# googlegenomics/spark-examples

Hardware: NVIDIA B200
Metric: genotype-cells/sec (N x V) into Gram (higher is better)
Workload: dtype int8

## Files before the change

### include/vpca.h

```cpp
#ifndef VPCA_H_
#define VPCA_H_

#include <stddef.h>
#include <stdint.h>

#ifdef __cplusplus
extern "C" {
#endif

#define VPCA_VERSION_MAJOR 0
#define VPCA_VERSION_MINOR 2

typedef enum vpca_status {
    VPCA_OK = 0,
    VPCA_ERR_BAD_ARG = -1,
    VPCA_ERR_INDEX_OUT_OF_RANGE = -2,
    VPCA_ERR_CUDA = -3,
    VPCA_ERR_NCCL = -4,
    VPCA_ERR_OVERFLOW = -5,
    VPCA_ERR_STATE = -6,
    VPCA_ERR_NOMEM = -7,
    VPCA_ERR_UNSUPPORTED = -8
} vpca_status;

typedef enum vpca_dtype {
    VPCA_DTYPE_I8 = 0,
    VPCA_DTYPE_BF16 = 1,
    VPCA_DTYPE_E2M1 = 2
} vpca_dtype;

typedef struct vpca_ctx vpca_ctx;

typedef struct vpca_config {
    uint32_t struct_size;
    int32_t n_samples;
    int32_t device;
    int32_t dtype;
    int32_t num_pc;
    int32_t max_multiplicity;
    int32_t partitions_in_flight;
    int32_t staging_lanes;
    int64_t chunk_variants;
    int64_t chunk_nnz;
    void* stream;
    void* d_gram;
    int32_t gram_band_row0;
    int32_t gram_band_rows;
} vpca_config;

int vpca_version(void);
int vpca_create(const vpca_config* cfg, vpca_ctx** out);
int vpca_destroy(vpca_ctx* ctx);
const char* vpca_last_error(const vpca_ctx* ctx);
int vpca_reset(vpca_ctx* ctx);
int vpca_synchronize(vpca_ctx* ctx);
int vpca_host_alloc(size_t bytes, void** out);
int vpca_host_free(void* p);

int vpca_encode_calls(vpca_ctx* ctx, const int64_t* offsets, const int32_t* sample_idx, int64_t nv, void* out,
                      int64_t ld);

int vpca_accumulate_calls(vpca_ctx* ctx, int64_t partition_id, const int64_t* offsets, const int32_t* sample_idx,
                          int64_t nv);
int vpca_accumulate_calls_u16(vpca_ctx* ctx, int64_t partition_id, const int64_t* offsets, const uint16_t* sample_idx,
                              int64_t nv);
int vpca_accumulate_bits(vpca_ctx* ctx, int64_t partition_id, const uint8_t* bits, int64_t nv, int64_t stride_bytes);
int vpca_accumulate_bed(vpca_ctx* ctx, int64_t partition_id, const uint8_t* rows, int64_t nv, int64_t stride_bytes,
                        int32_t counted_allele);
int vpca_commit(vpca_ctx* ctx, int64_t partition_id);
int vpca_abort(vpca_ctx* ctx, int64_t partition_id);

int vpca_accumulate_dense(vpca_ctx* ctx, const void* x, int64_t nv, int64_t ld, int on_device);

int vpca_accumulate_panels(vpca_ctx* ctx, const void* d_x, int64_t nv, int64_t panel_variants);

int vpca_gram_device_ptr(vpca_ctx* ctx, void** d_gram);
int vpca_gram_export_ipc(vpca_ctx* ctx, void* handle64);
int vpca_gram_set_peers(vpca_ctx* ctx, const void* handles, int32_t world, int32_t rank);
int vpca_gram_set_peers_local(vpca_ctx* const* ctxs, int32_t world);
int vpca_peer_barrier(vpca_ctx* ctx);
enum { VPCA_PEER_REPLICATE = 0, VPCA_PEER_OWNER_ROWS = 1 };
int vpca_gram_set_peer_mode(vpca_ctx* ctx, int32_t mode);
int vpca_gram_gather(vpca_ctx* ctx);
int vpca_owner_row_bands(int32_t n_samples, int32_t world, int32_t* row_end );
int vpca_get_gram_band(vpca_ctx* ctx, int32_t row0, int32_t rows, int32_t* out);

int vpca_finalize_gram(vpca_ctx* ctx);
int vpca_get_gram(vpca_ctx* ctx, int32_t* out);
int vpca_get_partial_gram(vpca_ctx* ctx, int32_t* out, int64_t* variants_in_gram );
int vpca_load_partial_gram(vpca_ctx* ctx, const int32_t* gram, int64_t variants_in_gram);
int64_t vpca_variant_count(vpca_ctx* ctx);
int vpca_set_gram(vpca_ctx* ctx, const int32_t* gram);

int vpca_compute_pca(vpca_ctx* ctx, int32_t k, double* vecs, double* evals, int32_t* non_zero_rows);
int vpca_get_centered(vpca_ctx* ctx, double* out);
int vpca_get_tridiagonal(vpca_ctx* ctx, double* diag, double* offdiag);

typedef struct vpca_projection {
    uint32_t struct_size;
    int32_t n_projected;
    const int32_t* sample_rows;
} vpca_projection;
int vpca_create_projecting(const vpca_config* cfg, const vpca_projection* proj, vpca_ctx** out);
int vpca_get_cross_gram(vpca_ctx* ctx, int32_t* out);
int vpca_project_pca(vpca_ctx* ctx, int32_t k, double* out);
int vpca_pca_loadings_calls(vpca_ctx* ctx, int32_t k, const int64_t* offsets, const int32_t* sample_idx, int64_t nv,
                            double* loadings, int32_t* carriers);
int vpca_pca_loadings_bed(vpca_ctx* ctx, int32_t k, const uint8_t* rows, int64_t nv, int64_t stride_bytes,
                          int32_t counted_allele, double* loadings, int32_t* carriers);
int vpca_pca_loadings_panels(vpca_ctx* ctx, int32_t k, const void* d_x, int64_t nv, int64_t panel_variants,
                             double* loadings, int32_t* carriers);
int vpca_pca_model_terms(vpca_ctx* ctx, int32_t k, double* eigenvalues, double* col_sums, double* rowsum_dots,
                         double* matrix_mean);

typedef struct vpca_model {
    uint32_t struct_size;
    int32_t n_fitted, k;
    int64_t n_variants;
    const double* loadings;
    const int32_t* carriers;
    const double* eigenvalues, *col_sums, *rowsum_dots;
    double matrix_mean;
} vpca_model;
int vpca_create_scoring(const vpca_config* cfg, const vpca_model* model, vpca_ctx** out);
int vpca_score_calls(vpca_ctx* ctx, int64_t partition_id, const int64_t* offsets, const int32_t* sample_idx, int64_t nv,
                     const int32_t* model_rows);
int vpca_score_bed(vpca_ctx* ctx, int64_t partition_id, const uint8_t* rows, int64_t nv, int64_t stride_bytes,
                   int32_t counted_allele, const int32_t* model_rows);
int vpca_score_panels(vpca_ctx* ctx, const void* d_x, int64_t nv, int64_t panel_variants, const int32_t* model_rows);
int vpca_score_project(vpca_ctx* ctx, int32_t k, double* out, int64_t* matched_variants );

int vpca_debug_projection_tiles(int32_t n_fit, int32_t n_total, int32_t cta_group, int32_t mxf4, int32_t* out,
                                int32_t max_tiles);

typedef struct vpca_pool vpca_pool;
int vpca_pool_create(const vpca_config* cfg, int32_t n_gpus, const int32_t* devices ,
                     vpca_pool** out);
int vpca_pool_destroy(vpca_pool* pool);
int32_t vpca_pool_size(const vpca_pool* pool);
vpca_ctx* vpca_pool_ctx(vpca_pool* pool, int64_t partition_id);
const char* vpca_pool_last_error(const vpca_pool* pool);
int vpca_pool_reset(vpca_pool* pool);
int vpca_pool_accumulate_calls(vpca_pool* pool, int64_t partition_id, const int64_t* offsets, const int32_t* sample_idx,
                               int64_t nv);
int vpca_pool_accumulate_calls_u16(vpca_pool* pool, int64_t partition_id, const int64_t* offsets,
                                   const uint16_t* sample_idx, int64_t nv);
int vpca_pool_accumulate_bits(vpca_pool* pool, int64_t partition_id, const uint8_t* bits, int64_t nv, int64_t stride_bytes);
int vpca_pool_accumulate_bed(vpca_pool* pool, int64_t partition_id, const uint8_t* rows, int64_t nv, int64_t stride_bytes,
                             int32_t counted_allele);
int vpca_pool_commit(vpca_pool* pool, int64_t partition_id);
int vpca_pool_abort(vpca_pool* pool, int64_t partition_id);
int vpca_pool_reduce_and_finalize(vpca_pool* pool);
int vpca_pool_get_gram(vpca_pool* pool, int32_t* out);
int vpca_pool_compute_pca(vpca_pool* pool, int32_t k, double* vecs, double* evals, int32_t* non_zero_rows);
struct vpca_stats;
int vpca_pool_get_stats(vpca_pool* pool, struct vpca_stats* out);

int vpca_synth_dense_device(vpca_ctx* ctx, uint64_t seed, int64_t v0, int64_t nv, int mode, void* d_x, int64_t ld);

int vpca_synth_panels_device(vpca_ctx* ctx, uint64_t seed, int64_t v0, int64_t nv, int mode, void* d_x,
                             int64_t panel_variants);

typedef struct vpca_stats {
    int64_t variants_accumulated;
    int64_t gram_launches;
    int64_t kernel_launches;
    int64_t h2d_bytes;
    int64_t d2h_bytes;
    float last_gram_ms;
    float last_eig_ms;
    int32_t gram_cta_group;
    int32_t gram_resident;
    int32_t eig_method;
    int32_t eig_iterations;
} vpca_stats;
int vpca_get_stats(vpca_ctx* ctx, vpca_stats* out);
int vpca_debug_gram_profile(vpca_ctx* ctx, int64_t* out, int32_t max_ctas);
int vpca_debug_lanczos_profile(vpca_ctx* ctx, int64_t* out, int32_t max_steps);

#define VPCA_JOIN 0
#define VPCA_MERGE 1
int vpca_hash_keys(vpca_ctx* ctx, const uint8_t* payload, const int64_t* key_offsets, int64_t nkeys, uint64_t* out);
int vpca_join_rows(vpca_ctx* ctx, int32_t mode, int32_t variant_set_count, int64_t n_left, const uint8_t* key_payload,
                   const int64_t* key_offsets, const int64_t* offsets, const int32_t* sample_idx, int64_t nrows,
                   int64_t* out_rows, int64_t* out_nnz);
int vpca_join_fetch(vpca_ctx* ctx, int64_t* out_offsets, int32_t* out_idx);
int vpca_join_size(vpca_ctx* ctx, int64_t* out_rows, int64_t* out_nnz);
int vpca_accumulate_joined(vpca_ctx* ctx, int64_t partition_id);

int vpca_debug_rebalance(const int32_t* tiles, int32_t num_tiles, int32_t workers, int32_t kb_window, int32_t col_limit,
                         double* cum, int32_t* out, int32_t max_pieces);
int vpca_debug_tiles(int32_t n_samples, int32_t cta_group, int32_t exact, int32_t* out, int32_t max_tiles);
int vpca_debug_band_tiles(int32_t n_samples, int32_t cta_group, int32_t row0, int32_t rows, int32_t* out, int32_t max_tiles);
int vpca_debug_max_clusters(int32_t device, int32_t cluster_size);
int vpca_debug_plan(const int32_t* tiles, int32_t num_tiles, int32_t workers, int32_t kb_window, int32_t* out, int32_t max_pieces);

#ifdef __cplusplus
}
#endif
#endif
```

### spark_examples_b200/csrc/gram_sm100.cu

```cuda
#include <cuda.h>
#include <cuda_runtime.h>

#include <cstring>

#include <algorithm>
#include <map>
#include <mutex>
#include <tuple>
#include <cstdio>
#include <cstdlib>
#include <string>
#include <vector>

#include "ptx_sm100.cuh"
#include "vpca_internal.h"

namespace vpca {

namespace {

constexpr int kThreads = 256;
constexpr int kKBytes = 128;
constexpr int kBoxRows = 128;
constexpr int kBoxBytes = kBoxRows * kKBytes;
constexpr int kUmmaN = 256;
constexpr int kUmmaNScaled = 240;
constexpr uint32_t kSfCol = 480;
constexpr uint32_t kTmemCols = 512;
constexpr long long kWatchdogCycles = 20000000000LL;

template <int CG, int KIND = 0>
struct Cfg {
    static constexpr int A_BYTES = kBoxBytes;
    static constexpr int B_BYTES = (kUmmaN / CG) * kKBytes;
    static constexpr int STAGE_BYTES = A_BYTES + B_BYTES;
    static constexpr int STAGES = CG == 1 ? 4 : 6;
    static constexpr int BAR_BYTES = 256;
    static constexpr int SMEM_BYTES = STAGES * STAGE_BYTES + BAR_BYTES + 1024;
};

constexpr int kMaxPeers = 16;

struct TileDesc {
    int rowA0, rowA1;
    int rowB;
    int n_eff;
    int wstart;
    int flags;
    int acc_cols;
    int pad1;
};
constexpr int kTileXpose = 1, kTileFiller = 2, kTileSelfB = 4;
constexpr int kMaxSegs = 4;

struct GramArgs {
    int32_t* S;
    int32_t* peer[kMaxPeers];
    int num_peers;
    int peer_mode;
    int own_end[kMaxPeers];
    const TileDesc* tiles;
    int* err;
    int n_cols;
    int num_tiles;
    int num_full;
    int total_weight;
    int kb_total;
    int kb_window;
    int num_workers;
    int resident;
    int elems_per_kb;
    int kb_per_panel;
    int sync_lead;
    int active_workers;
    int* win_done;
    long long* prof;
    const double* cum;
    int col_limit;
    int acc_stride;
    int row_limit;
    int red64;
    int tx_shift;
};

struct Seg {
    int tile, kb0, kb1, col, slot, first, flush, use, win, last_in_win;
    int rowA0, rowA1, rowB, n_eff, flags;
};

struct SegPlan {
    int n;
    int tile[kMaxSegs], lo[kMaxSegs], hi[kMaxSegs], col[kMaxSegs];
    int cols;
    int overflow;
};

__host__ __device__ inline void plan_segments(const TileDesc* tiles, int num_tiles, int first_tile, long long u_begin,
                                              long long u_end, int len, SegPlan& p) {
    p.n = 0;
    p.cols = 0;
    p.overflow = 0;
    const long long origin = (long long)tiles[first_tile].wstart * len;
    long long u = u_begin;
    int t = first_tile;
    while (u < u_end && t < num_tiles) {
        const int w = tiles[t].n_eff >> 4;
        const long long base = (long long)tiles[t].wstart * len - origin;
        const long long tend = base + (long long)w * len;
        if (tend <= u) {
            ++t;
            continue;
        }
        const long long e = u_end < tend ? u_end : tend;
        const int lo = (int)((u - base) / w);
        const int hi = e == tend ? len : (int)((e - base) / w);
        u = e;
        if (lo >= hi) continue;
        if (p.n == kMaxSegs) {
            p.overflow = 1;
            return;
        }
        p.tile[p.n] = t;
        p.lo[p.n] = lo;
        p.hi[p.n] = hi;
        p.col[p.n] = p.cols;
        p.cols += tiles[t].acc_cols;
        ++p.n;
    }
}

__host__ __device__ inline long long feasible_end(const TileDesc* tiles, int num_tiles, long long u_begin, long long u_end,
                                                  int len, int col_limit, int& hint) {
    int n = 0, cols = 0;
    long long u = u_begin;
    int t = hint;
    bool first = true;
    while (u < u_end && t < num_tiles) {
        const int w = tiles[t].n_eff >> 4;
        const long long base = (long long)tiles[t].wstart * len;
        const long long tend = base + (long long)w * len;
        if (tend <= u) {
            ++t;
            continue;
        }
        if (first) {
            hint = t;
            first = false;
        }
        const long long e = u_end < tend ? u_end : tend;
        const int lo = (int)((u - base) / w);
        const int hi = e == tend ? len : (int)((e - base) / w);
        if (lo < hi) {
            if (n == kMaxSegs || cols + tiles[t].acc_cols > col_limit) return u;
            ++n;
            cols += tiles[t].acc_cols;
        }
        u = e;
    }
    return u_end;
}

__host__ __device__ inline bool repair_split(const TileDesc* tiles, int num_tiles, int workers, long long uw, int len,
                                             int col_limit, double* cand) {
    long long ub = 0;
    int hint = 0;
    for (int i = 0; i < workers; ++i) {
        long long ue = (i + 1 == workers) ? uw : (long long)((double)uw * cand[i + 1]);
        if (ue < ub) ue = ub;
        const long long fe = feasible_end(tiles, num_tiles, ub, ue, len, col_limit, hint);
        if (fe < ue) {
            if (i + 1 == workers) return false;
            ue = fe;
        }
        if (i + 1 < workers) cand[i + 1] = ((double)ue + 0.5) / (double)uw;
        ub = ue;
    }
    return true;
}

struct Sched {
    SegPlan plan;
    long long u_begin, u_end, u;
    int kbw, nwin, kb_total, resident, win, seg_i, nflush, acc_stride;
    int worker, workers, num_tiles, wave, full_waves, tail_first;
    const TileDesc* tiles;

    __device__ void init(const GramArgs& a, int w) {
        kbw = a.kb_window;
        kb_total = a.kb_total;
        resident = a.resident;
        acc_stride = a.acc_stride;
        worker = w;
        workers = a.num_workers;
        num_tiles = a.num_tiles;
        tiles = a.tiles;
        nwin = (kb_total + kbw - 1) / kbw;
        win = 0;
        seg_i = 0;
        nflush = 0;
        wave = 0;
        if (resident) {
            const long long uw = (long long)a.total_weight * kbw;
            u_begin = (long long)((double)uw * a.cum[worker]);
            u_end = (worker + 1 == a.num_workers) ? uw : (long long)((double)uw * a.cum[worker + 1]);
            plan_segments(tiles, num_tiles, 0, u_begin, u_end, kbw, plan);
            if (plan.overflow || plan.cols > a.col_limit) {
                if (a.err != nullptr && threadIdx.x == 0) {
                    a.err[0] = 9;
                    a.err[1] = (int)blockIdx.x;
                    a.err[2] = plan.cols;
                    a.err[3] = plan.n;
                    __threadfence_system();
                }
                __trap();
            }
        } else {
            full_waves = a.num_full / workers;
            tail_first = full_waves * workers;
            const long long tail_units =
                tail_first < num_tiles ? (long long)(a.total_weight - tiles[tail_first].wstart) * kb_total : 0;
            u_begin = tail_units * worker / workers;
            u_end = tail_units * (worker + 1) / workers;
            plan.n = 0;
        }
        u = u_begin;
    }
    __device__ void fill(Seg& s, int t) const {
        const int4 lo = __ldg(reinterpret_cast<const int4*>(tiles + t));
        const int4 hi = __ldg(reinterpret_cast<const int4*>(tiles + t) + 1);
        s.tile = t;
        s.rowA0 = lo.x;
        s.rowA1 = lo.y;
        s.rowB = lo.z;
        s.n_eff = lo.w;
        s.flags = hi.y;
    }
    __device__ bool next(Seg& s) {
        if (!resident) {
            s.win = 0;
            s.last_in_win = 0;
            s.first = 1;
            s.flush = 1;
            s.slot = nflush & 1;
            s.col = s.slot * acc_stride;
            s.use = nflush >> 1;
            if (wave < full_waves) {
                fill(s, wave * workers + worker);
                s.kb0 = 0;
                s.kb1 = kb_total;
                ++wave;
                ++nflush;
                return true;
            }
            while (true) {
                if (seg_i < plan.n) {
                    fill(s, plan.tile[seg_i]);
                    s.kb0 = plan.lo[seg_i];
                    s.kb1 = plan.hi[seg_i];
                    ++seg_i;
                    ++nflush;
                    return true;
                }
                if (u >= u_end) return false;
                plan_segments(tiles, num_tiles, tail_first, u, u_end, kb_total, plan);
                seg_i = 0;
                if (plan.n == 0) return false;
                const int lt = plan.tile[plan.n - 1];
                const long long base = (long long)(tiles[lt].wstart - tiles[tail_first].wstart) * kb_total;
                const long long endu = base + (long long)plan.hi[plan.n - 1] * (tiles[lt].n_eff >> 4);
                u = plan.overflow ? endu : u_end;
            }
        }
        if (plan.n == 0) return false;
        if (seg_i == plan.n) {
            ++win;
            seg_i = 0;
        }
        if (win >= nwin) return false;
        const int i = seg_i++;
        fill(s, plan.tile[i]);
        const int base = win * kbw;
        const int cnt = min(kbw, kb_total - base);
        s.kb0 = base + min(plan.lo[i], cnt);
        s.kb1 = base + min(plan.hi[i], cnt);
        s.win = win;
        s.last_in_win = (seg_i == plan.n);
        s.col = plan.col[i];
        s.slot = i;
        s.first = (win == 0);
        s.flush = (win == nwin - 1);
        s.use = 0;
        return true;
    }
};

__device__ __forceinline__ void mbar_wait(uint32_t bar, uint32_t parity, int* err, int code) {
    if (ptx::mbar_try_wait(bar, parity)) return;
    const long long t0 = clock64();
    while (!ptx::mbar_try_wait(bar, parity)) {
        if (clock64() - t0 > kWatchdogCycles) {
            if (err != nullptr) {
                err[0] = code;
                err[1] = (int)blockIdx.x;
                err[2] = (int)bar;
                err[3] = (int)parity;
                __threadfence_system();
            }
            __trap();
        }
    }
}

__device__ __forceinline__ long long globaltimer_ns() {
    long long t;
    asm volatile("mov.u64 %0, %%globaltimer;" : "=l"(t));
    return t;
}

__device__ __forceinline__ void wait_window(const int* win_done, int w, int need) {
    const long long t0 = globaltimer_ns();
    while (true) {
        int v;
        asm volatile("ld.acquire.gpu.global.s32 %0, [%1];" : "=r"(v) : "l"(win_done + w) : "memory");
        if (v >= need) return;
        if (globaltimer_ns() - t0 > 200000) return;
        __nanosleep(256);
    }
}

__device__ __forceinline__ uint64_t make_smem_desc(uint32_t saddr) {
    return (uint64_t)((saddr & 0x3FFFFu) >> 4) | ((uint64_t)(1024 >> 4) << 32) | (1ull << 46) | (2ull << 61);
}

template <int CG, int KIND>
__device__ __forceinline__ uint32_t make_instr_desc(uint32_t N) {
    constexpr uint32_t M = 128 * CG;
    if constexpr (KIND == 3) {
        return (1u << 7) | (1u << 10) | ((N >> 3) << 17) | (1u << 23) | ((M >> 4) << 24);
    }
    constexpr uint32_t cfmt = (KIND == 0) ? 2u : 1u;
    constexpr uint32_t abfmt = (KIND == 2) ? 5u : 1u;
    return (cfmt << 4) | (abfmt << 7) | (abfmt << 10) | ((N >> 3) << 17) | ((M >> 4) << 24);
}

template <int CG, int KIND>
__global__ void __launch_bounds__(kThreads, 1) gram_kernel(const __grid_constant__ CUtensorMap tmap,
                                                           const __grid_constant__ CUtensorMap tmap_half, const GramArgs a) {
    using C = Cfg<CG, KIND>;
    extern __shared__ uint8_t smem_raw[];
    uint8_t* smem = reinterpret_cast<uint8_t*>((reinterpret_cast<uintptr_t>(smem_raw) + 1023) & ~uintptr_t(1023));
    const uint32_t smem_base = ptx::smem_u32(smem);
    const uint32_t bar_base = smem_base + C::STAGES * C::STAGE_BYTES;
    auto sA = [&](uint32_t st) { return smem_base + st * C::A_BYTES; };
    auto sB = [&](uint32_t st) { return smem_base + C::STAGES * C::A_BYTES + st * C::B_BYTES; };
    auto full_bar = [&](uint32_t i) { return bar_base + 8u * i; };
    auto empty_bar = [&](uint32_t i) { return bar_base + 8u * (C::STAGES + i); };
    auto tfull_bar = [&](uint32_t i) { return bar_base + 8u * (2 * C::STAGES + i); };
    auto tempty_bar = [&](uint32_t i) { return bar_base + 8u * (2 * C::STAGES + kMaxSegs + i); };
    volatile uint32_t* tmem_ptr_smem =
        reinterpret_cast<volatile uint32_t*>(smem + C::STAGES * C::STAGE_BYTES + 8 * (2 * C::STAGES + kMaxSegs + 2));

    const int warp = __shfl_sync(0xffffffffu, (int)(threadIdx.x >> 5), 0);
    const uint32_t lane = ptx::lane_id();
    const uint32_t cta_rank = (CG == 2) ? ptx::cluster_ctarank() : 0u;
    const bool leader = cta_rank == 0;
    const int worker = (CG == 2) ? (int)(blockIdx.x >> 1) : (int)blockIdx.x;
    const bool issuer = ptx::elect_one();

    if constexpr (CG == 2) ptx::cluster_sync();

    if (warp == 0 && issuer) {
        ptx::prefetch_tensormap(&tmap);
        ptx::prefetch_tensormap(&tmap_half);
    } else if (warp == 1 && issuer) {
        for (uint32_t i = 0; i < (uint32_t)C::STAGES; ++i) {
            ptx::mbar_init(full_bar(i), CG);
            ptx::mbar_init(empty_bar(i), 1);
        }
        for (uint32_t i = 0; i < (uint32_t)kMaxSegs; ++i) ptx::mbar_init(tfull_bar(i), 1);
        for (uint32_t i = 0; i < 2; ++i) ptx::mbar_init(tempty_bar(i), CG * 128);
        ptx::fence_mbar_init();
    } else if (warp == 2) {
        ptx::tmem_alloc<CG>(ptx::smem_u32(const_cast<uint32_t*>(tmem_ptr_smem)), kTmemCols);
        ptx::tmem_relinquish<CG>();
    }
    ptx::tc_fence_before();
    if constexpr (CG == 2) ptx::cluster_sync(); else __syncthreads();
    ptx::tc_fence_after();
    const uint32_t tmem_base = *tmem_ptr_smem;
    if constexpr (KIND == 3) {
        if (warp >= 4) {
            ptx::tmem_st_32x32b_x16_const(tmem_base + ((uint32_t)((warp & 3) * 32) << 16) + kSfCol, 0x7F7F7F7Fu);
            ptx::tmem_st_wait();
        }
        ptx::tc_fence_before();
        if constexpr (CG == 2) ptx::cluster_sync(); else __syncthreads();
        ptx::tc_fence_after();
    }
    if (a.prof != nullptr && threadIdx.x == 0) a.prof[(size_t)blockIdx.x * 4 + 0] = globaltimer_ns();

    if (warp == 0) {
        if (issuer) {
            Sched sc;
            sc.init(a, worker);
            Seg s;
            uint32_t it = 0;
            int synced_win = -1;
            while (sc.next(s)) {
                const int rowA = (CG == 2 && cta_rank != 0) ? s.rowA1 : s.rowA0;
                const int rowB = s.rowB + ((CG == 2) ? (int)cta_rank * (s.n_eff / 2) : 0);
                const bool half_box = (CG == 2) && (s.n_eff <= 128);
                const bool two_boxes = (CG == 1) && (s.n_eff > kBoxRows);
                const bool self_b = (CG == 2) && (s.flags & kTileSelfB) != 0;
                const uint32_t tx_cta =
                    (uint32_t)(C::A_BYTES + (self_b ? 0 : (half_box ? kBoxBytes / 2 : (two_boxes ? 2 * kBoxBytes : kBoxBytes))));
                if (a.sync_lead > 0 && leader && s.win != synced_win) {
                    synced_win = s.win;
                    if (s.win >= a.sync_lead) wait_window(a.win_done, s.win - a.sync_lead, a.active_workers);
                }
                for (int kb = s.kb0; kb < s.kb1; ++kb, ++it) {
                    const uint32_t st = it % C::STAGES, ph = (it / C::STAGES) & 1u;
                    mbar_wait(empty_bar(st), ph ^ 1u, a.err, 1);
                    const int pnl = kb / a.kb_per_panel;
                    const int kc = (kb - pnl * a.kb_per_panel) * a.elems_per_kb;
                    if constexpr (CG == 1) {
                        ptx::mbar_arrive_expect_tx(full_bar(st), tx_cta >> a.tx_shift);
                        ptx::tma_load_3d(sA(st), &tmap, full_bar(st), kc, rowA, pnl);
                        ptx::tma_load_3d(sB(st), &tmap, full_bar(st), kc, rowB, pnl);
                        if (two_boxes) ptx::tma_load_3d(sB(st) + kBoxBytes, &tmap, full_bar(st), kc, rowB + kBoxRows, pnl);
                    } else {
                        ptx::tma_load_3d_2sm(sA(st), &tmap, full_bar(st), kc, rowA, pnl);
                        if (!self_b) ptx::tma_load_3d_2sm(sB(st), half_box ? &tmap_half : &tmap, full_bar(st), kc, rowB, pnl);
                        if (leader) ptx::mbar_arrive_expect_tx(full_bar(st), (2u * tx_cta) >> a.tx_shift);
                        else ptx::mbar_arrive_cluster(full_bar(st), 0);
                    }
                }
                if (a.sync_lead > 0 && leader && s.last_in_win)
                    asm volatile("red.release.gpu.global.add.s32 [%0], 1;" ::"l"(a.win_done + s.win) : "memory");
            }
        }
    } else if (warp == 1 && leader) {
        Sched sc;
        sc.init(a, worker);
        Seg s;
        uint32_t it = 0;
        while (sc.next(s)) {
            if (s.first && !a.resident) {
                mbar_wait(tempty_bar((uint32_t)s.slot), (uint32_t)(s.use & 1) ^ 1u, a.err, 2);
                ptx::tc_fence_after();
            }
            const uint32_t d_tmem = tmem_base + (uint32_t)s.col;
            const uint32_t idesc = make_instr_desc<CG, KIND>((uint32_t)s.n_eff);
            for (int kb = s.kb0; kb < s.kb1; ++kb, ++it) {
                const uint32_t st = it % C::STAGES, ph = (it / C::STAGES) & 1u;
                mbar_wait(full_bar(st), ph, a.err, 3);
                ptx::tc_fence_after();
                if (issuer) {
                    const uint64_t adesc = make_smem_desc(sA(st));
                    const uint64_t bdesc = make_smem_desc((CG == 2 && (s.flags & kTileSelfB) != 0) ? sA(st) : sB(st));
                    uint32_t acc = (s.first && kb == s.kb0) ? 0u : 1u;
#pragma unroll
                    for (int k = 0; k < kKBytes / 32; ++k) {
                        if constexpr (KIND == 3)
                            ptx::umma_ss_mxf4<CG>(d_tmem, adesc + 2 * k, bdesc + 2 * k, idesc, acc, tmem_base + kSfCol,
                                                  tmem_base + kSfCol + 4);
                        else
                            ptx::umma_ss<CG, KIND>(d_tmem, adesc + 2 * k, bdesc + 2 * k, idesc, acc);
                        acc = 1u;
                    }
                    ptx::umma_commit<CG>(empty_bar(st));
                }
                __syncwarp();
            }
            if (s.flush) {
                if (issuer) ptx::umma_commit<CG>(tfull_bar((uint32_t)s.slot));
                __syncwarp();
            }
        }
        if (a.prof != nullptr && issuer) a.prof[(size_t)blockIdx.x * 4 + 2] = globaltimer_ns();
    } else if (warp >= 4) {
        const int q = warp & 3;
        Sched sc;
        sc.init(a, worker);
        Seg s;
        while (sc.next(s)) {
            if (!s.flush) continue;
            const uint32_t bar_i = (uint32_t)s.slot;
            mbar_wait(tfull_bar(bar_i), (uint32_t)(s.use & 1), a.err, 4);
            ptx::tc_fence_after();
            const bool filler = (CG == 2) && cta_rank != 0 && (s.flags & kTileFiller) != 0;
            const int colbase = ((CG == 2 && cta_rank != 0) ? s.rowA1 : s.rowA0) + q * 32;
            const int col = colbase + (int)lane;
            const uint32_t taddr = tmem_base + ((uint32_t)(q * 32) << 16) + (uint32_t)s.col;
            const int row_end = min(a.row_limit, s.rowB + s.n_eff);
            const int nchunks = filler ? 0 : (s.n_eff + 31) / 32;
#pragma unroll 1
            for (int c = 0; c < nchunks; ++c) {
                const int rbase = s.rowB + c * 32;
                if (rbase >= row_end) break;
                bool xpose = false;
                if (rbase + 31 < colbase) {
                    if ((s.flags & kTileXpose) == 0 || (rbase >> 7) >= (colbase >> 7)) continue;
                    xpose = true;
                }
                uint32_t r[32];
                ptx::tmem_ld_32x32b_x32(taddr + (uint32_t)(c * 32), r);
                ptx::tmem_ld_wait();
                int32_t* own_lo = nullptr;
                int32_t* own_hi = nullptr;
                int own_split = 0;
                if (a.num_peers != 0 && a.peer_mode == 1) {
                    const int probe = xpose ? col : rbase;
                    int o = 0;
                    while (o + 1 < a.num_peers && probe >= a.own_end[o]) ++o;
                    own_split = xpose ? 0x7fffffff : a.own_end[o];
                    own_lo = a.peer[o];
                    own_hi = a.peer[min(o + 1, a.num_peers - 1)];
                }
                if (!xpose && a.red64 != 0 && (a.n_cols & 1) == 0) {
#pragma unroll
                    for (int jj = 0; jj < 16; ++jj) {
                        const int row0 = rbase + 2 * jj, row1 = row0 + 1;
                        int v0, v1;
                        if constexpr (KIND == 0) { v0 = (int)r[2 * jj]; v1 = (int)r[2 * jj + 1]; }
                        else { v0 = __float2int_rn(__uint_as_float(r[2 * jj])); v1 = __float2int_rn(__uint_as_float(r[2 * jj + 1])); }
                        if (!(row0 < row_end && col < a.n_cols && row0 >= col)) v0 = 0;
                        if (!(row1 < row_end && col < a.n_cols && row1 >= col)) v1 = 0;
                        const int got = __shfl_xor_sync(0xffffffffu, (lane & 1) ? v0 : v1, 1);
                        const int srow = (lane & 1) ? row1 : row0;
                        const unsigned long long packed = (lane & 1)
                            ? ((unsigned long long)(unsigned)got | ((unsigned long long)(unsigned)v1 << 32))
                            : ((unsigned long long)(unsigned)v0 | ((unsigned long long)(unsigned)got << 32));
                        if (packed != 0ull) {
                            const size_t o = (size_t)srow * (size_t)a.n_cols + (size_t)(col & ~1);
                            if (a.num_peers == 0) {
                                asm volatile("red.global.add.u64 [%0], %1;" ::"l"(a.S + o), "l"(packed) : "memory");
                            } else if (a.peer_mode == 1) {
                                int32_t* dst = (srow >= own_split ? own_hi : own_lo) + o;
                                asm volatile("red.relaxed.sys.global.add.u64 [%0], %1;" ::"l"(dst), "l"(packed) : "memory");
                            } else {
                                for (int d = 0; d < a.num_peers; ++d)
                                    asm volatile("red.relaxed.sys.global.add.u64 [%0], %1;" ::"l"(a.peer[d] + o), "l"(packed)
                                                 : "memory");
                            }
                        }
                    }
                    continue;
                }
#pragma unroll
                for (int j = 0; j < 32; ++j) {
                    const int row = rbase + j;
                    if (row < row_end && col < a.n_cols && (xpose || row >= col)) {
                        int v;
                        if constexpr (KIND == 0) v = (int)r[j];
                        else v = __float2int_rn(__uint_as_float(r[j]));
                        if (v != 0) {
                            const int srow = xpose ? col : row, scol = xpose ? row : col;
                            const size_t o = (size_t)srow * (size_t)a.n_cols + (size_t)scol;
                            if (a.num_peers == 0) {
                                asm volatile("red.global.add.s32 [%0], %1;" ::"l"(a.S + o), "r"(v) : "memory");
                            } else if (a.peer_mode == 1) {
                                int32_t* dst = (srow >= own_split ? own_hi : own_lo) + o;
                                asm volatile("red.relaxed.sys.global.add.s32 [%0], %1;" ::"l"(dst), "r"(v) : "memory");
                            } else {
                                for (int d = 0; d < a.num_peers; ++d)
                                    asm volatile("red.relaxed.sys.global.add.s32 [%0], %1;" ::"l"(a.peer[d] + o), "r"(v)
                                                 : "memory");
                            }
                        }
                    }
                }
            }
            ptx::tc_fence_before();
            if (!a.resident) {
                if constexpr (CG == 1) ptx::mbar_arrive(tempty_bar(bar_i));
                else ptx::mbar_arrive_cluster(tempty_bar(bar_i), 0);
            }
        }
    }

    ptx::tc_fence_before();
    if constexpr (CG == 2) ptx::cluster_sync(); else __syncthreads();
    if (warp == 2) ptx::tmem_dealloc<CG>(tmem_base, kTmemCols);
    if (a.prof != nullptr && threadIdx.x == 0) a.prof[(size_t)blockIdx.x * 4 + 3] = globaltimer_ns();
}

__global__ void rebalance_kernel(const long long* __restrict__ prof, double* __restrict__ cum, int workers, int cta_group,
                                 double gain, double max_share, long long min_ns, int* __restrict__ gen, const TileDesc* __restrict__ tiles,
                                 int num_tiles, int total_weight, int kbw, int col_limit) {
    __shared__ double sh[1024];
    __shared__ double cand[1025];
    __shared__ double red_sum, red_min;
    __shared__ int reject, need_repair;
    const int w = threadIdx.x;
    const bool active = w < workers;
    double t = 0.0, share_old = 0.0;
    if (active) {
        const long long t0 = prof[(size_t)w * cta_group * 4 + 0], t1 = prof[(size_t)w * cta_group * 4 + 2];
        t = (double)(t1 - t0);
        share_old = cum[w + 1] - cum[w];
    }
    sh[w] = active ? t : 1e30;
    if (w == 0) {
        reject = 0;
        need_repair = 0;
    }
    __syncthreads();
    if (w == 0) {
        double mn = 1e30, mx = 0.0;
        for (int i = 0; i < workers; ++i) {
            mn = fmin(mn, sh[i]);
            mx = fmax(mx, sh[i]);
        }
        red_min = (mn < (double)min_ns || (mx - mn) < 0.03 * mx) ? -1.0 : mn;
    }
    __syncthreads();
    if (red_min < 0.0) return;
    const double speed = active ? share_old / t : 0.0;
    sh[w] = speed;
    __syncthreads();
    if (w == 0) {
        double sum = 0.0;
        for (int i = 0; i < workers; ++i) sum += sh[i];
        red_sum = sum;
    }
    __syncthreads();
    double share = 0.0;
    if (active) {
        const double est = speed / red_sum;
        share = (1.0 - gain) * share_old + gain * est;
        const double avg = 1.0 / workers;
        share = fmin(fmax(share, 0.5 * avg), max_share * avg);
    }
    __syncthreads();
    sh[w] = share;
    __syncthreads();
    if (w == 0) {
        double sum = 0.0;
        for (int i = 0; i < workers; ++i) sum += sh[i];
        double acc = 0.0;
        cand[0] = 0.0;
        for (int i = 0; i < workers; ++i) {
            acc += sh[i] / sum;
            cand[i + 1] = (i + 1 == workers) ? 1.0 : acc;
        }
    }
    __syncthreads();
    if (active) {
// ... 2 lines not shown
        const long long ue = (w + 1 == workers) ? uw : (long long)((double)uw * cand[w + 1]);
        int hint = 0;
        if (feasible_end(tiles, num_tiles, ub, ue, kbw, col_limit, hint) < ue) atomicExch(&need_repair, 1);
    }
    __syncthreads();
    if (need_repair && w == 0 && !repair_split(tiles, num_tiles, workers, (long long)total_weight * kbw, kbw, col_limit, cand)) reject = 1;
    __syncthreads();
    if (reject) return;
    if (w <= workers) cum[w] = cand[w];
    if (w == 0) *gen += 1;
}

__global__ void symmetrize_kernel(int32_t* __restrict__ S, int n) {
    __shared__ int32_t tile[32][33];
    const int bx = blockIdx.x, by = blockIdx.y;
    if (bx < by) return;
    const int tx = threadIdx.x, ty = threadIdx.y;
    for (int r = ty; r < 32; r += 8) {
        const int row = bx * 32 + r, col = by * 32 + tx;
        tile[r][tx] = (row < n && col < n) ? S[(size_t)row * n + col] : 0;
    }
    __syncthreads();
    for (int r = ty; r < 32; r += 8) {
        const int row = by * 32 + r, col = bx * 32 + tx;
        if (row < n && col < n && row < col) S[(size_t)row * n + col] = tile[tx][r];
    }
}

__global__ void add_i32_kernel(int32_t* __restrict__ dst, const int32_t* __restrict__ src, int64_t count) {
    int64_t i = (int64_t)blockIdx.x * blockDim.x + threadIdx.x;
    const int64_t stride = (int64_t)gridDim.x * blockDim.x;
    for (; i < count; i += stride) dst[i] += src[i];
}

struct PeerPtrs {
    int32_t* p[kMaxPeers];
};

__global__ void add_i32_peers_kernel(PeerPtrs dst, int npeers, const int32_t* __restrict__ src, int64_t count) {
    int64_t i = (int64_t)blockIdx.x * blockDim.x + threadIdx.x;
    const int64_t stride = (int64_t)gridDim.x * blockDim.x;
    for (; i < count; i += stride) {
        const int v = src[i];
        if (v != 0)
            for (int d = 0; d < npeers; ++d)
                asm volatile("red.relaxed.sys.global.add.s32 [%0], %1;" ::"l"(dst.p[d] + i), "r"(v) : "memory");
    }
}

struct OwnEnds {
    int e[kMaxPeers];
};

__device__ __forceinline__ int owner_of_row(const OwnEnds& own, int npeers, int row) {
    int q = 0;
    while (q + 1 < npeers && row >= own.e[q]) ++q;
    return q;
}

__global__ void add_i32_owner_kernel(PeerPtrs dst, OwnEnds own, int npeers, const int32_t* __restrict__ src, int n) {
    for (int row = blockIdx.x; row < n; row += gridDim.x) {
        int32_t* d = dst.p[owner_of_row(own, npeers, row)] + (size_t)row * n;
        const int32_t* s = src + (size_t)row * n;
        for (int c = threadIdx.x; c <= row; c += blockDim.x) {
            const int v = s[c];
            if (v != 0) asm volatile("red.relaxed.sys.global.add.s32 [%0], %1;" ::"l"(d + c), "r"(v) : "memory");
        }
    }
}

__global__ void __launch_bounds__(256) gather_rows_kernel(PeerPtrs src, int32_t* __restrict__ dst, OwnEnds own, int npeers,
                                                          int rank, int n) {
    const bool vec = (n & 3) == 0;
    for (int row = blockIdx.x; row < n; row += gridDim.x) {
        const int q = owner_of_row(own, npeers, row);
        if (q == rank) continue;
        const int32_t* s = src.p[q] + (size_t)row * n;
        int32_t* d = dst + (size_t)row * n;
        if (vec) {
            const int4* s4 = reinterpret_cast<const int4*>(s);
            int4* d4 = reinterpret_cast<int4*>(d);
            for (int c = threadIdx.x; c < (row + 4) / 4; c += blockDim.x) d4[c] = s4[c];
        } else {
            for (int c = threadIdx.x; c <= row; c += blockDim.x) d[c] = s[c];
        }
    }
}

__global__ void __launch_bounds__(256) push_rows_kernel(PeerPtrs dst, const int32_t* __restrict__ src, OwnEnds own,
                                                        int npeers, int rank, int n) {
    const bool vec = (n & 3) == 0;
    const int row_lo = rank == 0 ? 0 : own.e[rank - 1], row_hi = own.e[rank];
    for (int row = row_lo + blockIdx.x; row < row_hi; row += gridDim.x) {
        const int32_t* s = src + (size_t)row * n;
        if (vec) {
            const int4* s4 = reinterpret_cast<const int4*>(s);
            for (int c = threadIdx.x; c < (row + 4) / 4; c += blockDim.x) {
                const int4 v = s4[c];
                for (int d = 0; d < npeers; ++d)
                    if (d != rank) reinterpret_cast<int4*>(dst.p[d] + (size_t)row * n)[c] = v;
            }
        } else {
            for (int c = threadIdx.x; c <= row; c += blockDim.x) {
                const int v = s[c];
                for (int d = 0; d < npeers; ++d)
                    if (d != rank) dst.p[d][(size_t)row * n + c] = v;
            }
        }
    }
}

__global__ void peer_barrier_kernel(PeerPtrs flags, int npeers, int rank, int epoch) {
    const int d = threadIdx.x;
    if (d < npeers) {
        __threadfence_system();
        asm volatile("st.release.sys.global.s32 [%0], %1;" ::"l"(flags.p[d] + rank), "r"(epoch) : "memory");
        int v;
        const long long t0 = globaltimer_ns();
        do {
            asm volatile("ld.acquire.sys.global.s32 %0, [%1];" : "=r"(v) : "l"(flags.p[rank] + d) : "memory");
            if (v < epoch && globaltimer_ns() - t0 > 30000000000LL) __trap();
        } while (v < epoch);
    }
    __syncthreads();
    __threadfence_system();
}

typedef CUresult (*EncodeTiledFn)(CUtensorMap*, CUtensorMapDataType, cuuint32_t, void*, const cuuint64_t*,
                                  const cuuint64_t*, const cuuint32_t*, const cuuint32_t*, CUtensorMapInterleave,
                                  CUtensorMapSwizzle, CUtensorMapL2promotion, CUtensorMapFloatOOBfill);

EncodeTiledFn get_encode_fn() {
    static EncodeTiledFn fn = nullptr;
    if (fn == nullptr) {
        void* p = nullptr;
        cudaDriverEntryPointQueryResult qres;
        if (cudaGetDriverEntryPoint("cuTensorMapEncodeTiled", &p, cudaEnableDefault, &qres) == cudaSuccess &&
            qres == cudaDriverEntryPointSuccess)
            fn = reinterpret_cast<EncodeTiledFn>(p);
    }
    return fn;
}

template <int CG, int KIND>
cudaError_t launch(const CUtensorMap& tmap, const CUtensorMap& tmap_half, const GramArgs& args, int grid, cudaStream_t stream) {
    using C = Cfg<CG, KIND>;
    cudaError_t ea = cudaFuncSetAttribute(gram_kernel<CG, KIND>, cudaFuncAttributeMaxDynamicSharedMemorySize, C::SMEM_BYTES);
    if (ea != cudaSuccess) return ea;
    cudaLaunchConfig_t cfg{};
    cfg.gridDim = dim3((unsigned)grid);
    cfg.blockDim = dim3(kThreads);
    cfg.dynamicSmemBytes = C::SMEM_BYTES;
    cfg.stream = stream;
    cudaLaunchAttribute attr[1];
    attr[0].id = cudaLaunchAttributeClusterDimension;
    attr[0].val.clusterDim.x = CG;
    attr[0].val.clusterDim.y = 1;
    attr[0].val.clusterDim.z = 1;
    cfg.attrs = attr;
    cfg.numAttrs = 1;
    return cudaLaunchKernelEx(&cfg, gram_kernel<CG, KIND>, tmap, tmap_half, args);
}

}

namespace {
struct SplitKey {
    int dev, n, rows, tiles, kbw, workers, elem;
    bool operator<(const SplitKey& o) const {
        return std::tie(dev, n, rows, tiles, kbw, workers, elem) <
               std::tie(o.dev, o.n, o.rows, o.tiles, o.kbw, o.workers, o.elem);
    }
};
std::mutex g_split_mu;
std::map<SplitKey, std::vector<double>> g_splits;
}

static void remember_split(GramPlan& plan) {
    if (plan.d_cum == nullptr || plan.cum_workers <= 0 || !plan.adaptive) return;
    if (plan.own_hi > plan.own_lo && plan.num_peers <= 1) return;
    std::vector<double> cum((size_t)plan.cum_workers + 1);
    if (cudaMemcpy(cum.data(), plan.d_cum, cum.size() * sizeof(double), cudaMemcpyDeviceToHost) != cudaSuccess) {
        cudaGetLastError();
        return;
    }
    std::lock_guard<std::mutex> lk(g_split_mu);
    g_splits[SplitKey{plan.cum_dev, plan.cum_for_n, plan.cum_for_rows, plan.cum_tiles, plan.cum_kbw, plan.cum_workers, plan.cum_elem}] = std::move(cum);
}

void gram_plan_free(GramPlan& plan) {
    remember_split(plan);
    if (plan.d_tiles) cudaFree(plan.d_tiles);
    plan.h_tiles.clear();
    if (plan.d_err) cudaFreeHost(plan.d_err);
    if (plan.d_win_done) cudaFree(plan.d_win_done);
    if (plan.d_prof) cudaFree(plan.d_prof);
    if (plan.d_cum) cudaFree(plan.d_cum);
    plan.d_cum = nullptr;
    plan.d_win_done = nullptr;
    plan.d_prof = nullptr;
    plan.d_tiles = nullptr;
    plan.d_err = nullptr;
    plan.tiles_for_n = -1;
}

int gram_read_profile(GramPlan& plan, long long* out, int max_ctas) {
    if (plan.d_prof == nullptr) return 0;
    const int ctas = std::min(max_ctas, std::min(1024, plan.num_sms));
    if (cudaMemcpy(out, plan.d_prof, (size_t)ctas * 4 * sizeof(long long), cudaMemcpyDeviceToHost) != cudaSuccess) return 0;
    return ctas;
}

static void make_tiles(int n, int cg, bool exact, int bn, int row_lo, int row_hi, bool self_b, std::vector<TileDesc>& out,
                       int* num_full) {
    out.clear();
    auto n_eff = [&](int row0, int want) { return std::min(want, ((n - row0) + 15) & ~15); };
    if (!exact) {
        const int BM = 128 * cg;
        const int span = row_hi - row_lo;
        const int nbn = (span + bn - 1) / bn, nbm = (n + BM - 1) / BM;
        const int units = (span + 15) / 16;
        std::vector<int> row0(nbn + 1, row_lo);
        for (int b = 0; b < nbn; ++b) row0[b + 1] = row0[b] + 16 * (units / nbn + (b < units % nbn ? 1 : 0));
        constexpr int kStrip = 8;
        for (int bb = 0; bb < nbn; bb += kStrip)
            for (int am = 0; am < nbm; ++am)
                for (int b = bb; b < std::min(nbn, bb + kStrip); ++b) {
                    const int max_row = std::min(row_hi, row0[b + 1]) - 1;
                    if (am * BM > max_row) continue;
                    TileDesc t{};
                    t.rowA0 = am * BM;
                    t.rowA1 = am * BM + 128;
                    t.rowB = row0[b];
                    t.n_eff = std::min(row0[b + 1], ((row_hi + 15) & ~15)) - row0[b];
                    t.acc_cols = bn;
                    if (self_b && cg == 2 && t.rowB == t.rowA0 && t.n_eff == 2 * 128) t.flags |= kTileSelfB;
                    out.push_back(t);
                }
    } else {
        const int nb = (n + 127) / 128;
        std::vector<TileDesc> two, one;
        auto emit = [&](std::vector<TileDesc>& dst, int c0, int c1, int r0, int rows, bool filler) {
            TileDesc t{};
            t.rowA0 = c0 * 128;
            t.rowA1 = c1 * 128;
            t.rowB = r0 * 128;
            t.n_eff = n_eff(r0 * 128, rows * 128);
            t.acc_cols = (t.n_eff + 31) & ~31;
            t.flags = kTileXpose | (filler ? kTileFiller : 0);
            dst.push_back(t);
        };
        std::vector<std::vector<int>> need(nb);
        for (int r = 0; r < nb; ++r)
            for (int c = 0; c <= r; ++c) need[r].push_back(c);
        if (cg == 2)
            for (int r = 0; r + 2 < nb; r += 4) {
                need[r].push_back(r + 2);
                need[r + 2].erase(std::find(need[r + 2].begin(), need[r + 2].end(), r));
            }
        for (int r0 = 0; r0 < nb; r0 += 2) {
            const bool pair = r0 + 1 < nb;
            std::vector<int> common, left0, left1;
            if (pair) {
                for (int c : need[r0])
                    if (std::find(need[r0 + 1].begin(), need[r0 + 1].end(), c) != need[r0 + 1].end()) common.push_back(c);
                if (cg == 2 && (common.size() & 1)) common.pop_back();
            }
            for (int c : need[r0])
                if (std::find(common.begin(), common.end(), c) == common.end()) left0.push_back(c);
            if (pair)
                for (int c : need[r0 + 1])
                    if (std::find(common.begin(), common.end(), c) == common.end()) left1.push_back(c);
            for (size_t i = 0; i < common.size(); i += cg) emit(two, common[i], common[cg == 2 ? i + 1 : i], r0, 2, false);
            for (int side = 0; side < (pair ? 2 : 1); ++side) {
                const std::vector<int>& left = side == 0 ? left0 : left1;
                for (size_t i = 0; i < left.size(); i += cg) {
                    const bool filler = cg == 2 && i + 1 >= left.size();
                    emit(one, left[i], filler ? left[i] : left[cg == 2 ? i + 1 : i], r0 + side, 1, filler);
                }
            }
        }
        auto mid = std::stable_partition(two.begin(), two.end(), [&](const TileDesc& t) { return t.n_eff == 256; });
        std::stable_sort(two.begin(), mid, [](const TileDesc& x, const TileDesc& y) {
            const int sx = x.rowB / 1024, sy = y.rowB / 1024;
            if (sx != sy) return sx < sy;
            const int cx = std::min(x.rowA0, x.rowA1) / 256, cy = std::min(y.rowA0, y.rowA1) / 256;
            if (cx != cy) return cx < cy;
            return x.rowB < y.rowB;
        });
        *num_full = (int)(mid - two.begin());
        out = two;
        out.insert(out.end(), one.begin(), one.end());
    }
    if (!exact) *num_full = (int)out.size();
    int w = 0;
    for (auto& t : out) {
        t.wstart = w;
        w += t.n_eff >> 4;
    }
}

static cudaError_t build_tiles(GramPlan& plan, int n, bool exact, int BN, int row_lo, int row_hi, cudaStream_t stream) {
    std::vector<TileDesc> tiles;
    int num_full = 0;
    make_tiles(n, plan.cta_group, exact, BN, row_lo, row_hi, plan.self_b, tiles, &num_full);
    if (plan.d_tiles) cudaFree(plan.d_tiles);
    plan.d_tiles = nullptr;
    cudaError_t e = cudaMalloc(&plan.d_tiles, tiles.size() * sizeof(TileDesc));
    if (e != cudaSuccess) return e;
    e = cudaMemcpyAsync(plan.d_tiles, tiles.data(), tiles.size() * sizeof(TileDesc), cudaMemcpyHostToDevice, stream);
    if (e != cudaSuccess) return e;
    e = cudaStreamSynchronize(stream);
    plan.h_tiles.assign(reinterpret_cast<const int32_t*>(tiles.data()),
                        reinterpret_cast<const int32_t*>(tiles.data() + tiles.size()));
    plan.num_tiles = (int)tiles.size();
    plan.num_full = num_full;
    plan.total_weight = tiles.empty() ? 0 : tiles.back().wstart + (tiles.back().n_eff >> 4);
    plan.tiles_for_n = n;
    plan.tiles_for_cg = plan.cta_group;
    plan.tiles_for_bn = exact ? -1 : BN;
    plan.tiles_row_lo = row_lo;
    plan.tiles_row_hi = row_hi;
    plan.tiles_col_limit = (!exact && BN == kUmmaNScaled) ? (int)kSfCol : (int)kTmemCols;
    return e;
}

static bool initial_split(const GramPlan& plan, int workers, int kbw, std::vector<double>& cum) {
    if (plan.total_weight <= 0) return false;
    const TileDesc* tiles = reinterpret_cast<const TileDesc*>(plan.h_tiles.data());
    const long long uw = (long long)plan.total_weight * kbw;
    cum.resize((size_t)workers + 1);
    for (int w = 0; w <= workers; ++w) cum[w] = (double)w / (double)workers;
    if (!repair_split(tiles, plan.num_tiles, workers, uw, kbw, plan.tiles_col_limit, cum.data())) return false;
    for (int w = 0; w < workers; ++w) {
        const long long ub = (long long)((double)uw * cum[w]);
        const long long ue = (w + 1 == workers) ? uw : (long long)((double)uw * cum[w + 1]);
        SegPlan p;
        plan_segments(tiles, plan.num_tiles, 0, ub, ue, kbw, p);
        if (p.overflow || p.cols > plan.tiles_col_limit) return false;
    }
    return true;
}

int gram_debug_tiles(int n, int cta_group, int exact, int32_t* out, int max_tiles) {
    std::vector<TileDesc> tiles;
    int num_full = 0;
    make_tiles(n, cta_group == 1 ? 1 : 2, exact != 0, exact ? kUmmaN : kUmmaNScaled, 0, n, true, tiles, &num_full);
    const int cnt = std::min<int>((int)tiles.size(), max_tiles);
    if (out != nullptr && cnt > 0) memcpy(out, tiles.data(), (size_t)cnt * sizeof(TileDesc));
    return (int)tiles.size();
}

int gram_debug_projection_tiles(int n_fit, int n_total, int cta_group, bool mxf4, int32_t* out, int max_tiles) {
    std::vector<TileDesc> tiles;
    int num_full = 0;
    make_tiles(n_fit, cta_group == 1 ? 1 : 2, false, mxf4 ? kUmmaNScaled : kUmmaN, 0, n_total, true, tiles, &num_full);
    const int cnt = std::min<int>((int)tiles.size(), max_tiles);
    if (out != nullptr && cnt > 0) memcpy(out, tiles.data(), (size_t)cnt * sizeof(TileDesc));
    return (int)tiles.size();
}

int gram_debug_band_tiles(int n, int cta_group, int row_lo, int row_hi, int32_t* out, int max_tiles) {
    std::vector<TileDesc> tiles;
    int num_full = 0;
    make_tiles(n, cta_group == 1 ? 1 : 2, false, kUmmaN, row_lo, row_hi, true, tiles, &num_full);
    const int cnt = std::min<int>((int)tiles.size(), max_tiles);
    if (out != nullptr && cnt > 0) memcpy(out, tiles.data(), (size_t)cnt * sizeof(TileDesc));
    return (int)tiles.size();
}

int gram_debug_plan(const int32_t* tiles8, int num_tiles, int workers, int kbw, int32_t* out, int max_pieces) {
    const TileDesc* tiles = reinterpret_cast<const TileDesc*>(tiles8);
    if (num_tiles <= 0) return 0;
    const int col_limit = tiles[0].acc_cols == kUmmaNScaled ? (int)kSfCol : (int)kTmemCols;
    std::vector<double> cum((size_t)workers + 1);
    for (int w = 0; w <= workers; ++w) cum[w] = (double)w / (double)workers;
    return gram_debug_repair(tiles8, num_tiles, workers, kbw, col_limit, cum.data(), out, max_pieces);
}

int gram_debug_repair(const int32_t* tiles8, int num_tiles, int workers, int kbw, int col_limit, double* cum, int32_t* out,
                      int max_pieces) {
    const TileDesc* tiles = reinterpret_cast<const TileDesc*>(tiles8);
    if (num_tiles <= 0) return 0;
    const long long total = tiles[num_tiles - 1].wstart + (tiles[num_tiles - 1].n_eff >> 4);
    const long long uw = total * kbw;
    if (!repair_split(tiles, num_tiles, workers, uw, kbw, col_limit, cum)) return -1000;
    int cnt = 0;
    for (int w = 0; w < workers; ++w) {
        const long long ub = (long long)((double)uw * cum[w]);
        const long long ue = (w + 1 == workers) ? uw : (long long)((double)uw * cum[w + 1]);
        SegPlan p;
        plan_segments(tiles, num_tiles, 0, ub, ue, kbw, p);
        if (p.overflow || p.cols > col_limit) return -1 - w;
        for (int i = 0; i < p.n; ++i, ++cnt)
            if (cnt < max_pieces) {
                int32_t* o = out + (size_t)cnt * 6;
                o[0] = w; o[1] = p.tile[i]; o[2] = p.lo[i]; o[3] = p.hi[i]; o[4] = p.col[i]; o[5] = p.cols;
            }
    }
    return cnt;
}

cudaError_t gram_accumulate(GramPlan& plan, const void* d_x, int elem_bits, int n, int n_rows, int64_t nv, int64_t ld,
                            int64_t panel, int32_t* d_S, cudaStream_t stream, std::string* err) {
    if (nv <= 0) return cudaSuccess;
    EncodeTiledFn encode = get_encode_fn();
    if (encode == nullptr) {
        if (err) *err = "cuTensorMapEncodeTiled entry point not available";
        return cudaErrorNotSupported;
    }
    if (plan.num_sms == 0) {
        int dev = 0;
        cudaGetDevice(&dev);
        cudaDeviceGetAttribute(&plan.num_sms, cudaDevAttrMultiProcessorCount, dev);
        const char* cg = getenv("VPCA_CTA_GROUP");
        if (cg != nullptr) plan.cta_group = (atoi(cg) == 1) ? 1 : 2;
        const char* kw = getenv("VPCA_KB_WINDOW");
        if (kw != nullptr) plan.kb_window = atoi(kw);
        const char* sl = getenv("VPCA_SYNC_LEAD");
        if (sl != nullptr) plan.sync_lead = atoi(sl);
        const char* pf = getenv("VPCA_GRAM_PROF");
        plan.profile = (pf != nullptr && atoi(pf) != 0);
        const char* ad = getenv("VPCA_ADAPTIVE");
        if (ad != nullptr) plan.adaptive = atoi(ad) != 0;
        const char* mx = getenv("VPCA_E2M1_MXF4");
        if (mx != nullptr) plan.e2m1_mxf4 = atoi(mx) != 0;
        const char* sb = getenv("VPCA_SELF_B");
        if (sb != nullptr) plan.self_b = atoi(sb) != 0;
        const char* r64 = getenv("VPCA_RED64");
        if (r64 != nullptr) plan.red64 = atoi(r64) != 0;
        const char* gain = getenv("VPCA_REBALANCE_GAIN");
        if (gain != nullptr) plan.gain = std::min(1.0, std::max(0.1, atof(gain)));
        const char* ex = getenv("VPCA_EXACT_COVER");
        if (ex != nullptr) plan.exact_cover = atoi(ex) != 0;
    }
    if (plan.d_win_done == nullptr) {
        cudaError_t e = cudaMalloc(&plan.d_win_done, GramPlan::kMaxWindows * sizeof(int));
        if (e != cudaSuccess) return e;
    }
    if ((plan.profile || plan.adaptive) && plan.d_prof == nullptr) {
        cudaError_t e = cudaMalloc(&plan.d_prof, 1024 * 4 * sizeof(long long));
        if (e != cudaSuccess) return e;
        e = cudaMemsetAsync(plan.d_prof, 0, 1024 * 4 * sizeof(long long), stream);
        if (e != cudaSuccess) return e;
    }
    if (plan.d_err == nullptr) {
        cudaError_t e = cudaHostAlloc(&plan.d_err, 4 * sizeof(int), cudaHostAllocMapped);
        if (e != cudaSuccess) return e;
        for (int i = 0; i < 4; ++i) plan.d_err[i] = 0;
    }
    const bool mxf4 = (elem_bits == 4 && plan.e2m1_mxf4);
    const int tile_bn = mxf4 ? kUmmaNScaled : kUmmaN;
    const bool banded = plan.own_hi > plan.own_lo && plan.num_peers <= 1;
    const int row_lo = banded ? plan.own_lo : 0, row_hi = banded ? plan.own_hi : n_rows;
    const bool exact = !mxf4 && plan.exact_cover && !banded;
    if ((banded || exact || plan.num_peers > 1) && n_rows != n) {
        if (err) *err = "projected rows need the rectangle tiling without peers or bands";
        return cudaErrorNotSupported;
    }
    if (plan.tiles_for_n != n || plan.tiles_for_cg != plan.cta_group || plan.tiles_for_bn != (exact ? -1 : tile_bn) ||
        plan.tiles_row_lo != row_lo || plan.tiles_row_hi != row_hi) {
        cudaError_t e = build_tiles(plan, n, exact, tile_bn, row_lo, row_hi, stream);
        if (e != cudaSuccess) return e;
    }
    if (panel > 0) {
        if ((panel % 128) != 0) {
            if (err) *err = "panel_variants must be a multiple of 128";
            return cudaErrorInvalidValue;
        }
        ld = panel;
    }
    const uintptr_t align = (elem_bits == 4) ? 31 : 15;
    if ((reinterpret_cast<uintptr_t>(d_x) & align) != 0 || (((ld * elem_bits) / 8) & align) != 0 ||
        (elem_bits == 4 && (ld % 128) != 0)) {
        if (err) *err = "dense tile must be 16-byte aligned with a 16-byte multiple row pitch (32 / ld % 128 == 0 for e2m1)";
        return cudaErrorInvalidValue;
    }

    const int cgp = plan.cta_group;
    const int workers = (cgp == 2) ? plan.num_sms / 2 : plan.num_sms;
    const int elems_per_kb = (elem_bits == 16) ? 64 : (mxf4 ? 256 : 128);
    const int kind = (elem_bits == 8) ? 0 : (elem_bits == 16 ? 1 : (mxf4 ? 3 : 2));
    if (mxf4 && panel > 0 && (panel % 256) != 0) {
        if (err) *err = "kind::mxf4 needs panel_variants % 256 == 0";
        return cudaErrorInvalidValue;
    }

    CUtensorMap tmap;
    const int64_t npanels = panel > 0 ? (nv + panel - 1) / panel : 1;
    const int64_t dim0 = panel > 0 ? panel : (elem_bits == 4 ? (mxf4 ? ((nv + 1) / 2) * 2 : ((nv + 127) / 128) * 128) : nv);
    const cuuint64_t gdim[3] = {(cuuint64_t)dim0, (cuuint64_t)n_rows, (cuuint64_t)npanels};
    const cuuint64_t gstride[2] = {(cuuint64_t)ld * (cuuint64_t)elem_bits / 8,
                                   (cuuint64_t)n_rows * (cuuint64_t)ld * (cuuint64_t)elem_bits / 8};
    const cuuint32_t box[3] = {(cuuint32_t)elems_per_kb, (cuuint32_t)kBoxRows, 1};
    const cuuint32_t estr[3] = {1, 1, 1};
    const CUtensorMapDataType tmtype = elem_bits == 8 ? CU_TENSOR_MAP_DATA_TYPE_UINT8
                                       : (elem_bits == 16 ? CU_TENSOR_MAP_DATA_TYPE_BFLOAT16
                                                          : (mxf4 ? CU_TENSOR_MAP_DATA_TYPE_16U4_ALIGN8B
                                                                  : CU_TENSOR_MAP_DATA_TYPE_16U4_ALIGN16B));
    CUresult r = encode(&tmap, tmtype, 3,
                        const_cast<void*>(d_x), gdim, gstride, box, estr, CU_TENSOR_MAP_INTERLEAVE_NONE,
                        CU_TENSOR_MAP_SWIZZLE_128B, CU_TENSOR_MAP_L2_PROMOTION_L2_256B,
                        CU_TENSOR_MAP_FLOAT_OOB_FILL_NONE);
    if (r != CUDA_SUCCESS) {
        if (err) *err = "cuTensorMapEncodeTiled failed with CUresult " + std::to_string((int)r);
        return cudaErrorInvalidValue;
    }
    CUtensorMap tmap_half;
    const cuuint32_t box_half[3] = {(cuuint32_t)elems_per_kb, (cuuint32_t)(kBoxRows / 2), 1};
    r = encode(&tmap_half, tmtype, 3, const_cast<void*>(d_x), gdim, gstride, box_half, estr, CU_TENSOR_MAP_INTERLEAVE_NONE,
               CU_TENSOR_MAP_SWIZZLE_128B, CU_TENSOR_MAP_L2_PROMOTION_L2_256B, CU_TENSOR_MAP_FLOAT_OOB_FILL_NONE);
    if (r != CUDA_SUCCESS) {
        if (err) *err = "cuTensorMapEncodeTiled (64-row box) failed with CUresult " + std::to_string((int)r);
        return cudaErrorInvalidValue;
    }

    GramArgs args{};
    args.S = banded ? d_S - (ptrdiff_t)plan.own_lo * n : d_S;
    args.num_peers = (plan.num_peers > 1 && d_S == plan.peer_base[plan.peer_rank]) ? plan.num_peers : 0;
    for (int d = 0; d < kMaxPeers; ++d) args.peer[d] = d < plan.num_peers ? plan.peer_S[d] : nullptr;
    args.peer_mode = plan.peer_mode;
    for (int d = 0; d < kMaxPeers; ++d) args.own_end[d] = plan.own_end[d];
    args.tiles = static_cast<const TileDesc*>(plan.d_tiles);
    cudaHostGetDevicePointer(reinterpret_cast<void**>(&args.err), plan.d_err, 0);
    args.n_cols = n;
    args.num_tiles = plan.num_tiles;
    args.num_full = plan.num_full;
    args.total_weight = plan.total_weight;
    args.kb_total = (int)((nv + elems_per_kb - 1) / elems_per_kb);
    args.kb_per_panel = panel > 0 ? (int)(panel / elems_per_kb) : args.kb_total;
    args.num_workers = workers;
    args.elems_per_kb = elems_per_kb;
    args.acc_stride = mxf4 ? kUmmaNScaled : kUmmaN;
    args.col_limit = plan.tiles_col_limit;
    args.row_limit = row_hi;
    args.red64 = plan.red64 ? 1 : 0;
    {
        int kbw = plan.kb_window;
        if (kbw <= 0 && panel > 0) kbw = args.kb_per_panel;
        if (kbw <= 0) {
            const long long target = 32ll << 20;
            kbw = (int)std::max<long long>(8, std::min<long long>(4096, target / ((long long)n_rows * kKBytes)));
        }
        kbw = std::min(kbw, args.kb_total);
        std::vector<double> cum0;
        args.resident = (plan.num_tiles <= 4 * workers && initial_split(plan, workers, kbw, cum0)) ? 1 : 0;
        int dev = 0;
        cudaGetDevice(&dev);
        args.kb_window = args.resident ? kbw : args.kb_total;
        if (args.resident && (plan.d_cum == nullptr || plan.cum_workers != workers || plan.cum_tiles != plan.num_tiles ||
                              plan.cum_kbw != kbw || plan.cum_for_n != n || plan.cum_for_rows != n_rows ||
                              plan.cum_elem != elem_bits)) {
            remember_split(plan);
            if (plan.adaptive && !banded) {
                std::lock_guard<std::mutex> lk(g_split_mu);
                auto it = g_splits.find(SplitKey{dev, n, n_rows, plan.num_tiles, kbw, workers, elem_bits});
                if (it != g_splits.end()) {
                    std::vector<double> learned = it->second;
                    const TileDesc* tiles = reinterpret_cast<const TileDesc*>(plan.h_tiles.data());
                    if (repair_split(tiles, plan.num_tiles, workers, (long long)plan.total_weight * kbw, kbw, plan.tiles_col_limit,
                                     learned.data()))
                        cum0 = learned;
                }
            }
            if (plan.d_cum) cudaFree(plan.d_cum);
            plan.d_cum = nullptr;
            cudaError_t e = cudaMalloc(&plan.d_cum, (size_t)(workers + 2) * sizeof(double) + sizeof(int));
            if (e != cudaSuccess) return e;
            cum0.push_back(0.0);
            cum0.push_back(0.0);
            e = cudaMemcpyAsync(plan.d_cum, cum0.data(), (size_t)(workers + 2) * sizeof(double) + sizeof(int),
                                cudaMemcpyHostToDevice, stream);
            if (e != cudaSuccess) return e;
            plan.cum_workers = workers;
            plan.cum_tiles = plan.num_tiles;
            plan.cum_kbw = kbw;
            plan.cum_for_n = n;
            plan.cum_for_rows = n_rows;
            plan.cum_dev = dev;
            plan.cum_elem = elem_bits;
        }
    }
    plan.last_resident = args.resident;
    const int nwin = (args.kb_total + args.kb_window - 1) / args.kb_window;
    const long long uw = (long long)args.total_weight * args.kb_window;
    args.active_workers = (int)std::min<long long>(workers, uw);
    args.sync_lead = (args.resident && nwin <= GramPlan::kMaxWindows) ? plan.sync_lead : 0;
    args.win_done = plan.d_win_done;
    const bool adapt = plan.adaptive && args.resident && workers <= 1024 && args.active_workers == workers;
    args.prof = (plan.profile || adapt) ? plan.d_prof : nullptr;
    args.cum = plan.d_cum;
    args.tx_shift = (elem_bits == 4 && !mxf4 && getenv("VPCA_E2M1_TX_FULL") == nullptr) ? 1 : 0;
    if (args.sync_lead > 0) {
        cudaError_t e = cudaMemsetAsync(plan.d_win_done, 0, (size_t)nwin * sizeof(int), stream);
        if (e != cudaSuccess) return e;
    }

    const int grid = workers * cgp;
    cudaError_t le;
    if (cgp == 2)
        le = kind == 0 ? launch<2, 0>(tmap, tmap_half, args, grid, stream)
                       : (kind == 1 ? launch<2, 1>(tmap, tmap_half, args, grid, stream)
                                    : (kind == 2 ? launch<2, 2>(tmap, tmap_half, args, grid, stream) : launch<2, 3>(tmap, tmap_half, args, grid, stream)));
    else
        le = kind == 0 ? launch<1, 0>(tmap, tmap_half, args, grid, stream)
                       : (kind == 1 ? launch<1, 1>(tmap, tmap_half, args, grid, stream)
                                    : (kind == 2 ? launch<1, 2>(tmap, tmap_half, args, grid, stream) : launch<1, 3>(tmap, tmap_half, args, grid, stream)));
    if (le != cudaSuccess) return le;
    if (adapt) {
        rebalance_kernel<<<1, 1024, 0, stream>>>(plan.d_prof, plan.d_cum, workers, cgp, plan.gain, 1.35, 300000,
                                                 reinterpret_cast<int*>(plan.d_cum + workers + 2), static_cast<const TileDesc*>(plan.d_tiles), plan.num_tiles,
                                                 plan.total_weight, args.kb_window, plan.tiles_col_limit);
        le = cudaGetLastError();
    }
    return le;
}

cudaError_t gram_preload_kernels(cudaStream_t stream) {
    cudaFuncAttributes fa;
    cudaError_t e = cudaSuccess;
#define VPCA_LOAD(k) if (e == cudaSuccess) e = cudaFuncGetAttributes(&fa, k)
    VPCA_LOAD((gram_kernel<1, 0>)); VPCA_LOAD((gram_kernel<1, 1>)); VPCA_LOAD((gram_kernel<1, 2>)); VPCA_LOAD((gram_kernel<1, 3>));
    VPCA_LOAD((gram_kernel<2, 0>)); VPCA_LOAD((gram_kernel<2, 1>)); VPCA_LOAD((gram_kernel<2, 2>)); VPCA_LOAD((gram_kernel<2, 3>));
    VPCA_LOAD(rebalance_kernel); VPCA_LOAD(symmetrize_kernel); VPCA_LOAD(add_i32_kernel); VPCA_LOAD(add_i32_peers_kernel);
    VPCA_LOAD(add_i32_owner_kernel); VPCA_LOAD(gather_rows_kernel); VPCA_LOAD(push_rows_kernel); VPCA_LOAD(peer_barrier_kernel);
#undef VPCA_LOAD
    if (e != cudaSuccess) return e;
    PeerPtrs pp{};
    OwnEnds own{};
    peer_barrier_kernel<<<1, 32, 0, stream>>>(pp, 0, 0, 0);
    push_rows_kernel<<<1, 32, 0, stream>>>(pp, nullptr, own, 0, 0, 0);
    gather_rows_kernel<<<1, 32, 0, stream>>>(pp, nullptr, own, 0, 0, 0);
    add_i32_owner_kernel<<<1, 32, 0, stream>>>(pp, own, 0, nullptr, 0);
    add_i32_peers_kernel<<<1, 32, 0, stream>>>(pp, 0, nullptr, 0);
    add_i32_kernel<<<1, 32, 0, stream>>>(nullptr, nullptr, 0);
    symmetrize_kernel<<<dim3(1, 1), dim3(32, 8), 0, stream>>>(nullptr, 0);
    return cudaGetLastError();
}

int gram_debug_max_clusters(int cluster_size) {
    using C = Cfg<2, 0>;
    if (cudaFuncSetAttribute(gram_kernel<2, 0>, cudaFuncAttributeMaxDynamicSharedMemorySize, C::SMEM_BYTES) != cudaSuccess) return -1;
    if (cluster_size > 8 &&
        cudaFuncSetAttribute(gram_kernel<2, 0>, cudaFuncAttributeNonPortableClusterSizeAllowed, 1) != cudaSuccess) return -1;
    int sms = 0, dev = 0;
    cudaGetDevice(&dev);
    cudaDeviceGetAttribute(&sms, cudaDevAttrMultiProcessorCount, dev);
    cudaLaunchConfig_t cfg{};
    cfg.gridDim = dim3((unsigned)(sms / cluster_size * cluster_size));
    cfg.blockDim = dim3(kThreads);
    cfg.dynamicSmemBytes = C::SMEM_BYTES;
    cudaLaunchAttribute attr[1];
    attr[0].id = cudaLaunchAttributeClusterDimension;
    attr[0].val.clusterDim.x = (unsigned)cluster_size;
    attr[0].val.clusterDim.y = 1;
    attr[0].val.clusterDim.z = 1;
    cfg.attrs = attr;
    cfg.numAttrs = 1;
    int clusters = 0;
    if (cudaOccupancyMaxActiveClusters(&clusters, gram_kernel<2, 0>, &cfg) != cudaSuccess) {
        cudaGetLastError();
        return -1;
    }
    return clusters;
}

cudaError_t gram_symmetrize(int32_t* d_S, int n, cudaStream_t stream) {
    const int nb = (n + 31) / 32;
    symmetrize_kernel<<<dim3(nb, nb), dim3(32, 8), 0, stream>>>(d_S, n);
    return cudaGetLastError();
}

cudaError_t gram_add(int32_t* d_dst, const int32_t* d_src, int64_t count, cudaStream_t stream) {
    add_i32_kernel<<<592, 256, 0, stream>>>(d_dst, d_src, count);
    return cudaGetLastError();
}

cudaError_t gram_add_peers(GramPlan& plan, const int32_t* d_src, int64_t count, cudaStream_t stream) {
    PeerPtrs pp{};
    for (int d = 0; d < plan.num_peers; ++d) pp.p[d] = plan.peer_S[d];
    add_i32_peers_kernel<<<592, 256, 0, stream>>>(pp, plan.num_peers, d_src, count);
    return cudaGetLastError();
}

cudaError_t gram_add_owners(GramPlan& plan, const int32_t* d_src, int n, cudaStream_t stream) {
    PeerPtrs pp{};
    OwnEnds own{};
    for (int d = 0; d < plan.num_peers; ++d) pp.p[d] = plan.peer_S[d];
    for (int d = 0; d < kMaxPeers; ++d) own.e[d] = plan.own_end[d];
    add_i32_owner_kernel<<<592, 256, 0, stream>>>(pp, own, plan.num_peers, d_src, n);
    return cudaGetLastError();
}

cudaError_t gram_gather_rows(GramPlan& plan, int32_t* d_S, int n, cudaStream_t stream) {
    PeerPtrs pp{};
    OwnEnds own{};
    for (int d = 0; d < plan.num_peers; ++d) pp.p[d] = plan.peer_S[d];
    for (int d = 0; d < kMaxPeers; ++d) own.e[d] = plan.own_end[d];
    const char* how = getenv("VPCA_GATHER");
    if (how != nullptr && strcmp(how, "pull") == 0) {
        gather_rows_kernel<<<1184, 256, 0, stream>>>(pp, d_S, own, plan.num_peers, plan.peer_rank, n);
    } else if (how != nullptr && strcmp(how, "copy") == 0) {
        for (int q = 0; q < plan.num_peers; ++q) {
            if (q == plan.peer_rank) continue;
            const int r0 = q == 0 ? 0 : plan.own_end[q - 1], r1 = plan.own_end[q];
            cudaError_t e = cudaMemcpy2DAsync(d_S + (size_t)r0 * n, (size_t)n * 4, plan.peer_S[q] + (size_t)r0 * n,
                                              (size_t)n * 4, (size_t)std::min(n, r1) * 4, (size_t)(r1 - r0),
                                              cudaMemcpyDeviceToDevice, stream);
            if (e != cudaSuccess) return e;
        }
    } else {
        push_rows_kernel<<<1184, 256, 0, stream>>>(pp, d_S, own, plan.num_peers, plan.peer_rank, n);
    }
    return cudaGetLastError();
}

cudaError_t gram_peer_barrier(GramPlan& plan, cudaStream_t stream) {
    PeerPtrs pp{};
    for (int d = 0; d < plan.num_peers; ++d) pp.p[d] = plan.peer_flags[d];
    plan.peer_epoch += 1;
    peer_barrier_kernel<<<1, 32, 0, stream>>>(pp, plan.num_peers, plan.peer_rank, plan.peer_epoch);
    return cudaGetLastError();
}

}
```

### spark_examples_b200/csrc/vpca.cu

```cuda
#include <cuda_runtime.h>

#include <algorithm>
#include <atomic>
#include <cmath>
#include <condition_variable>
#include <cstdarg>
#include <cstdio>
#include <cstring>
#include <map>
#include <mutex>
#include <string>
#include <vector>

#include "vpca_internal.h"

using namespace vpca;

namespace {
thread_local std::string tls_error;
thread_local const vpca_ctx* tls_error_ctx = nullptr;
thread_local std::string tls_error_copy;
}

struct vpca_ctx {
// ... 137 lines not shown
    return VPCA_OK;
}

void free_lane(vpca_ctx::Lane& L) {
    if (L.stream) cudaStreamSynchronize(L.stream);
    if (L.copy_stream) cudaStreamSynchronize(L.copy_stream);
    for (int b = 0; b < 2; ++b) {
        cudaFree(L.d_off[b]);
        cudaFree(L.d_idx[b]);
        cudaFree(L.d_x[b]);
        if (L.ev_copy[b]) cudaEventDestroy(L.ev_copy[b]);
        if (L.ev_done[b]) cudaEventDestroy(L.ev_done[b]);
        L.d_off[b] = nullptr;
        L.d_idx[b] = nullptr;
        L.d_x[b] = nullptr;
        L.ev_copy[b] = L.ev_done[b] = nullptr;
    }
    for (cudaEvent_t* ev : {&L.ev_order, &L.ev_t0, &L.ev_t1})
        if (*ev) {
            cudaEventDestroy(*ev);
            *ev = nullptr;
        }
    cudaFree(L.d_flags);
    L.d_flags = nullptr;
    cudaFree(L.d_scratch);
    L.d_scratch = nullptr;
    L.cap_scratch = 0;
    if (L.h_flags) cudaFreeHost(L.h_flags);
    L.h_flags = nullptr;
    gram_plan_free(L.plan);
    if (L.copy_stream) cudaStreamDestroy(L.copy_stream);
    if (L.stream) cudaStreamDestroy(L.stream);
    L.copy_stream = L.stream = nullptr;
    L.ready = false;
}

void copy_peers(const GramPlan& from, GramPlan& to) {
    to.own_lo = from.own_lo;
    to.own_hi = from.own_hi;
    to.num_peers = from.num_peers;
    to.peer_rank = from.peer_rank;
    to.peer_mode = from.peer_mode;
    for (int d = 0; d < 16; ++d) {
        to.peer_S[d] = from.peer_S[d];
        to.peer_flags[d] = from.peer_flags[d];
        to.own_end[d] = from.own_end[d];
    }
}

void sync_peers_to_lanes(vpca_ctx* ctx) {
    for (auto& L : ctx->lanes) copy_peers(ctx->plan, L.plan);
}

void staging_geometry(vpca_ctx* ctx) {
    if (ctx->chunk_variants != 0) return;
    const int n = ctx->rows(), bits = ctx->elem_bits;
    int64_t cv = ctx->cfg.chunk_variants;
    if (cv <= 0) {
        cv = (256ll << 20) * 8 / ((int64_t)n * bits);
        cv = std::max<int64_t>(1024, std::min<int64_t>(cv, 1 << 20));
    }
    if (const char* pe = getenv("VPCA_PANEL")) {
        const int64_t pv = atoll(pe);
        if (pv >= 128 && pv % 128 == 0) ctx->panel = pv;
    }
    cv = std::max<int64_t>(ctx->panel, (cv / ctx->panel) * ctx->panel);
    int64_t cz = ctx->cfg.chunk_nnz;
    if (cz <= 0) cz = 64ll << 20;
    cz = std::max<int64_t>(cz, 1024);
    ctx->chunk_variants = cv;
    ctx->chunk_nnz = cz;
}

int ensure_lane(vpca_ctx* ctx, vpca_ctx::Lane& L) {
    if (L.ready) return VPCA_OK;
    const int n = ctx->rows(), bits = ctx->elem_bits;
    const int64_t cv = ctx->chunk_variants, cz = ctx->chunk_nnz;
    cudaError_t e = cudaStreamCreateWithFlags(&L.stream, cudaStreamNonBlocking);
    if (e == cudaSuccess) e = cudaStreamCreateWithFlags(&L.copy_stream, cudaStreamNonBlocking);
    for (int b = 0; b < 2 && e == cudaSuccess; ++b) {
        e = cudaMalloc(&L.d_off[b], (size_t)(cv + 1) * sizeof(int64_t));
        if (e == cudaSuccess) e = cudaMalloc(&L.d_idx[b], (size_t)cz * sizeof(int32_t));
        if (e == cudaSuccess) e = cudaMalloc(&L.d_x[b], (size_t)n * (size_t)cv * bits / 8);
        if (e == cudaSuccess) e = cudaEventCreateWithFlags(&L.ev_copy[b], cudaEventDisableTiming);
        if (e == cudaSuccess) e = cudaEventCreateWithFlags(&L.ev_done[b], cudaEventDisableTiming);
    }
    if (e == cudaSuccess) e = cudaEventCreateWithFlags(&L.ev_order, cudaEventDisableTiming);
    if (e == cudaSuccess) e = cudaEventCreate(&L.ev_t0);
    if (e == cudaSuccess) e = cudaEventCreate(&L.ev_t1);
    if (e == cudaSuccess) e = cudaMalloc(&L.d_flags, sizeof(int));
    if (e == cudaSuccess) e = cudaHostAlloc(&L.h_flags, sizeof(int), cudaHostAllocPortable);
    if (e != cudaSuccess) {
        free_lane(L);
        return fail(ctx, e == cudaErrorMemoryAllocation ? VPCA_ERR_NOMEM : VPCA_ERR_CUDA, "staging lane: %s",
                    cudaGetErrorString(e));
    }
    copy_peers(ctx->plan, L.plan);
    L.ready = true;
    return VPCA_OK;
}

struct LaneGuard {
    vpca_ctx* ctx;
    vpca_ctx::Lane* lane = nullptr;
    int rc = VPCA_OK;
    explicit LaneGuard(vpca_ctx* c) : ctx(c) {
        std::unique_lock<std::mutex> lk(ctx->mu);
        staging_geometry(ctx);
        ctx->cv.wait(lk, [&] {
            for (auto& L : ctx->lanes)
                if (!L.busy) return true;
            return false;
        });
        for (auto& L : ctx->lanes)
            if (!L.busy) {
                lane = &L;
                break;
            }
        lane->busy = true;
        rc = ensure_lane(ctx, *lane);
        if (rc == VPCA_OK) {
            cudaError_t e = cudaEventRecord(lane->ev_order, ctx->stream);
            if (e == cudaSuccess) e = cudaStreamWaitEvent(lane->stream, lane->ev_order, 0);
            if (e != cudaSuccess) rc = fail(ctx, VPCA_ERR_CUDA, "lane ordering: %s", cudaGetErrorString(e));
        }
    }
    ~LaneGuard() {
        {
            std::lock_guard<std::mutex> lk(ctx->mu);
            lane->busy = false;
        }
        ctx->cv.notify_one();
    }
};

int launch_gram(vpca_ctx* ctx, GramPlan& plan, cudaStream_t stream, cudaEvent_t t0, cudaEvent_t t1, const void* d_x,
                int64_t nv, int64_t ld, int64_t panel, int32_t* d_target) {
    int64_t limit = nv;
    if (ctx->elem_bits != 8) {
        limit = (int64_t)(16777216ll / ((int64_t)ctx->max_mult * ctx->max_mult));
        const int64_t q = panel > 0 ? panel : 128;
        limit = (limit / q) * q;
        if (limit <= 0)
            return fail(ctx, VPCA_ERR_UNSUPPORTED, "max_multiplicity %d leaves no exact fp32 accumulation window for panels of "
                        "%lld variants", ctx->max_mult, (long long)q);
    }
    for (int64_t v0 = 0; v0 < nv; v0 += limit) {
        const int64_t cnt = std::min<int64_t>(limit, nv - v0);
        std::string msg;
        cudaEventRecord(t0, stream);
        const size_t byte_off = panel > 0 ? (size_t)(v0 / panel) * (size_t)ctx->rows() * (size_t)panel * ctx->elem_bits / 8
                                          : (size_t)v0 * ctx->elem_bits / 8;
        cudaError_t e = gram_accumulate(plan, static_cast<const char*>(d_x) + byte_off, ctx->elem_bits, ctx->n, ctx->rows(),
                                        cnt, ld, panel, d_target, stream, &msg);
        cudaEventRecord(t1, stream);
        if (e != cudaSuccess)
            return fail(ctx, VPCA_ERR_CUDA, "Gram launch failed: %s %s", cudaGetErrorString(e), msg.c_str());
        ctx->c_gram += 1;
        ctx->c_launches += 1;
    }
    return VPCA_OK;
}

vpca_ctx::Slot* find_slot(vpca_ctx* ctx, int64_t pid, bool create, int* rc) {
    *rc = VPCA_OK;
    for (auto& s : ctx->slots)
        if (s.used && s.pid == pid) return &s;
    if (!create) return nullptr;
    for (auto& s : ctx->slots)
        if (!s.used) {
            if (s.d_S == nullptr) {
                cudaError_t e = cudaMalloc(&s.d_S, ctx->slot_bytes());
                if (e == cudaSuccess) e = cudaEventCreateWithFlags(&s.ev_free, cudaEventDisableTiming);
                if (e != cudaSuccess) {
                    cudaFree(s.d_S);
                    s.d_S = nullptr;
                    *rc = fail(ctx, VPCA_ERR_NOMEM, "cudaMalloc of a partition Gram failed: %s", cudaGetErrorString(e));
                    return nullptr;
                }
            }
            s.used = true;
            s.fresh = true;
            s.busy = false;
            s.pid = pid;
            s.nv = 0;
            s.matched = 0;
            return &s;
        }
    *rc = fail(ctx, VPCA_ERR_STATE, "more than %d partitions in flight; commit or abort one first",
               (int)ctx->slots.size());
    return nullptr;
}

struct CallScope {
    vpca_ctx* ctx;
    int64_t pid, nv;
    int64_t matched = 0;
    vpca_ctx::Slot* slot = nullptr;
    int32_t* target = nullptr;
    bool fresh = false;
    int begin() {
        std::lock_guard<std::mutex> lk(ctx->mu);
        if (ctx->finalized) return fail(ctx, VPCA_ERR_STATE, "Gram already finalized; call vpca_reset first");
        int rc = ctx->scoring ? VPCA_OK : check_overflow(ctx, nv);
        if (rc != VPCA_OK) return rc;
        target = ctx->scoring ? reinterpret_cast<int32_t*>(ctx->d_direct) : ctx->d_S;
        if (pid >= 0) {
            slot = find_slot(ctx, pid, true, &rc);
            if (slot == nullptr) return rc;
            if (slot->busy) {
                slot = nullptr;
                return fail(ctx, VPCA_ERR_STATE, "partition %lld is being written by another thread (spark.speculation "
                            "must stay off)", (long long)pid);
            }
            slot->busy = true;
            fresh = slot->fresh;
            slot->fresh = false;
            target = slot->d_S;
            ctx->inflight_variants += nv;
        } else if (ctx->band_rows != ctx->n) {
            return fail(ctx, VPCA_ERR_STATE, "a band-only Gram takes device-resident input (vpca_accumulate_panels / "
                        "vpca_accumulate_dense with on_device = 1)");
        }
        return VPCA_OK;
    }
    int end(int rc) {
        std::lock_guard<std::mutex> lk(ctx->mu);
        if (slot != nullptr) {
            slot->busy = false;
            if (rc == VPCA_OK) {
                slot->nv += nv;
                slot->matched += matched;
            } else {
                ctx->inflight_variants -= nv + slot->nv;
                ctx->st.variants_accumulated -= slot->nv;
                slot->used = false;
            }
        } else if (rc == VPCA_OK) {
            ctx->total_variants += nv;
            ctx->direct_matched += matched;
        } else if (rc == VPCA_ERR_INDEX_OUT_OF_RANGE || rc == VPCA_ERR_OVERFLOW) {
            std::lock_guard<std::mutex> lk2(ctx->err_mu);
            ctx->err += " [direct accumulation: the Gram may hold a partial batch, call vpca_reset]";
            tls_error = ctx->err;
        }
        if (rc == VPCA_OK) ctx->st.variants_accumulated += nv;
        return rc;
    }
};

int prepare_slot(vpca_ctx* ctx, vpca_ctx::Lane& L, CallScope& sc) {
    if (sc.slot == nullptr || !sc.fresh) return VPCA_OK;
    CUDA_OK(ctx, cudaStreamWaitEvent(L.stream, sc.slot->ev_free, 0));
    CUDA_OK(ctx, cudaMemsetAsync(sc.slot->d_S, 0, ctx->slot_bytes(), L.stream));
    return VPCA_OK;
}

void lane_gram_time(vpca_ctx* ctx, vpca_ctx::Lane& L) {
    float ms = 0.f;
    if (cudaEventElapsedTime(&ms, L.ev_t0, L.ev_t1) == cudaSuccess) {
        ctx->lane_gram_ms.store(ms);
        std::lock_guard<std::mutex> lk(ctx->mu);
        ctx->gram_timed = false;
        ctx->st.gram_cta_group = L.plan.cta_group;
        ctx->st.gram_resident = L.plan.last_resident;
    }
}

struct ChunkSink {
    enum Kind { GRAM, LOADINGS, SCORE } kind = GRAM;
    int32_t* gram = nullptr;
    int k = 0;
    double* d_L = nullptr;
    int32_t* d_cnt = nullptr;
    double* h_L = nullptr;
    int32_t* h_cnt = nullptr;
    const int32_t* d_mrows = nullptr;
    double* d_part = nullptr;
    double* d_acc = nullptr;
    bool launched = false;
};

int consume_chunk(vpca_ctx* ctx, GramPlan& plan, cudaStream_t stream, cudaEvent_t t0, cudaEvent_t t1, ChunkSink& sink,
                  const void* d_x, int64_t v, int64_t nvc, int64_t panel) {
    switch (sink.kind) {
    case ChunkSink::GRAM: {
        const int rc = launch_gram(ctx, plan, stream, t0, t1, d_x, nvc, panel, panel, sink.gram);
        if (rc == VPCA_OK) sink.launched = true;
        return rc;
    }
    case ChunkSink::LOADINGS:
        CUDA_OK(ctx, model_loadings(d_x, ctx->elem_bits, nvc, panel, ctx->rows(), ctx->n, ctx->eig.d_evecs, sink.k, sink.d_L,
                                    sink.d_cnt, stream));
        CUDA_OK(ctx, cudaMemcpyAsync(sink.h_L + (size_t)v * sink.k, sink.d_L, (size_t)nvc * sink.k * sizeof(double),
                                     cudaMemcpyDeviceToHost, stream));
        CUDA_OK(ctx, cudaMemcpyAsync(sink.h_cnt + v, sink.d_cnt, (size_t)nvc * sizeof(int32_t), cudaMemcpyDeviceToHost, stream));
        ctx->c_launches += (sink.k + 7) / 8;
        ctx->c_d2h += nvc * (sink.k * 8 + 4);
        return VPCA_OK;
    case ChunkSink::SCORE:
        CUDA_OK(ctx, model_score(d_x, ctx->elem_bits, nvc, panel, ctx->rows(), sink.d_mrows + v, ctx->d_model_L, ctx->d_model_n,
                                 sink.k, sink.d_part, sink.d_acc, stream));
        ctx->c_launches += (sink.k + 7) / 8 + 1;
        return VPCA_OK;
    }
    return fail(ctx, VPCA_ERR_BAD_ARG, "internal: unknown chunk consumer");
}
// ... 1146 lines not shown
    int rc = score_args(ctx, nv, model_rows, &matched);
    if (rc != VPCA_OK) return rc;
    if (offsets == nullptr || (nv > 0 && sample_idx == nullptr && offsets[nv] > offsets[0]))
        return fail(ctx, VPCA_ERR_BAD_ARG, "vpca_score_calls: bad argument");
    CUDA_OK(ctx, cudaSetDevice(ctx->cfg.device));
    if (nv == 0) return VPCA_OK;
    return score_on_lane(ctx, partition_id, nv, matched, model_rows, [&](vpca_ctx::Lane& L, ChunkSink& sink) {
        return process_calls(ctx, L, offsets, sample_idx, 4, nv, &sink, nullptr, 0);
    });
}

int vpca_score_bed(vpca_ctx* ctx, int64_t partition_id, const uint8_t* rows, int64_t nv, int64_t stride_bytes,
                   int32_t counted_allele, const int32_t* model_rows) {
    int64_t matched = 0;
    int rc = score_args(ctx, nv, model_rows, &matched);
    if (rc != VPCA_OK) return rc;
    if (counted_allele != 1 && counted_allele != 2)
        return fail(ctx, VPCA_ERR_BAD_ARG, "vpca_score_bed: counted_allele must be 1 (A1) or 2 (A2)");
    rc = packed_args(ctx, rows, nv, stride_bytes, counted_allele);
    if (rc != VPCA_OK) return rc;
    CUDA_OK(ctx, cudaSetDevice(ctx->cfg.device));
    if (nv == 0) return VPCA_OK;
    return score_on_lane(ctx, partition_id, nv, matched, model_rows, [&](vpca_ctx::Lane& L, ChunkSink& sink) {
        return packed_chunks(ctx, L, rows, nv, stride_bytes, counted_allele, sink);
    });
}

int vpca_score_panels(vpca_ctx* ctx, const void* d_x, int64_t nv, int64_t panel_variants, const int32_t* model_rows) {
    int64_t matched = 0;
    int rc = score_args(ctx, nv, model_rows, &matched);
    if (rc != VPCA_OK) return rc;
    std::lock_guard<std::mutex> dl(ctx->direct_mu);
    std::lock_guard<std::mutex> lk(ctx->mu);
    rc = panels_args(ctx, d_x, nv, panel_variants);
    if (rc != VPCA_OK) return rc;
    CUDA_OK(ctx, cudaSetDevice(ctx->cfg.device));
    if (nv == 0) return VPCA_OK;
    ChunkSink sink;
    rc = score_sink(ctx, &ctx->d_scratch, &ctx->cap_scratch, ctx->stream, model_rows, nv, ctx->d_direct, sink);
    if (rc == VPCA_OK) rc = consume_chunk(ctx, ctx->plan, ctx->stream, ctx->ev_t0, ctx->ev_t1, sink, d_x, 0, nv, panel_variants);
    if (rc != VPCA_OK) return rc;
    ctx->total_variants += nv;
    ctx->st.variants_accumulated += nv;
    ctx->direct_matched += matched;
    return VPCA_OK;
}

int vpca_score_project(vpca_ctx* ctx, int32_t k, double* out, int64_t* matched_variants) {
    if (ctx == nullptr) return fail(nullptr, VPCA_ERR_BAD_ARG, "ctx is NULL");
    if (!ctx->scoring) return fail(ctx, VPCA_ERR_UNSUPPORTED, "vpca_score_project needs a context made by vpca_create_scoring");
    std::lock_guard<std::mutex> dl(ctx->direct_mu);
    std::lock_guard<std::mutex> lk(ctx->mu);
    if (k < 1 || k > ctx->model_k) return fail(ctx, VPCA_ERR_BAD_ARG, "vpca_score_project: k=%d outside [1, %d]", k, ctx->model_k);
    if (out == nullptr) return fail(ctx, VPCA_ERR_BAD_ARG, "out is NULL");
    for (auto& s : ctx->slots)
        if (s.used) return fail(ctx, VPCA_ERR_STATE, "partition %lld is neither committed nor aborted", (long long)s.pid);
    for (auto& L : ctx->lanes)
        if (L.busy) return fail(ctx, VPCA_ERR_STATE, "vpca_score_project while a scoring call is in flight");
    CUDA_OK(ctx, cudaSetDevice(ctx->cfg.device));
    const int m = ctx->n, K = ctx->model_k;
    const size_t ab = align256(ctx->slot_bytes());
    CUDA_OK(ctx, grow_buffer(&ctx->d_scratch, &ctx->cap_scratch, (int64_t)(ab + (size_t)m * k * sizeof(double))));
    double* d_sum = reinterpret_cast<double*>(ctx->d_scratch);
    double* d_y = reinterpret_cast<double*>(ctx->d_scratch + ab);
    CUDA_OK(ctx, cudaMemcpyAsync(d_sum, ctx->d_direct, ctx->slot_bytes(), cudaMemcpyDeviceToDevice, ctx->stream));
    int64_t cnt = ctx->direct_matched;
    for (auto& kv : ctx->scored) {
        CUDA_OK(ctx, model_add(d_sum, kv.second.d_acc, m, K, ctx->stream));
        cnt += kv.second.matched;
    }
    CUDA_OK(ctx, model_finish(d_sum, m, K, k, ctx->model_nfit, ctx->d_model_terms, d_y, ctx->stream));
    ctx->c_launches += (int64_t)ctx->scored.size() + 1;
    CUDA_OK(ctx, cudaMemcpyAsync(out, d_y, (size_t)m * k * sizeof(double), cudaMemcpyDeviceToHost, ctx->stream));
    CUDA_OK(ctx, cudaStreamSynchronize(ctx->stream));
    ctx->c_d2h += (int64_t)m * k * 8;
    if (matched_variants != nullptr) *matched_variants = cnt;
    return VPCA_OK;
}

int vpca_debug_projection_tiles(int32_t n_fit, int32_t n_total, int32_t cta_group, int32_t mxf4, int32_t* out,
                                int32_t max_tiles) {
    if (n_fit < 1 || n_total < n_fit || max_tiles < 0 || (out == nullptr && max_tiles > 0))
        return fail(nullptr, VPCA_ERR_BAD_ARG, "vpca_debug_projection_tiles: bad argument");
    return gram_debug_projection_tiles(n_fit, n_total, cta_group, mxf4 != 0, out, max_tiles);
}

int vpca_get_centered(vpca_ctx* ctx, double* out) {
    if (ctx == nullptr || out == nullptr) return fail(ctx, VPCA_ERR_BAD_ARG, "NULL argument");
    REFUSE_ON_SCORING(ctx);
    std::lock_guard<std::mutex> lk(ctx->mu);
    if (!ctx->finalized) return fail(ctx, VPCA_ERR_STATE, "call vpca_finalize_gram first");
    if (ctx->band_rows != ctx->n) return fail(ctx, VPCA_ERR_STATE, "this context stores a row band of the Gram");
    CUDA_OK(ctx, cudaSetDevice(ctx->cfg.device));
    int rc = run_center(ctx, true);
    if (rc != VPCA_OK) return rc;
    const size_t bytes = (size_t)ctx->n * ctx->n * sizeof(double);
    CUDA_OK(ctx, cudaMemcpyAsync(out, ctx->eig.d_C, bytes, cudaMemcpyDeviceToHost, ctx->stream));
    CUDA_OK(ctx, cudaStreamSynchronize(ctx->stream));
    ctx->c_d2h += (int64_t)bytes;
    ctx->pca_done = false;
    return VPCA_OK;
}

int vpca_get_tridiagonal(vpca_ctx* ctx, double* diag, double* offdiag) {
    if (ctx == nullptr || diag == nullptr || offdiag == nullptr) return fail(ctx, VPCA_ERR_BAD_ARG, "NULL argument");
    REFUSE_ON_SCORING(ctx);
    std::lock_guard<std::mutex> lk(ctx->mu);
    if (!ctx->pca_done) return fail(ctx, VPCA_ERR_STATE, "call vpca_compute_pca first");
    if (ctx->eig.last_method == 2)
        return fail(ctx, VPCA_ERR_STATE, "the last solve used Lanczos and did not tridiagonalise C (set VPCA_EIG=direct)");
    CUDA_OK(ctx, cudaSetDevice(ctx->cfg.device));
    CUDA_OK(ctx, cudaMemcpyAsync(diag, ctx->eig.d_diag, (size_t)ctx->n * 8, cudaMemcpyDeviceToHost, ctx->stream));
    CUDA_OK(ctx, cudaMemcpyAsync(offdiag, ctx->eig.d_off, (size_t)(ctx->n - 1) * 8, cudaMemcpyDeviceToHost, ctx->stream));
    CUDA_OK(ctx, cudaStreamSynchronize(ctx->stream));
    return VPCA_OK;
}

int vpca_synth_dense_device(vpca_ctx* ctx, uint64_t seed, int64_t v0, int64_t nv, int mode, void* d_x, int64_t ld) {
    if (ctx == nullptr) return fail(nullptr, VPCA_ERR_BAD_ARG, "ctx is NULL");
    std::lock_guard<std::mutex> lk(ctx->mu);
    if (d_x == nullptr || nv < 0 || ld < nv || v0 < 0 || (mode != 0 && mode != 1))
        return fail(ctx, VPCA_ERR_BAD_ARG, "vpca_synth_dense_device: bad argument");
    if (mode == 1 && ctx->max_mult < 2)
        return fail(ctx, VPCA_ERR_BAD_ARG, "dosage mode needs max_multiplicity >= 2");
    CUDA_OK(ctx, cudaSetDevice(ctx->cfg.device));
    cudaError_t e = synth_dense(seed, ctx->rows(), v0, nv, mode, ctx->elem_bits, d_x, ld, 0, ctx->stream);
    if (e != cudaSuccess) return fail(ctx, VPCA_ERR_CUDA, "synthetic generator: %s", cudaGetErrorString(e));
    ctx->c_launches += 2 * ((nv + (1 << 22) - 1) >> 22);
    return VPCA_OK;
}

int vpca_get_stats(vpca_ctx* ctx, vpca_stats* out) {
    if (ctx == nullptr || out == nullptr) return fail(ctx, VPCA_ERR_BAD_ARG, "NULL argument");
    std::lock_guard<std::mutex> lk(ctx->mu);
    CUDA_OK(ctx, cudaSetDevice(ctx->cfg.device));
    if (ctx->gram_timed && cudaEventSynchronize(ctx->ev_t1) == cudaSuccess) {
        float ms = 0.f;
        if (cudaEventElapsedTime(&ms, ctx->ev_t0, ctx->ev_t1) == cudaSuccess) ctx->st.last_gram_ms = ms;
    } else if (!ctx->gram_timed) {
        ctx->st.last_gram_ms = ctx->lane_gram_ms.load();
    }
    if (ctx->eig_timed && cudaEventSynchronize(ctx->ev_e1) == cudaSuccess) {
        float ms = 0.f;
        if (cudaEventElapsedTime(&ms, ctx->ev_e0, ctx->ev_e1) == cudaSuccess) ctx->st.last_eig_ms = ms;
    }
    ctx->st.gram_launches = ctx->c_gram.load();
    ctx->st.kernel_launches = ctx->c_launches.load();
    ctx->st.h2d_bytes = ctx->c_h2d.load();
    ctx->st.d2h_bytes = ctx->c_d2h.load();
    *out = ctx->st;
    return VPCA_OK;
}

int vpca_gram_export_ipc(vpca_ctx* ctx, void* handle64) {
    if (ctx == nullptr || handle64 == nullptr) return fail(ctx, VPCA_ERR_BAD_ARG, "NULL argument");
    REFUSE_ON_SCORING(ctx);
    std::lock_guard<std::mutex> lk(ctx->mu);
    if (ctx->n_proj > 0) return fail(ctx, VPCA_ERR_UNSUPPORTED, "projecting contexts reduce through vpca_gram_device_ptr");
    if (!ctx->own_S) return fail(ctx, VPCA_ERR_STATE, "the peer-reduce mode needs a library-owned Gram (vpca_config.d_gram == NULL)");
    if (ctx->band_rows != ctx->n) return fail(ctx, VPCA_ERR_STATE, "band-only Grams are shared with vpca_gram_set_peers_local");
    static_assert(sizeof(cudaIpcMemHandle_t) == 64, "cudaIpcMemHandle_t is 64 bytes");
    CUDA_OK(ctx, cudaSetDevice(ctx->cfg.device));
    cudaIpcMemHandle_t h;
    CUDA_OK(ctx, cudaIpcGetMemHandle(&h, ctx->d_S));
    memcpy(handle64, &h, sizeof(h));
    return VPCA_OK;
}

int vpca_gram_set_peers(vpca_ctx* ctx, const void* handles, int32_t world, int32_t rank) {
    if (ctx == nullptr || handles == nullptr || world < 1 || world > 16 || rank < 0 || rank >= world)
        return fail(ctx, VPCA_ERR_BAD_ARG, "vpca_gram_set_peers: bad argument (world <= 16)");
    REFUSE_ON_SCORING(ctx);
    std::lock_guard<std::mutex> lk(ctx->mu);
    if (ctx->n_proj > 0) return fail(ctx, VPCA_ERR_UNSUPPORTED, "projecting contexts reduce through vpca_gram_device_ptr");
    if (!ctx->own_S) return fail(ctx, VPCA_ERR_STATE, "the peer-reduce mode needs a library-owned Gram");
    if (ctx->plan.num_peers != 0) return fail(ctx, VPCA_ERR_STATE, "peers already set");
    CUDA_OK(ctx, cudaSetDevice(ctx->cfg.device));
    const size_t nn = (size_t)ctx->n * ctx->n;
    for (int d = 0; d < world; ++d) {
        int32_t* base = ctx->d_S;
        if (d != rank) {
            cudaIpcMemHandle_t h;
            memcpy(&h, static_cast<const char*>(handles) + (size_t)d * sizeof(h), sizeof(h));
            void* ptr = nullptr;
            cudaError_t e = cudaIpcOpenMemHandle(&ptr, h, cudaIpcMemLazyEnablePeerAccess);
            if (e != cudaSuccess) {
                for (int q = 0; q < d; ++q)
                    if (q != rank) cudaIpcCloseMemHandle(ctx->plan.peer_base[q]);
                return fail(ctx, VPCA_ERR_NCCL, "cudaIpcOpenMemHandle(rank %d) failed: %s", d, cudaGetErrorString(e));
            }
            base = static_cast<int32_t*>(ptr);
        }
        ctx->plan.peer_base[d] = base;
        ctx->plan.peer_S[d] = base;
        ctx->plan.peer_flags[d] = base + nn;
    }
    CUDA_OK(ctx, gram_preload_kernels(ctx->stream));
    CUDA_OK(ctx, encode_preload_kernels());
    CUDA_OK(ctx, cudaStreamSynchronize(ctx->stream));
    ctx->plan.peers_ipc = true;
    ctx->plan.peer_rank = rank;
    ctx->plan.num_peers = world;
    sync_peers_to_lanes(ctx);
    return VPCA_OK;
}

int vpca_gram_set_peers_local(vpca_ctx* const* ctxs, int32_t world) {
    if (ctxs == nullptr || world < 1 || world > 16) return fail(nullptr, VPCA_ERR_BAD_ARG, "vpca_gram_set_peers_local: world must be in [1, 16]");
    for (int r = 0; r < world; ++r) {
        if (ctxs[r] == nullptr) return fail(nullptr, VPCA_ERR_BAD_ARG, "ctxs[%d] is NULL", r);
        REFUSE_ON_SCORING(ctxs[r]);
        if (ctxs[r]->n_proj > 0)
            return fail(ctxs[r], VPCA_ERR_UNSUPPORTED, "projecting contexts reduce through vpca_gram_device_ptr");
        if (!ctxs[r]->own_S) return fail(ctxs[r], VPCA_ERR_STATE, "the peer-reduce mode needs a library-owned Gram");
        if (ctxs[r]->n != ctxs[0]->n) return fail(ctxs[r], VPCA_ERR_BAD_ARG, "all contexts must have the same n_samples");
        if (ctxs[r]->plan.num_peers != 0) return fail(ctxs[r], VPCA_ERR_STATE, "peers already set");
        for (int q = 0; q < r; ++q)
            if (ctxs[q] == ctxs[r]) return fail(ctxs[r], VPCA_ERR_BAD_ARG, "ctxs[%d] and ctxs[%d] are the same context", q, r);
    }
    for (int r = 0; r < world; ++r) {
        vpca_ctx* c = ctxs[r];
        CUDA_OK(c, cudaSetDevice(c->cfg.device));
        for (int d = 0; d < world; ++d) {
            const int od = ctxs[d]->cfg.device;
            if (od == c->cfg.device) continue;
            int can = 0;
            CUDA_OK(c, cudaDeviceCanAccessPeer(&can, c->cfg.device, od));
            if (!can) return fail(c, VPCA_ERR_NCCL, "device %d cannot access device %d (no NVLink / PCIe peer path)", c->cfg.device, od);
            cudaError_t e = cudaDeviceEnablePeerAccess(od, 0);
            if (e == cudaErrorPeerAccessAlreadyEnabled) {
                cudaGetLastError();
            } else if (e != cudaSuccess) {
                return fail(c, VPCA_ERR_NCCL, "cudaDeviceEnablePeerAccess(%d -> %d): %s", c->cfg.device, od, cudaGetErrorString(e));
            }
        }
    }
    for (int r = 0; r < world; ++r) {
        vpca_ctx* c = ctxs[r];
        CUDA_OK(c, cudaSetDevice(c->cfg.device));
        CUDA_OK(c, gram_preload_kernels(c->stream));
        CUDA_OK(c, encode_preload_kernels());
        CUDA_OK(c, cudaStreamSynchronize(c->stream));
    }
    for (int r = 0; r < world; ++r) {
        vpca_ctx* c = ctxs[r];
        std::lock_guard<std::mutex> lk(c->mu);
        for (int d = 0; d < world; ++d) {
            vpca_ctx* o = ctxs[d];
            c->plan.peer_base[d] = o->d_S;
            c->plan.peer_S[d] = o->d_S - (ptrdiff_t)o->band_row0 * o->n;
            c->plan.peer_flags[d] = o->d_S + (size_t)o->band_rows * o->n;
            c->plan.band_row0[d] = o->band_row0;
            c->plan.band_rows[d] = o->band_rows;
        }
        c->plan.peers_ipc = false;
        c->plan.peer_rank = r;
        c->plan.num_peers = world;
        sync_peers_to_lanes(c);
    }
    return VPCA_OK;
}

int vpca_gram_set_peer_mode(vpca_ctx* ctx, int32_t mode) {
    if (ctx == nullptr) return fail(nullptr, VPCA_ERR_BAD_ARG, "ctx is NULL");
    REFUSE_ON_SCORING(ctx);
    std::lock_guard<std::mutex> lk(ctx->mu);
    if (mode != VPCA_PEER_REPLICATE && mode != VPCA_PEER_OWNER_ROWS)
        return fail(ctx, VPCA_ERR_BAD_ARG, "vpca_gram_set_peer_mode: unknown mode %d", mode);
    if (ctx->plan.num_peers < 1) return fail(ctx, VPCA_ERR_STATE, "call vpca_gram_set_peers first");
    const int world = ctx->plan.num_peers, n = ctx->n;
    if (mode == VPCA_PEER_OWNER_ROWS) {
        if (n < 64 * world)
            return fail(ctx, VPCA_ERR_UNSUPPORTED, "owner-rows mode needs n_samples >= 64 x world (%d < %d)", n, 64 * world);
        int ends[16];
        vpca_owner_row_bands(n, world, ends);
        for (int q = 0; q < 16; ++q) ctx->plan.own_end[q] = q < world ? ends[q] : n;
        for (int q = 0; q < world; ++q) {
            const int lo = q == 0 ? 0 : ends[q - 1];
            if (ctx->plan.band_rows[q] != 0 && ctx->plan.band_rows[q] != n &&
                (ctx->plan.band_row0[q] != lo || ctx->plan.band_rows[q] != ends[q] - lo))
                return fail(ctx, VPCA_ERR_BAD_ARG, "rank %d stores rows [%d, %d) but owns [%d, %d) (see vpca_owner_row_bands)", q,
                            ctx->plan.band_row0[q], ctx->plan.band_row0[q] + ctx->plan.band_rows[q], lo, ends[q]);
        }
    } else if (ctx->band_rows != n) {
        return fail(ctx, VPCA_ERR_BAD_ARG, "a band-only Gram supports VPCA_PEER_OWNER_ROWS only");
    }
    ctx->plan.peer_mode = mode;
    sync_peers_to_lanes(ctx);
    return VPCA_OK;
}

int vpca_owner_row_bands(int32_t n_samples, int32_t world, int32_t* row_end) {
    if (row_end == nullptr || world < 1 || world > 16 || n_samples < 64 * world)
        return fail(nullptr, VPCA_ERR_BAD_ARG, "vpca_owner_row_bands: need 1 <= world <= 16 and n_samples >= 64 x world");
    const int n = n_samples;
    int prev = 0;
    for (int q = 0; q < world; ++q) {
        int end = (q + 1 == world) ? n : (int)(std::sqrt((double)(q + 1) / world) * n / 32.0 + 0.5) * 32;
        end = std::max(end, prev + 32);
        if (q + 1 < world) end = std::min(end, n - 32 * (world - 1 - q));
        row_end[q] = end;
        prev = end;
    }
    return VPCA_OK;
}

// ... 103 lines not shown
```

### spark_examples_b200/csrc/vpca_internal.h

```cpp
#pragma once
#include <cstdint>
#include <cuda_runtime.h>
#include <string>
#include <vector>

#include "../../include/vpca.h"

namespace vpca {

struct GramPlan {
    int cta_group = 2;
    int kb_window = 0;
    int num_sms = 0;
    void* d_tiles = nullptr;
    std::vector<int32_t> h_tiles;
    int num_tiles = 0;
    int num_full = 0;
    int total_weight = 0;
    int tiles_col_limit = 512;
    bool exact_cover = false;
    int tiles_for_n = -1;
    int tiles_for_cg = 0;
    int tiles_for_bn = 0;
    int tiles_row_lo = 0, tiles_row_hi = 0;
    int own_lo = 0, own_hi = 0;
    bool e2m1_mxf4 = true;
    int last_resident = 0;
    int* d_err = nullptr;
    static constexpr int kMaxWindows = 1 << 16;
    int sync_lead = 0;
    int* d_win_done = nullptr;
    bool self_b = true;
    bool red64 = true;
    double gain = 0.5;
    bool adaptive = true;
    double* d_cum = nullptr;
    int cum_workers = 0, cum_tiles = 0, cum_kbw = 0, cum_for_n = 0, cum_for_rows = 0, cum_dev = 0, cum_elem = 0;
    int num_peers = 0, peer_rank = 0, peer_epoch = 0;
    int32_t* peer_S[16] = {};
    int32_t* peer_base[16] = {};
    int32_t* peer_flags[16] = {};
    int band_row0[16] = {}, band_rows[16] = {};
    bool peers_ipc = false;
    int peer_mode = 0;
    int own_end[16] = {};
    bool profile = false;
    long long* d_prof = nullptr;
};
int gram_read_profile(GramPlan& plan, long long* out, int max_ctas);

cudaError_t gram_accumulate(GramPlan& plan, const void* d_x, int elem_bits, int n, int n_rows, int64_t nv, int64_t ld,
                            int64_t panel, int32_t* d_S, cudaStream_t stream, std::string* err);
cudaError_t gram_symmetrize(int32_t* d_S, int n, cudaStream_t stream);
cudaError_t gram_add(int32_t* d_dst, const int32_t* d_src, int64_t count, cudaStream_t stream);
cudaError_t gram_add_peers(GramPlan& plan, const int32_t* d_src, int64_t count, cudaStream_t stream);
cudaError_t gram_add_owners(GramPlan& plan, const int32_t* d_src, int n, cudaStream_t stream);
cudaError_t gram_gather_rows(GramPlan& plan, int32_t* d_S, int n, cudaStream_t stream);
cudaError_t gram_peer_barrier(GramPlan& plan, cudaStream_t stream);
cudaError_t gram_preload_kernels(cudaStream_t stream);
cudaError_t encode_preload_kernels();
void gram_plan_free(GramPlan& plan);
int gram_debug_max_clusters(int cluster_size);
int gram_debug_band_tiles(int n, int cta_group, int row_lo, int row_hi, int32_t* out, int max_tiles);
int gram_debug_projection_tiles(int n_fit, int n_total, int cta_group, bool mxf4, int32_t* out, int max_tiles);
int gram_debug_tiles(int n, int cta_group, int exact, int32_t* out, int max_tiles);
int gram_debug_plan(const int32_t* tiles8, int num_tiles, int workers, int kbw, int32_t* out, int max_pieces);
int gram_debug_repair(const int32_t* tiles8, int num_tiles, int workers, int kbw, int col_limit, double* cum, int32_t* out,
                      int max_pieces);

cudaError_t encode_calls(const int64_t* d_off, int64_t base, const void* d_idx, int idx_bytes, int64_t nv, int n,
                         int elem_bits, int max_mult, void* d_x, int64_t ld, int64_t panel, const int32_t* d_rows,
                         int* d_flags, cudaStream_t stream);

cudaError_t encode_bits(const uint8_t* d_bits, int64_t stride, int64_t nv, int n, int elem_bits, void* d_x, int64_t ld,
                        int64_t panel, int code, const int32_t* d_rows, cudaStream_t stream);

struct JoinWork {
    uint64_t* d_hash = nullptr;
    int32_t* d_table = nullptr;
    uint64_t table_slots = 0;
    int64_t* d_rows = nullptr;
    int64_t* d_len = nullptr;
    int64_t* d_row_base = nullptr;
    int64_t* d_nnz_base = nullptr;
    int32_t* d_leader = nullptr;
    int64_t* d_prefix = nullptr;
    int64_t* d_block = nullptr;
    int64_t* d_totals = nullptr;
    int64_t* h_totals = nullptr;
    int64_t cap_rows = 0;
    int64_t* d_out_off = nullptr;
    int32_t* d_out_idx = nullptr;
    int64_t cap_out_rows = 0, cap_out_nnz = 0;
    int64_t out_rows = -1, out_nnz = 0;
    uint8_t* d_payload = nullptr;
    int64_t* d_key_off = nullptr;
    int64_t* d_off = nullptr;
    int32_t* d_idx = nullptr;
    int64_t cap_payload = 0, cap_in_rows = 0, cap_in_nnz = 0;
};
cudaError_t hash_keys(const uint8_t* d_payload, const int64_t* d_off, int64_t nkeys, uint64_t* d_hash, cudaStream_t stream);
cudaError_t join_rows(JoinWork& w, int mode, int variant_set_count, int64_t n_left, const uint8_t* d_payload,
                      const int64_t* d_key_off, const int64_t* d_off, const int32_t* d_idx, int64_t nrows, cudaStream_t stream,
                      int64_t* out_rows, int64_t* out_nnz, int64_t* launches);
void join_free(JoinWork& w);

struct EigWork {
    int n = 0;
    double* d_C = nullptr;
    double* d_rowsum = nullptr;
    double* d_v = nullptr;
    double* d_w = nullptr;
    double* d_p = nullptr;
    double* d_diag = nullptr;
    double* d_off = nullptr;
    double* d_tau = nullptr;
    double* d_scal = nullptr;
    double* d_mm = nullptr;
    double* d_evals = nullptr;
    double* d_evecs = nullptr;
    double* d_lu = nullptr;
    int* d_nz = nullptr;
    int* d_step = nullptr;
    cudaGraphExec_t graph_exec = nullptr;
    int graph_n = 0;
    bool graph_fused = false;
    int kmax = 0;
    double* d_V = nullptr;
    double* d_lzw = nullptr;
    double* d_lzs = nullptr;
    int* d_lzst = nullptr;
    unsigned* d_lzbar = nullptr;
    double* d_lzG = nullptr;
    long long* d_lzprof = nullptr;
    bool c_valid = false;
    int lz_blocks = 0;
    const int32_t* d_S = nullptr;
    cudaGraphExec_t lz_graph = nullptr;
    int last_method = 0;
    int last_iters = 0;
    int mode = 0;
};
cudaError_t eig_alloc(EigWork& w, int n, int kmax);
void eig_free(EigWork& w);
cudaError_t center_gram(EigWork& w, const int32_t* d_S, cudaStream_t stream, bool materialise);
cudaError_t center_matrix(EigWork& w, cudaStream_t stream);
cudaError_t eig_topk(EigWork& w, int k, cudaStream_t stream, int64_t* launches);
int proj_chunks(int n);
cudaError_t eig_project(const EigWork& w, const int32_t* d_X, int m, int k, double* d_rowmean, double* d_part, double* d_y,
                        cudaStream_t stream);

cudaError_t model_loadings(const void* d_x, int elem_bits, int64_t nv, int64_t panel, int rows, int n_fit, const double* d_u,
                           int k, double* d_L, int32_t* d_carriers, cudaStream_t stream);
size_t model_score_scratch(int m, int k);
cudaError_t model_score(const void* d_x, int elem_bits, int64_t nv, int64_t panel, int m, const int32_t* d_mrows,
                        const double* d_L, const int32_t* d_n, int k, double* d_scratch, double* d_acc, cudaStream_t stream);
cudaError_t model_terms(const double* d_u, const double* d_rowsum, int n, int k, double* d_a, double* d_b, cudaStream_t stream);
cudaError_t model_add(double* d_dst, const double* d_src, int m, int k, cudaStream_t stream);
cudaError_t model_finish(const double* d_acc, int m, int k, int kout, int n_fit, const double* d_terms, double* d_y,
                         cudaStream_t stream);

cudaError_t synth_dense(uint64_t seed, int n, int64_t v0, int64_t nv, int mode, int elem_bits, void* d_x,
                        int64_t ld, int64_t panel, cudaStream_t stream);

}
```

### spark_examples_b200/native.py

```python
from __future__ import annotations

import ctypes
import os
from pathlib import Path
from typing import Optional, Tuple

import numpy as np

VPCA_OK = 0
VPCA_ERR_BAD_ARG = -1
VPCA_ERR_INDEX_OUT_OF_RANGE = -2
VPCA_ERR_CUDA = -3
VPCA_ERR_NCCL = -4
VPCA_ERR_OVERFLOW = -5
VPCA_ERR_STATE = -6
VPCA_ERR_NOMEM = -7
VPCA_ERR_UNSUPPORTED = -8
JOIN, MERGE = 0, 1

DTYPE_I8 = 0
DTYPE_BF16 = 1
DTYPE_E2M1 = 2

_STATUS_NAMES = {
    -1: "BAD_ARG", -2: "INDEX_OUT_OF_RANGE", -3: "CUDA", -4: "NCCL", -5: "OVERFLOW", -6: "STATE",
    -7: "NOMEM", -8: "UNSUPPORTED",
}

EXPORTED_SYMBOLS = (
    "vpca_version", "vpca_create", "vpca_destroy", "vpca_last_error", "vpca_reset", "vpca_encode_calls",
    "vpca_accumulate_calls", "vpca_commit", "vpca_abort", "vpca_accumulate_dense", "vpca_gram_device_ptr",
    "vpca_finalize_gram", "vpca_get_gram", "vpca_set_gram", "vpca_compute_pca", "vpca_get_centered",
    "vpca_get_tridiagonal", "vpca_synth_dense_device", "vpca_get_stats", "vpca_debug_gram_profile",
    "vpca_gram_export_ipc", "vpca_gram_set_peers", "vpca_peer_barrier", "vpca_accumulate_panels",
    "vpca_synth_panels_device", "vpca_accumulate_calls_u16", "vpca_get_partial_gram", "vpca_load_partial_gram",
    "vpca_accumulate_bits", "vpca_gram_set_peer_mode", "vpca_gram_gather", "vpca_accumulate_bed",
    "vpca_synchronize", "vpca_host_alloc", "vpca_host_free", "vpca_gram_set_peers_local", "vpca_owner_row_bands",
    "vpca_get_gram_band", "vpca_variant_count", "vpca_debug_rebalance",
    "vpca_debug_lanczos_profile", "vpca_debug_max_clusters", "vpca_debug_band_tiles", "vpca_hash_keys", "vpca_join_rows", "vpca_join_fetch", "vpca_join_size", "vpca_accumulate_joined",
    "vpca_pool_create", "vpca_pool_destroy", "vpca_pool_size", "vpca_pool_ctx", "vpca_pool_last_error", "vpca_pool_reset",
    "vpca_pool_accumulate_calls", "vpca_pool_accumulate_calls_u16", "vpca_pool_accumulate_bits", "vpca_pool_accumulate_bed",
    "vpca_pool_commit", "vpca_pool_abort", "vpca_pool_reduce_and_finalize", "vpca_pool_get_gram", "vpca_pool_compute_pca",
    "vpca_pool_get_stats", "vpca_debug_tiles", "vpca_debug_plan",
    "vpca_create_projecting", "vpca_get_cross_gram", "vpca_project_pca", "vpca_debug_projection_tiles",
    "vpca_pca_loadings_calls", "vpca_pca_loadings_bed", "vpca_pca_loadings_panels", "vpca_pca_model_terms",
    "vpca_create_scoring", "vpca_score_calls", "vpca_score_bed", "vpca_score_panels", "vpca_score_project",
)


class VpcaError(RuntimeError):

    def __init__(self, code: int, message: str):
        super().__init__(f"vpca {_STATUS_NAMES.get(code, code)}: {message}")
        self.code = code


class IndexOutOfRange(VpcaError, IndexError):
    """Sample index outside [0, N): the reference throws at VariantsPca.scala:59 / :188."""


class VpcaConfig(ctypes.Structure):
    _fields_ = [
        ("struct_size", ctypes.c_uint32),
        ("n_samples", ctypes.c_int32),
        ("device", ctypes.c_int32),
        ("dtype", ctypes.c_int32),
        ("num_pc", ctypes.c_int32),
        ("max_multiplicity", ctypes.c_int32),
        ("partitions_in_flight", ctypes.c_int32),
        ("staging_lanes", ctypes.c_int32),
        ("chunk_variants", ctypes.c_int64),
        ("chunk_nnz", ctypes.c_int64),
        ("stream", ctypes.c_void_p),
        ("d_gram", ctypes.c_void_p),
        ("gram_band_row0", ctypes.c_int32),
        ("gram_band_rows", ctypes.c_int32),
    ]


class VpcaProjection(ctypes.Structure):
    _fields_ = [
        ("struct_size", ctypes.c_uint32),
        ("n_projected", ctypes.c_int32),
        ("sample_rows", ctypes.POINTER(ctypes.c_int32)),
    ]


class VpcaModel(ctypes.Structure):
    _fields_ = [
        ("struct_size", ctypes.c_uint32),
        ("n_fitted", ctypes.c_int32),
        ("k", ctypes.c_int32),
        ("n_variants", ctypes.c_int64),
        ("loadings", ctypes.c_void_p),
        ("carriers", ctypes.c_void_p),
        ("eigenvalues", ctypes.c_void_p),
        ("col_sums", ctypes.c_void_p),
        ("rowsum_dots", ctypes.c_void_p),
        ("matrix_mean", ctypes.c_double),
    ]


class VpcaStats(ctypes.Structure):
    _fields_ = [
        ("variants_accumulated", ctypes.c_int64),
        ("gram_launches", ctypes.c_int64),
        ("kernel_launches", ctypes.c_int64),
        ("h2d_bytes", ctypes.c_int64),
        ("d2h_bytes", ctypes.c_int64),
        ("last_gram_ms", ctypes.c_float),
        ("last_eig_ms", ctypes.c_float),
        ("gram_cta_group", ctypes.c_int32),
        ("gram_resident", ctypes.c_int32),
        ("eig_method", ctypes.c_int32),
        ("eig_iterations", ctypes.c_int32),
    ]


_PKG = Path(__file__).resolve().parent
LIB_PATH = _PKG / "libvpca.so"
_lib: Optional[ctypes.CDLL] = None


def library_path() -> Path:
    return Path(os.environ.get("VPCA_LIBRARY", str(LIB_PATH)))


def load_library() -> ctypes.CDLL:
    global _lib
    if _lib is not None:
        return _lib
    path = library_path()
    if not path.exists():
        raise VpcaError(VPCA_ERR_CUDA, f"{path} not found: build it with `python -c 'import __graft_entry__ as g; "
                        "g.build()'` (there is no CPU fallback)")
    L = ctypes.CDLL(str(path))
    vp, i64, i32 = ctypes.c_void_p, ctypes.c_int64, ctypes.c_int32
    L.vpca_version.restype = ctypes.c_int
    L.vpca_version.argtypes = []
    L.vpca_create.restype = ctypes.c_int
    L.vpca_create.argtypes = [ctypes.POINTER(VpcaConfig), ctypes.POINTER(vp)]
    L.vpca_destroy.restype = ctypes.c_int
    L.vpca_destroy.argtypes = [vp]
    L.vpca_last_error.restype = ctypes.c_char_p
    L.vpca_last_error.argtypes = [vp]
    L.vpca_reset.restype = ctypes.c_int
    L.vpca_reset.argtypes = [vp]
    L.vpca_encode_calls.restype = ctypes.c_int
    L.vpca_encode_calls.argtypes = [vp, vp, vp, i64, vp, i64]
    L.vpca_accumulate_calls.restype = ctypes.c_int
    L.vpca_accumulate_calls.argtypes = [vp, i64, vp, vp, i64]
    L.vpca_accumulate_calls_u16.restype = ctypes.c_int
    L.vpca_accumulate_calls_u16.argtypes = [vp, i64, vp, vp, i64]
    L.vpca_hash_keys.restype = ctypes.c_int
    L.vpca_hash_keys.argtypes = [vp, vp, vp, i64, vp]
    L.vpca_join_rows.restype = ctypes.c_int
    L.vpca_join_rows.argtypes = [vp, i32, i32, i64, vp, vp, vp, vp, i64, ctypes.POINTER(i64), ctypes.POINTER(i64)]
    L.vpca_join_size.restype = ctypes.c_int
    L.vpca_join_size.argtypes = [vp, ctypes.POINTER(i64), ctypes.POINTER(i64)]
    L.vpca_join_fetch.restype = ctypes.c_int
    L.vpca_join_fetch.argtypes = [vp, vp, vp]
    L.vpca_accumulate_joined.restype = ctypes.c_int
    L.vpca_accumulate_joined.argtypes = [vp, i64]
    L.vpca_accumulate_bits.restype = ctypes.c_int
    L.vpca_accumulate_bits.argtypes = [vp, i64, vp, i64, i64]
    L.vpca_accumulate_bed.restype = ctypes.c_int
    L.vpca_accumulate_bed.argtypes = [vp, i64, vp, i64, i64, ctypes.c_int32]
    L.vpca_commit.restype = ctypes.c_int
    L.vpca_commit.argtypes = [vp, i64]
    L.vpca_abort.restype = ctypes.c_int
    L.vpca_abort.argtypes = [vp, i64]
    L.vpca_accumulate_dense.restype = ctypes.c_int
    L.vpca_accumulate_dense.argtypes = [vp, vp, i64, i64, ctypes.c_int]
    L.vpca_gram_device_ptr.restype = ctypes.c_int
    L.vpca_gram_device_ptr.argtypes = [vp, ctypes.POINTER(vp)]
    L.vpca_finalize_gram.restype = ctypes.c_int
    L.vpca_finalize_gram.argtypes = [vp]
    L.vpca_get_gram.restype = ctypes.c_int
    L.vpca_get_gram.argtypes = [vp, vp]
    L.vpca_get_partial_gram.restype = ctypes.c_int
    L.vpca_get_partial_gram.argtypes = [vp, vp, ctypes.POINTER(i64)]
    L.vpca_load_partial_gram.restype = ctypes.c_int
    L.vpca_load_partial_gram.argtypes = [vp, vp, i64]
    L.vpca_variant_count.restype = i64
    L.vpca_variant_count.argtypes = [vp]
    L.vpca_synchronize.restype = ctypes.c_int
    L.vpca_synchronize.argtypes = [vp]
    L.vpca_host_alloc.restype = ctypes.c_int
    L.vpca_host_alloc.argtypes = [ctypes.c_size_t, ctypes.POINTER(vp)]
    L.vpca_host_free.restype = ctypes.c_int
    L.vpca_host_free.argtypes = [vp]
    L.vpca_gram_set_peers_local.restype = ctypes.c_int
    L.vpca_gram_set_peers_local.argtypes = [ctypes.POINTER(vp), i32]
    L.vpca_owner_row_bands.restype = ctypes.c_int
    L.vpca_owner_row_bands.argtypes = [i32, i32, ctypes.POINTER(i32)]
    L.vpca_get_gram_band.restype = ctypes.c_int
    L.vpca_get_gram_band.argtypes = [vp, i32, i32, vp]
    L.vpca_pool_create.restype = ctypes.c_int
    L.vpca_pool_create.argtypes = [ctypes.POINTER(VpcaConfig), i32, ctypes.POINTER(i32), ctypes.POINTER(vp)]
    L.vpca_pool_destroy.restype = ctypes.c_int
    L.vpca_pool_destroy.argtypes = [vp]
    L.vpca_pool_size.restype = i32
    L.vpca_pool_size.argtypes = [vp]
    L.vpca_pool_ctx.restype = vp
    L.vpca_pool_ctx.argtypes = [vp, i64]
    L.vpca_pool_last_error.restype = ctypes.c_char_p
    L.vpca_pool_last_error.argtypes = [vp]
    L.vpca_pool_reset.restype = ctypes.c_int
    L.vpca_pool_reset.argtypes = [vp]
    L.vpca_pool_accumulate_calls.restype = ctypes.c_int
    L.vpca_pool_accumulate_calls.argtypes = [vp, i64, vp, vp, i64]
    L.vpca_pool_accumulate_calls_u16.restype = ctypes.c_int
    L.vpca_pool_accumulate_calls_u16.argtypes = [vp, i64, vp, vp, i64]
    L.vpca_pool_accumulate_bits.restype = ctypes.c_int
    L.vpca_pool_accumulate_bits.argtypes = [vp, i64, vp, i64, i64]
    L.vpca_pool_accumulate_bed.restype = ctypes.c_int
    L.vpca_pool_accumulate_bed.argtypes = [vp, i64, vp, i64, i64, i32]
    L.vpca_pool_commit.restype = ctypes.c_int
    L.vpca_pool_commit.argtypes = [vp, i64]
    L.vpca_pool_abort.restype = ctypes.c_int
    L.vpca_pool_abort.argtypes = [vp, i64]
    L.vpca_pool_reduce_and_finalize.restype = ctypes.c_int
    L.vpca_pool_reduce_and_finalize.argtypes = [vp]
    L.vpca_pool_get_gram.restype = ctypes.c_int
    L.vpca_pool_get_gram.argtypes = [vp, vp]
    L.vpca_pool_compute_pca.restype = ctypes.c_int
    L.vpca_pool_compute_pca.argtypes = [vp, i32, vp, vp, ctypes.POINTER(i32)]
    L.vpca_pool_get_stats.restype = ctypes.c_int
    L.vpca_pool_get_stats.argtypes = [vp, ctypes.POINTER(VpcaStats)]
    L.vpca_debug_tiles.restype = ctypes.c_int
    L.vpca_debug_tiles.argtypes = [i32, i32, i32, vp, i32]
    L.vpca_debug_plan.restype = ctypes.c_int
    L.vpca_debug_plan.argtypes = [vp, i32, i32, i32, vp, i32]
    L.vpca_debug_lanczos_profile.restype = ctypes.c_int
    L.vpca_debug_lanczos_profile.argtypes = [vp, vp, i32]
    L.vpca_debug_rebalance.restype = ctypes.c_int
    L.vpca_debug_rebalance.argtypes = [vp, i32, i32, i32, i32, vp, vp, i32]
    L.vpca_set_gram.restype = ctypes.c_int
    L.vpca_set_gram.argtypes = [vp, vp]
    L.vpca_compute_pca.restype = ctypes.c_int
    L.vpca_compute_pca.argtypes = [vp, i32, vp, vp, ctypes.POINTER(i32)]
    L.vpca_get_centered.restype = ctypes.c_int
    L.vpca_get_centered.argtypes = [vp, vp]
    L.vpca_get_tridiagonal.restype = ctypes.c_int
    L.vpca_get_tridiagonal.argtypes = [vp, vp, vp]
    L.vpca_synth_dense_device.restype = ctypes.c_int
    L.vpca_synth_dense_device.argtypes = [vp, ctypes.c_uint64, i64, i64, ctypes.c_int, vp, i64]
    L.vpca_get_stats.restype = ctypes.c_int
    L.vpca_get_stats.argtypes = [vp, ctypes.POINTER(VpcaStats)]
    L.vpca_accumulate_panels.restype = ctypes.c_int
    L.vpca_accumulate_panels.argtypes = [vp, vp, i64, i64]
    L.vpca_synth_panels_device.restype = ctypes.c_int
    L.vpca_synth_panels_device.argtypes = [vp, ctypes.c_uint64, i64, i64, ctypes.c_int, vp, i64]
    L.vpca_gram_export_ipc.restype = ctypes.c_int
    L.vpca_gram_export_ipc.argtypes = [vp, vp]
    L.vpca_gram_set_peers.restype = ctypes.c_int
    L.vpca_gram_set_peers.argtypes = [vp, vp, i32, i32]
    L.vpca_peer_barrier.restype = ctypes.c_int
    L.vpca_peer_barrier.argtypes = [vp]
    L.vpca_gram_set_peer_mode.restype = ctypes.c_int
    L.vpca_gram_set_peer_mode.argtypes = [vp, ctypes.c_int32]
    L.vpca_gram_gather.restype = ctypes.c_int
    L.vpca_gram_gather.argtypes = [vp]
    L.vpca_debug_gram_profile.restype = ctypes.c_int
    L.vpca_debug_gram_profile.argtypes = [vp, vp, i32]
    L.vpca_create_projecting.restype = ctypes.c_int
    L.vpca_create_projecting.argtypes = [ctypes.POINTER(VpcaConfig), ctypes.POINTER(VpcaProjection), ctypes.POINTER(vp)]
    L.vpca_get_cross_gram.restype = ctypes.c_int
    L.vpca_get_cross_gram.argtypes = [vp, vp]
    L.vpca_project_pca.restype = ctypes.c_int
    L.vpca_project_pca.argtypes = [vp, i32, vp]
    L.vpca_debug_projection_tiles.restype = ctypes.c_int
    L.vpca_debug_projection_tiles.argtypes = [i32, i32, i32, i32, vp, i32]
    L.vpca_pca_loadings_calls.restype = ctypes.c_int
    L.vpca_pca_loadings_calls.argtypes = [vp, i32, vp, vp, i64, vp, vp]
    L.vpca_pca_loadings_bed.restype = ctypes.c_int
    L.vpca_pca_loadings_bed.argtypes = [vp, i32, vp, i64, i64, i32, vp, vp]
    L.vpca_pca_loadings_panels.restype = ctypes.c_int
    L.vpca_pca_loadings_panels.argtypes = [vp, i32, vp, i64, i64, vp, vp]
    L.vpca_pca_model_terms.restype = ctypes.c_int
    L.vpca_pca_model_terms.argtypes = [vp, i32, vp, vp, vp, vp]
    L.vpca_create_scoring.restype = ctypes.c_int
    L.vpca_create_scoring.argtypes = [ctypes.POINTER(VpcaConfig), ctypes.POINTER(VpcaModel), ctypes.POINTER(vp)]
    L.vpca_score_calls.restype = ctypes.c_int
    L.vpca_score_calls.argtypes = [vp, i64, vp, vp, i64, vp]
    L.vpca_score_bed.restype = ctypes.c_int
    L.vpca_score_bed.argtypes = [vp, i64, vp, i64, i64, i32, vp]
    L.vpca_score_panels.restype = ctypes.c_int
    L.vpca_score_panels.argtypes = [vp, vp, i64, i64, vp]
    L.vpca_score_project.restype = ctypes.c_int
    L.vpca_score_project.argtypes = [vp, i32, vp, ctypes.POINTER(i64)]
    _lib = L
    return L


def _host_ptr(a: np.ndarray) -> int:
    return a.ctypes.data


class NativePca:

    def __init__(self, n_samples: int, device: int = 0, dtype: int = DTYPE_I8, num_pc: int = 2,
                 max_multiplicity: int = 2, partitions_in_flight: int = 4, chunk_variants: int = 0,
                 chunk_nnz: int = 0, stream: int = 0, d_gram: int = 0, staging_lanes: int = 0,
                 gram_band: Optional[Tuple[int, int]] = None, n_projected: int = 0, sample_rows=None, model=None):
        self._lib = load_library()
        self.n = int(n_samples)
        self.n_projected = int(n_projected)
        self.rows = self.n + self.n_projected
        self.dtype = int(dtype)
        self.elem_bits = {DTYPE_I8: 8, DTYPE_BF16: 16, DTYPE_E2M1: 4}[self.dtype]
        self.elem_bytes = self.elem_bits / 8
        self.max_multiplicity = int(max_multiplicity) if max_multiplicity > 0 else 2
        row0, rows = gram_band if gram_band is not None else (0, 0)
        cfg = VpcaConfig(ctypes.sizeof(VpcaConfig), n_samples, device, dtype, num_pc, max_multiplicity,
                         partitions_in_flight, staging_lanes, chunk_variants, chunk_nnz, stream or None, d_gram or None,
                         row0, rows)
        handle = ctypes.c_void_p()
        self.model_k = 0
        if model is not None:
            L = np.ascontiguousarray(model.loadings, dtype=np.float64)
            n_var, k = L.shape
            cnt = np.ascontiguousarray(model.carriers, dtype=np.int32)
            terms = [np.ascontiguousarray(getattr(model, f), dtype=np.float64)
                     for f in ("eigenvalues", "col_sums", "rowsum_dots")]
            if cnt.shape != (n_var,) or any(t.shape != (k,) for t in terms):
                raise VpcaError(VPCA_ERR_BAD_ARG, "model: carriers must have V entries and the terms k")
            vm = VpcaModel(ctypes.sizeof(VpcaModel), int(model.n_fitted), k, n_var, _host_ptr(L) if n_var else None,
                           _host_ptr(cnt) if n_var else None, *[_host_ptr(t) for t in terms], float(model.matrix_mean))
            rc = self._lib.vpca_create_scoring(ctypes.byref(cfg), ctypes.byref(vm), ctypes.byref(handle))
            self.model_k = k
        elif self.n_projected > 0 or sample_rows is not None:
            rows_map = None
            if sample_rows is not None:
                rows_map = np.ascontiguousarray(sample_rows, dtype=np.int32)
                if rows_map.shape != (self.rows,):
                    raise VpcaError(VPCA_ERR_BAD_ARG, f"sample_rows must have n_samples + n_projected = {self.rows} entries")
            proj = VpcaProjection(ctypes.sizeof(VpcaProjection), self.n_projected,
                                  rows_map.ctypes.data_as(ctypes.POINTER(ctypes.c_int32)) if rows_map is not None else None)
            rc = self._lib.vpca_create_projecting(ctypes.byref(cfg), ctypes.byref(proj), ctypes.byref(handle))
        else:
            rc = self._lib.vpca_create(ctypes.byref(cfg), ctypes.byref(handle))
        self._h = handle if rc == VPCA_OK else None
        if rc != VPCA_OK:
            self._raise(rc, None)

    def _raise(self, rc: int, handle):
        msg = self._lib.vpca_last_error(handle).decode("utf-8", "replace")
        if rc == VPCA_ERR_INDEX_OUT_OF_RANGE:
            raise IndexOutOfRange(rc, msg)
        raise VpcaError(rc, msg)

    def _check(self, rc: int):
        if rc != VPCA_OK:
            self._raise(rc, self._h)

    def close(self):
        if getattr(self, "_h", None) is not None:
            self._lib.vpca_destroy(self._h)
            self._h = None

    def __del__(self):
        try:
            self.close()
        except Exception:
            pass

    def __enter__(self):
        return self

    def __exit__(self, *exc):
        self.close()

    def reset(self):
        self._check(self._lib.vpca_reset(self._h))

    @staticmethod
    def _csr(offsets, sample_idx) -> Tuple[np.ndarray, np.ndarray]:
        off = np.ascontiguousarray(offsets, dtype=np.int64)
        idx = np.ascontiguousarray(sample_idx, dtype=np.int32)
        if off.ndim != 1 or len(off) < 1:
            raise VpcaError(VPCA_ERR_BAD_ARG, "offsets must be a 1-D array with nv+1 entries")
        return off, idx

    def encodeCalls(self, offsets, sample_idx) -> np.ndarray:
        off, idx = self._csr(offsets, sample_idx)
        nv = len(off) - 1
        if self.elem_bits == 4:
            ld = max(128, ((nv + 127) // 128) * 128)
            out = np.zeros((self.rows, ld // 2), dtype=np.uint8)
            self._check(self._lib.vpca_encode_calls(self._h, _host_ptr(off), _host_ptr(idx) if len(idx) else None, nv,
                                                    _host_ptr(out), ld))
            return out
        out = np.zeros((self.rows, max(nv, 1)), dtype=np.int8 if self.elem_bits == 8 else np.uint16)
        self._check(self._lib.vpca_encode_calls(self._h, _host_ptr(off), _host_ptr(idx) if len(idx) else None, nv,
                                                _host_ptr(out), out.shape[1]))
        return out[:, :nv]

    def accumulateCalls(self, partition_id: int, offsets, sample_idx):
        off, idx = self._csr(offsets, sample_idx)
        self._check(self._lib.vpca_accumulate_calls(self._h, int(partition_id), _host_ptr(off),
                                                    _host_ptr(idx) if len(idx) else None, len(off) - 1))
# ... 123 lines not shown
        self._check(self._lib.vpca_gram_set_peers(self._h, blob, len(handles), int(rank)))
        self._check(self._lib.vpca_gram_set_peer_mode(self._h, {"replicate": 0, "owner_rows": 1}[mode]))

    def gatherGram(self):
        self._check(self._lib.vpca_gram_gather(self._h))

    def peerBarrier(self):
        self._check(self._lib.vpca_peer_barrier(self._h))

    def finalizeGram(self):
        self._check(self._lib.vpca_finalize_gram(self._h))

    def getGram(self) -> np.ndarray:
        out = np.empty((self.n, self.n), dtype=np.int32)
        self._check(self._lib.vpca_get_gram(self._h, _host_ptr(out)))
        return out

    def partialGram(self, with_count: bool = False):
        out = np.empty((self.rows, self.n), dtype=np.int32)
        nv = ctypes.c_int64(0)
        self._check(self._lib.vpca_get_partial_gram(self._h, _host_ptr(out), ctypes.byref(nv)))
        return (out, int(nv.value)) if with_count else out

    def loadPartialGram(self, gram: np.ndarray, variants_in_gram: int):
        g = np.ascontiguousarray(gram, dtype=np.int32)
        if g.shape != (self.rows, self.n):
            raise VpcaError(VPCA_ERR_BAD_ARG, "gram must be (n + n_projected, n)")
        self._check(self._lib.vpca_load_partial_gram(self._h, _host_ptr(g), int(variants_in_gram)))

    def variantCount(self) -> int:
        v = int(self._lib.vpca_variant_count(self._h))
        if v < 0:
            self._raise(v, self._h)
        return v

    def synchronize(self):
        self._check(self._lib.vpca_synchronize(self._h))

    def gramBand(self, row0: int, rows: int) -> np.ndarray:
        out = np.empty((rows, self.n), dtype=np.int32)
        self._check(self._lib.vpca_get_gram_band(self._h, int(row0), int(rows), _host_ptr(out)))
        return out

    def setGram(self, gram: np.ndarray):
        g = np.ascontiguousarray(gram, dtype=np.int32)
        if g.shape != (self.n, self.n):
            raise VpcaError(VPCA_ERR_BAD_ARG, "gram must be (n, n)")
        self._check(self._lib.vpca_set_gram(self._h, _host_ptr(g)))

    def computePca(self, k: int = 2):
        flat = np.empty(self.n * k, dtype=np.float64)
        evals = np.empty(k, dtype=np.float64)
        nz = ctypes.c_int32(0)
        self._check(self._lib.vpca_compute_pca(self._h, int(k), _host_ptr(flat), _host_ptr(evals), ctypes.byref(nz)))
        return flat.reshape(k, self.n).T.copy(), evals, int(nz.value)

    def crossGram(self) -> np.ndarray:
        out = np.empty((self.n_projected, self.n), dtype=np.int32)
        self._check(self._lib.vpca_get_cross_gram(self._h, _host_ptr(out)))
        return out

    def projectPca(self, k: int = 2) -> np.ndarray:
        flat = np.empty(max(self.n_projected * k, 1), dtype=np.float64)
        self._check(self._lib.vpca_project_pca(self._h, int(k), _host_ptr(flat)))
        return flat[:self.n_projected * k].reshape(k, self.n_projected).T.copy()

    def pcaLoadingsCalls(self, k: int, offsets, sample_idx):
        off, idx = self._csr(offsets, sample_idx)
        nv = len(off) - 1
        L, cnt = np.empty((nv, k), np.float64), np.empty(nv, np.int32)
        self._check(self._lib.vpca_pca_loadings_calls(self._h, int(k), _host_ptr(off), _host_ptr(idx) if len(idx) else None,
                                                      nv, _host_ptr(L), _host_ptr(cnt)))
        return L, cnt

    def pcaLoadingsBed(self, k: int, rows: np.ndarray, counted_allele: int = 1):
        b = np.ascontiguousarray(rows, dtype=np.uint8)
        if b.ndim != 2:
            raise VpcaError(VPCA_ERR_BAD_ARG, "rows must be (nv, stride_bytes)")
        L, cnt = np.empty((b.shape[0], k), np.float64), np.empty(b.shape[0], np.int32)
        self._check(self._lib.vpca_pca_loadings_bed(self._h, int(k), _host_ptr(b), b.shape[0], b.shape[1],
                                                    int(counted_allele), _host_ptr(L), _host_ptr(cnt)))
        return L, cnt

    def pcaLoadingsPanels(self, k: int, d_ptr: int, nv: int, panel_variants: int):
        L, cnt = np.empty((nv, k), np.float64), np.empty(nv, np.int32)
        self._check(self._lib.vpca_pca_loadings_panels(self._h, int(k), d_ptr, int(nv), int(panel_variants), _host_ptr(L),
                                                       _host_ptr(cnt)))
        return L, cnt

    def pcaModelTerms(self, k: int) -> dict:
        ev, a, b = (np.empty(k, np.float64) for _ in range(3))
        mm = np.empty(1, np.float64)
        self._check(self._lib.vpca_pca_model_terms(self._h, int(k), _host_ptr(ev), _host_ptr(a), _host_ptr(b), _host_ptr(mm)))
        return dict(eigenvalues=ev, col_sums=a, rowsum_dots=b, matrix_mean=float(mm[0]))

    @staticmethod
    def _model_rows(model_rows, nv: int) -> np.ndarray:
        r = np.ascontiguousarray(model_rows, dtype=np.int32)
        if r.shape != (nv,):
            raise VpcaError(VPCA_ERR_BAD_ARG, f"model_rows must have one entry per variant ({nv})")
        return r

    def scoreCalls(self, partition_id: int, offsets, sample_idx, model_rows):
        off, idx = self._csr(offsets, sample_idx)
        r = self._model_rows(model_rows, len(off) - 1)
        self._check(self._lib.vpca_score_calls(self._h, int(partition_id), _host_ptr(off), _host_ptr(idx) if len(idx) else None,
                                               len(off) - 1, _host_ptr(r) if len(r) else None))

    def scoreBed(self, partition_id: int, rows: np.ndarray, model_rows, counted_allele: int = 1):
        b = np.ascontiguousarray(rows, dtype=np.uint8)
        if b.ndim != 2:
            raise VpcaError(VPCA_ERR_BAD_ARG, "rows must be (nv, stride_bytes)")
        r = self._model_rows(model_rows, b.shape[0])
        self._check(self._lib.vpca_score_bed(self._h, int(partition_id), _host_ptr(b), b.shape[0], b.shape[1],
                                             int(counted_allele), _host_ptr(r) if len(r) else None))

    def scorePanels(self, d_ptr: int, nv: int, panel_variants: int, model_rows):
        r = self._model_rows(model_rows, nv)
        self._check(self._lib.vpca_score_panels(self._h, d_ptr, int(nv), int(panel_variants), _host_ptr(r) if len(r) else None))

    def scoreProject(self, k: int = 2):
        flat = np.empty(self.n * k, dtype=np.float64)
        matched = ctypes.c_int64(0)
        self._check(self._lib.vpca_score_project(self._h, int(k), _host_ptr(flat), ctypes.byref(matched)))
        return flat.reshape(k, self.n).T.copy(), int(matched.value)

    def getCentered(self) -> np.ndarray:
        out = np.empty((self.n, self.n), dtype=np.float64)
        self._check(self._lib.vpca_get_centered(self._h, _host_ptr(out)))
        return out

    def getTridiagonal(self):
        d = np.empty(self.n, dtype=np.float64)
        e = np.empty(self.n - 1, dtype=np.float64)
        self._check(self._lib.vpca_get_tridiagonal(self._h, _host_ptr(d), _host_ptr(e)))
        return d, e

    def synthDenseDevice(self, seed: int, v0: int, nv: int, mode: int, d_ptr: int, ld: int):
        self._check(self._lib.vpca_synth_dense_device(self._h, ctypes.c_uint64(seed), int(v0), int(nv), int(mode),
                                                      d_ptr, int(ld)))

    def gramProfile(self, max_ctas: int = 1024) -> np.ndarray:
        out = np.zeros((max_ctas, 4), dtype=np.int64)
        rc = self._lib.vpca_debug_gram_profile(self._h, _host_ptr(out), max_ctas)
        if rc < 0:
            self._raise(rc, self._h)
        return out[:rc]

    def stats(self) -> dict:
        st = VpcaStats()
        self._check(self._lib.vpca_get_stats(self._h, ctypes.byref(st)))
        return {name: getattr(st, name) for name, _ in VpcaStats._fields_}


def debugTiles(n_samples: int, cta_group: int = 2, exact: bool = True) -> np.ndarray:
    L = load_library()
    cnt = L.vpca_debug_tiles(int(n_samples), int(cta_group), 1 if exact else 0, None, 0)
    if cnt < 0:
        raise VpcaError(cnt, L.vpca_last_error(None).decode("utf-8", "replace"))
    out = np.zeros((cnt, 8), dtype=np.int32)
    L.vpca_debug_tiles(int(n_samples), int(cta_group), 1 if exact else 0, _host_ptr(out), cnt)
    return out


def debugPlan(tiles: np.ndarray, workers: int, kb_window: int) -> np.ndarray:
    L = load_library()
    t = np.ascontiguousarray(tiles, dtype=np.int32)
    cap = 8 * int(workers) + 8
    out = np.zeros((cap, 6), dtype=np.int32)
    cnt = L.vpca_debug_plan(_host_ptr(t), len(t), int(workers), int(kb_window), _host_ptr(out), cap)
    if cnt < 0:
        raise VpcaError(VPCA_ERR_STATE, L.vpca_last_error(None).decode("utf-8", "replace"))
    return out[:cnt]


def debugProjectionTiles(n_fit: int, n_total: int, cta_group: int, mxf4: bool) -> np.ndarray:
    L = load_library()
    cnt = L.vpca_debug_projection_tiles(int(n_fit), int(n_total), int(cta_group), 1 if mxf4 else 0, None, 0)
    if cnt < 0:
        raise VpcaError(cnt, L.vpca_last_error(None).decode("utf-8", "replace"))
    out = np.zeros((cnt, 8), dtype=np.int32)
    L.vpca_debug_projection_tiles(int(n_fit), int(n_total), int(cta_group), 1 if mxf4 else 0, _host_ptr(out), cnt)
    return out


def debugBandTiles(n_samples: int, cta_group: int, row0: int, rows: int) -> np.ndarray:
    L = load_library()
    L.vpca_debug_band_tiles.restype = ctypes.c_int
    L.vpca_debug_band_tiles.argtypes = [ctypes.c_int32] * 4 + [ctypes.c_void_p, ctypes.c_int32]
    cnt = L.vpca_debug_band_tiles(int(n_samples), int(cta_group), int(row0), int(rows), None, 0)
    if cnt < 0:
        raise VpcaError(cnt, L.vpca_last_error(None).decode("utf-8", "replace"))
    out = np.zeros((cnt, 8), dtype=np.int32)
    L.vpca_debug_band_tiles(int(n_samples), int(cta_group), int(row0), int(rows), _host_ptr(out), cnt)
    return out


def gramSourceFingerprint() -> str:
    import hashlib
    import re
    src = (Path(__file__).resolve().parent / "csrc" / "gram_sm100.cu").read_text()
    src = re.sub(r"/\*.*?\*/", "", src, flags=re.S)
    src = re.sub(r"//[^\n]*", "", src)
    src = re.sub(r"\s+", "", src)
    return hashlib.sha256(src.encode()).hexdigest()[:16]


def maxClusters(device: int, cluster_size: int) -> int:
    L = load_library()
    L.vpca_debug_max_clusters.restype = ctypes.c_int
    L.vpca_debug_max_clusters.argtypes = [ctypes.c_int32, ctypes.c_int32]
    c = L.vpca_debug_max_clusters(int(device), int(cluster_size))
    if c < 0:
        raise VpcaError(c, L.vpca_last_error(None).decode("utf-8", "replace"))
    return c


def debugRebalance(tiles: np.ndarray, workers: int, kb_window: int, cum: np.ndarray, col_limit: int = 512):
    L = load_library()
    t = np.ascontiguousarray(tiles, dtype=np.int32)
    c = np.ascontiguousarray(cum, dtype=np.float64).copy()
    assert c.shape == (workers + 1,)
    cap = 8 * int(workers) + 8
    out = np.zeros((cap, 6), dtype=np.int32)
    cnt = L.vpca_debug_rebalance(_host_ptr(t), len(t), int(workers), int(kb_window), int(col_limit), _host_ptr(c),
                                 _host_ptr(out), cap)
    if cnt < 0:
        raise VpcaError(cnt, L.vpca_last_error(None).decode("utf-8", "replace"))
    return c, out[:cnt]


def ownerRowBands(n_samples: int, world: int) -> list:
    L = load_library()
    ends = (ctypes.c_int32 * world)()
    rc = L.vpca_owner_row_bands(int(n_samples), int(world), ends)
    if rc != VPCA_OK:
        raise VpcaError(rc, L.vpca_last_error(None).decode("utf-8", "replace"))
    out, prev = [], 0
    for q in range(world):
        out.append((prev, int(ends[q]) - prev))
        prev = int(ends[q])
    return out


def setPeersLocal(contexts, mode: str = "owner_rows"):
    L = load_library()
    arr = (ctypes.c_void_p * len(contexts))(*[c._h.value for c in contexts])
    rc = L.vpca_gram_set_peers_local(arr, len(contexts))
    if rc != VPCA_OK:
        raise VpcaError(rc, L.vpca_last_error(None).decode("utf-8", "replace"))
    for c in contexts:
        c._check(L.vpca_gram_set_peer_mode(c._h, {"replicate": 0, "owner_rows": 1}[mode]))


class NativePcaPool:

    def __init__(self, n_samples: int, n_gpus: int, devices=None, dtype: int = DTYPE_I8, num_pc: int = 2,
                 max_multiplicity: int = 2, partitions_in_flight: int = 4, staging_lanes: int = 0,
                 chunk_variants: int = 0, chunk_nnz: int = 0):
        self._lib = load_library()
        self.n = int(n_samples)
        cfg = VpcaConfig(ctypes.sizeof(VpcaConfig), n_samples, 0, dtype, num_pc, max_multiplicity, partitions_in_flight,
                         staging_lanes, chunk_variants, chunk_nnz, None, None, 0, 0)
        devs = None
        if devices is not None:
            devs = (ctypes.c_int32 * n_gpus)(*[int(d) for d in devices])
        h = ctypes.c_void_p()
        rc = self._lib.vpca_pool_create(ctypes.byref(cfg), int(n_gpus), devs, ctypes.byref(h))
        self._h = h if rc == VPCA_OK else None
        if rc != VPCA_OK:
            self._raise(rc)

    def _raise(self, rc: int):
        msg = self._lib.vpca_pool_last_error(self._h).decode("utf-8", "replace")
        if rc == VPCA_ERR_INDEX_OUT_OF_RANGE:
            raise IndexOutOfRange(rc, msg)
        raise VpcaError(rc, msg)

    def _check(self, rc: int):
        if rc != VPCA_OK:
            self._raise(rc)

    def close(self):
        if getattr(self, "_h", None) is not None:
            self._lib.vpca_pool_destroy(self._h)
            self._h = None

    def __del__(self):
        try:
            self.close()
        except Exception:
            pass

    def __enter__(self):
        return self

    def __exit__(self, *exc):
        self.close()

    @property
    def size(self) -> int:
        return int(self._lib.vpca_pool_size(self._h))

    def reset(self):
        self._check(self._lib.vpca_pool_reset(self._h))

# ... 46 lines not shown
```

Before: 1528 billion.

## Route small-valued int8 genotypes through fused on-device FP4 transcode and MXF4 Gram

Adds a cooperative KIND=4 Gram kernel. Spare warps transcode int8 genotype panels (values bounded by max_mult) into e2m1 FP4 in a ring buffer, and the tensor cores consume that ring with kind::mxf4 MMAs. Per-window ready and free counters let transcoding overlap the MMA work. If any value is out of range, a guarded int8 kernel launch recomputes the result exactly. The aim is to double MMA throughput and halve the operand bytes, at the cost of an extra read and write pass over the input, grid-wide spin waits, and a fallback launch that is always enqueued.

```diff
diff --git a/include/vpca.h b/include/vpca.h
--- a/include/vpca.h
+++ b/include/vpca.h
@@ -175,6 +175,7 @@
     int32_t eig_iterations;
 } vpca_stats;
 int vpca_get_stats(vpca_ctx* ctx, vpca_stats* out);
+int vpca_get_i8_mxf4_stats(vpca_ctx* ctx, int64_t out[2]);
 int vpca_debug_gram_profile(vpca_ctx* ctx, int64_t* out, int32_t max_ctas);
 int vpca_debug_lanczos_profile(vpca_ctx* ctx, int64_t* out, int32_t max_steps);
 
diff --git a/spark_examples_b200/csrc/gram_sm100.cu b/spark_examples_b200/csrc/gram_sm100.cu
--- a/spark_examples_b200/csrc/gram_sm100.cu
+++ b/spark_examples_b200/csrc/gram_sm100.cu
@@ -81,6 +81,17 @@
     int row_limit;
     int red64;
     int tx_shift;
+    const int8_t* xsrc;
+    uint8_t* ring;
+    int ring_slots;
+    int n_rows_x;
+    int max_mult;
+    int last_valid;
+    int* bad;
+    int* win_ready;
+    int* win_free;
+    const int* guard;
+    int* recomputes;
 };
 
 struct Seg {
@@ -328,6 +339,91 @@
     }
 }
 
+__device__ __forceinline__ void wait_count(const int* cnt, int need, int* err, int code) {
+    const long long t0 = clock64();
+    while (true) {
+        int v;
+        asm volatile("ld.acquire.gpu.global.s32 %0, [%1];" : "=r"(v) : "l"(cnt) : "memory");
+        if (v >= need) return;
+        if (clock64() - t0 > kWatchdogCycles) {
+            if (err != nullptr) {
+                err[0] = code;
+                err[1] = (int)blockIdx.x;
+                err[2] = v;
+                err[3] = need;
+                __threadfence_system();
+            }
+            __trap();
+        }
+        __nanosleep(64);
+    }
+}
+
+__device__ __forceinline__ void fence_proxy_async_global() {
+    asm volatile("fence.proxy.async.global;" ::: "memory");
+}
+
+__device__ __forceinline__ uint32_t e2m1_pack8(uint32_t lo, uint32_t hi) {
+    const uint32_t y = __byte_perm(lo | (lo >> 4), hi | (hi >> 4), 0x6420);
+    const uint32_t m = (y & 0x22222222u) | (y & ~(y >> 1) & 0x11111111u) | ((y >> 1) & 0x22222222u);
+    return y + m;
+}
+
+__device__ void transcode_panels(const GramArgs& a, int t) {
+    constexpr int kThr = kThreads - 64, kUnroll = 4;
+    const int nwin = (a.kb_total + a.kb_window - 1) / a.kb_window;
+    const int cells = a.kb_per_panel * 256;
+    const int upr = cells / 32;
+    const int units = a.n_rows_x * upr;
+    const int u0 = (int)((long long)units * blockIdx.x / gridDim.x), u1 = (int)((long long)units * (blockIdx.x + 1) / gridDim.x);
+    const uint32_t mmx = 0x01010101u * (uint32_t)a.max_mult;
+    uint32_t bad = 0;
+    for (int w = 0; w < nwin; ++w) {
+        if (w >= a.ring_slots) {
+            if (t == 0) wait_count(a.win_free + (w - a.ring_slots), a.num_workers, a.err, 6);
+            asm volatile("bar.sync 1, %0;" ::"n"(kThr) : "memory");
+            fence_proxy_async_global();
+        }
+        const uint4* src = reinterpret_cast<const uint4*>(a.xsrc + (size_t)w * a.n_rows_x * cells);
+        uint4* dst = reinterpret_cast<uint4*>(a.ring + (size_t)(w % a.ring_slots) * a.n_rows_x * (cells / 2));
+        const int valid = (w == nwin - 1) ? a.last_valid : cells;
+        for (int ub = u0 + t; ub < u1; ub += kUnroll * kThr) {
+            uint4 v[kUnroll][2];
+#pragma unroll
+            for (int j = 0; j < kUnroll; ++j) {
+                const int u = ub + j * kThr;
+                if (u < u1) {
+                    v[j][0] = __ldcs(src + 2 * (size_t)u);
+                    v[j][1] = __ldcs(src + 2 * (size_t)u + 1);
+                }
+            }
+#pragma unroll
+            for (int j = 0; j < kUnroll; ++j) {
+                const int u = ub + j * kThr;
+                if (u >= u1) break;
+                uint4 o = make_uint4(0u, 0u, 0u, 0u);
+                if (valid == cells || (u % upr) * 32 < valid) {
+                    const uint4 p = v[j][0], q = v[j][1];
+                    bad |= __vcmpgtu4(p.x, mmx) | __vcmpgtu4(p.y, mmx) | __vcmpgtu4(p.z, mmx) | __vcmpgtu4(p.w, mmx) |
+                           __vcmpgtu4(q.x, mmx) | __vcmpgtu4(q.y, mmx) | __vcmpgtu4(q.z, mmx) | __vcmpgtu4(q.w, mmx);
+                    o = make_uint4(e2m1_pack8(p.x, p.y), e2m1_pack8(p.z, p.w), e2m1_pack8(q.x, q.y), e2m1_pack8(q.z, q.w));
+                }
+                dst[u] = o;
+            }
+        }
+        if (bad != 0) {
+            atomicOr(a.bad, 1);
+            bad = 0;
+        }
+        fence_proxy_async_global();
+        asm volatile("bar.sync 1, %0;" ::"n"(kThr) : "memory");
+        if (t == 0) {
+            __threadfence();
+            asm volatile("red.release.gpu.global.add.s32 [%0], 1;" ::"l"(a.win_ready + w) : "memory");
+        }
+    }
+}
+
 __device__ __forceinline__ uint64_t make_smem_desc(uint32_t saddr) {
     return (uint64_t)((saddr & 0x3FFFFu) >> 4) | ((uint64_t)(1024 >> 4) << 32) | (1ull << 46) | (2ull << 61);
 }
@@ -335,7 +431,7 @@
 template <int CG, int KIND>
 __device__ __forceinline__ uint32_t make_instr_desc(uint32_t N) {
     constexpr uint32_t M = 128 * CG;
-    if constexpr (KIND == 3) {
+    if constexpr (KIND >= 3) {
         return (1u << 7) | (1u << 10) | ((N >> 3) << 17) | (1u << 23) | ((M >> 4) << 24);
     }
     constexpr uint32_t cfmt = (KIND == 0) ? 2u : 1u;
@@ -367,6 +463,13 @@
     const int worker = (CG == 2) ? (int)(blockIdx.x >> 1) : (int)blockIdx.x;
     const bool issuer = ptx::elect_one();
 
+    if constexpr (KIND == 0) {
+        if (a.guard != nullptr) {
+            if (*reinterpret_cast<const volatile int*>(a.guard) == 0) return;
+            if (blockIdx.x == 0 && threadIdx.x == 0) atomicAdd(a.recomputes, 1);
+        }
+    }
+
     if constexpr (CG == 2) ptx::cluster_sync();
 
     if (warp == 0 && issuer) {
@@ -388,7 +491,7 @@
     if constexpr (CG == 2) ptx::cluster_sync(); else __syncthreads();
     ptx::tc_fence_after();
     const uint32_t tmem_base = *tmem_ptr_smem;
-    if constexpr (KIND == 3) {
+    if constexpr (KIND >= 3) {
         if (warp >= 4) {
             ptx::tmem_st_32x32b_x16_const(tmem_base + ((uint32_t)((warp & 3) * 32) << 16) + kSfCol, 0x7F7F7F7Fu);
             ptx::tmem_st_wait();
@@ -414,15 +517,22 @@
                 const bool self_b = (CG == 2) && (s.flags & kTileSelfB) != 0;
                 const uint32_t tx_cta =
                     (uint32_t)(C::A_BYTES + (self_b ? 0 : (half_box ? kBoxBytes / 2 : (two_boxes ? 2 * kBoxBytes : kBoxBytes))));
-                if (a.sync_lead > 0 && leader && s.win != synced_win) {
+                if constexpr (KIND == 4) {
+                    if (s.win != synced_win && s.kb0 < s.kb1) {
+                        synced_win = s.win;
+                        wait_count(a.win_ready + s.win, (int)gridDim.x, a.err, 5);
+                        fence_proxy_async_global();
+                    }
+                } else if (a.sync_lead > 0 && leader && s.win != synced_win) {
                     synced_win = s.win;
                     if (s.win >= a.sync_lead) wait_window(a.win_done, s.win - a.sync_lead, a.active_workers);
                 }
                 for (int kb = s.kb0; kb < s.kb1; ++kb, ++it) {
                     const uint32_t st = it % C::STAGES, ph = (it / C::STAGES) & 1u;
                     mbar_wait(empty_bar(st), ph ^ 1u, a.err, 1);
-                    const int pnl = kb / a.kb_per_panel;
+                    int pnl = kb / a.kb_per_panel;
                     const int kc = (kb - pnl * a.kb_per_panel) * a.elems_per_kb;
+                    if constexpr (KIND == 4) pnl %= a.ring_slots;
                     if constexpr (CG == 1) {
                         ptx::mbar_arrive_expect_tx(full_bar(st), tx_cta >> a.tx_shift);
                         ptx::tma_load_3d(sA(st), &tmap, full_bar(st), kc, rowA, pnl);
@@ -444,6 +554,7 @@
         sc.init(a, worker);
         Seg s;
         uint32_t it = 0;
+        int freed = 0;
         while (sc.next(s)) {
             if (s.first && !a.resident) {
                 mbar_wait(tempty_bar((uint32_t)s.slot), (uint32_t)(s.use & 1) ^ 1u, a.err, 2);
@@ -461,7 +572,7 @@
                     uint32_t acc = (s.first && kb == s.kb0) ? 0u : 1u;
 #pragma unroll
                     for (int k = 0; k < kKBytes / 32; ++k) {
-                        if constexpr (KIND == 3)
+                        if constexpr (KIND >= 3)
                             ptx::umma_ss_mxf4<CG>(d_tmem, adesc + 2 * k, bdesc + 2 * k, idesc, acc, tmem_base + kSfCol,
                                                   tmem_base + kSfCol + 4);
                         else
@@ -472,13 +583,33 @@
                 }
                 __syncwarp();
             }
+            if constexpr (KIND == 4) {
+                if (s.last_in_win && issuer) {
+                    asm volatile("red.release.gpu.global.add.s32 [%0], 1;" ::"l"(a.win_free + s.win) : "memory");
+                    freed = s.win + 1;
+                }
+            }
             if (s.flush) {
                 if (issuer) ptx::umma_commit<CG>(tfull_bar((uint32_t)s.slot));
                 __syncwarp();
             }
         }
+        if constexpr (KIND == 4) {
+            const int nwin = (a.kb_total + a.kb_window - 1) / a.kb_window;
+            for (; issuer && freed < nwin; ++freed)
+                asm volatile("red.release.gpu.global.add.s32 [%0], 1;" ::"l"(a.win_free + freed) : "memory");
+        }
         if (a.prof != nullptr && issuer) a.prof[(size_t)blockIdx.x * 4 + 2] = globaltimer_ns();
+    } else if (KIND == 4 && warp >= 2 && warp < 4) {
+        transcode_panels(a, (int)threadIdx.x - 64);
     } else if (warp >= 4) {
+        bool skip = false;
+        if constexpr (KIND == 4) {
+            transcode_panels(a, (int)threadIdx.x - 64);
+            const int nwin = (a.kb_total + a.kb_window - 1) / a.kb_window;
+            wait_count(a.win_ready + nwin - 1, (int)gridDim.x, a.err, 7);
+            skip = *reinterpret_cast<const volatile int*>(a.bad) != 0;
+        }
         const int q = warp & 3;
         Sched sc;
         sc.init(a, worker);
@@ -493,7 +624,7 @@
             const int col = colbase + (int)lane;
             const uint32_t taddr = tmem_base + ((uint32_t)(q * 32) << 16) + (uint32_t)s.col;
             const int row_end = min(a.row_limit, s.rowB + s.n_eff);
-            const int nchunks = filler ? 0 : (s.n_eff + 31) / 32;
+            const int nchunks = (filler || skip) ? 0 : (s.n_eff + 31) / 32;
 #pragma unroll 1
             for (int c = 0; c < nchunks; ++c) {
                 const int rbase = s.rowB + c * 32;
@@ -802,24 +933,54 @@
     cfg.blockDim = dim3(kThreads);
     cfg.dynamicSmemBytes = C::SMEM_BYTES;
     cfg.stream = stream;
-    cudaLaunchAttribute attr[1];
+    cudaLaunchAttribute attr[2];
     attr[0].id = cudaLaunchAttributeClusterDimension;
     attr[0].val.clusterDim.x = CG;
     attr[0].val.clusterDim.y = 1;
     attr[0].val.clusterDim.z = 1;
+    attr[1].id = cudaLaunchAttributeCooperative;
+    attr[1].val.cooperative = 1;
+    cfg.attrs = attr;
+    cfg.numAttrs = KIND == 4 ? 2 : 1;
+    return cudaLaunchKernelEx(&cfg, gram_kernel<CG, KIND>, tmap, tmap_half, args);
+}
+
+bool i8_mxf4_fits(int grid) {
+    using C = Cfg<2, 4>;
+    int dev = 0, coop = 0;
+    cudaGetDevice(&dev);
+    if (cudaDeviceGetAttribute(&coop, cudaDevAttrCooperativeLaunch, dev) != cudaSuccess || coop == 0) return false;
+    if (cudaFuncSetAttribute(gram_kernel<2, 4>, cudaFuncAttributeMaxDynamicSharedMemorySize, C::SMEM_BYTES) != cudaSuccess) {
+        cudaGetLastError();
+        return false;
+    }
+    cudaLaunchConfig_t cfg{};
+    cfg.gridDim = dim3((unsigned)grid);
+    cfg.blockDim = dim3(kThreads);
+    cfg.dynamicSmemBytes = C::SMEM_BYTES;
+    cudaLaunchAttribute attr[1];
+    attr[0].id = cudaLaunchAttributeClusterDimension;
+    attr[0].val.clusterDim.x = 2;
+    attr[0].val.clusterDim.y = 1;
+    attr[0].val.clusterDim.z = 1;
     cfg.attrs = attr;
     cfg.numAttrs = 1;
-    return cudaLaunchKernelEx(&cfg, gram_kernel<CG, KIND>, tmap, tmap_half, args);
+    int clusters = 0;
+    if (cudaOccupancyMaxActiveClusters(&clusters, gram_kernel<2, 4>, &cfg) != cudaSuccess) {
+        cudaGetLastError();
+        return false;
+    }
+    return 2 * clusters >= grid;
 }
 
 }
 
 namespace {
 struct SplitKey {
-    int dev, n, rows, tiles, kbw, workers, elem;
+    int dev, n, rows, tiles, kbw, workers, elem, kind;
     bool operator<(const SplitKey& o) const {
-        return std::tie(dev, n, rows, tiles, kbw, workers, elem) <
-               std::tie(o.dev, o.n, o.rows, o.tiles, o.kbw, o.workers, o.elem);
+        return std::tie(dev, n, rows, tiles, kbw, workers, elem, kind) <
+               std::tie(o.dev, o.n, o.rows, o.tiles, o.kbw, o.workers, o.elem, o.kind);
     }
 };
 std::mutex g_split_mu;
@@ -835,10 +996,21 @@
         return;
     }
     std::lock_guard<std::mutex> lk(g_split_mu);
-    g_splits[SplitKey{plan.cum_dev, plan.cum_for_n, plan.cum_for_rows, plan.cum_tiles, plan.cum_kbw, plan.cum_workers, plan.cum_elem}] = std::move(cum);
+    g_splits[SplitKey{plan.cum_dev, plan.cum_for_n, plan.cum_for_rows, plan.cum_tiles, plan.cum_kbw, plan.cum_workers, plan.cum_elem,
+                      plan.cum_kind}] = std::move(cum);
 }
 
 void gram_plan_free(GramPlan& plan) {
+    if (plan.fp4 != nullptr) {
+        gram_plan_free(*plan.fp4);
+        delete plan.fp4;
+        plan.fp4 = nullptr;
+    }
+    if (plan.d_ring) cudaFree(plan.d_ring);
+    if (plan.d_sync) cudaFree(plan.d_sync);
+    plan.d_ring = nullptr;
+    plan.ring_bytes = 0;
+    plan.d_sync = nullptr;
     remember_split(plan);
     if (plan.d_tiles) cudaFree(plan.d_tiles);
     plan.h_tiles.clear();
@@ -1051,14 +1223,7 @@
     return cnt;
 }
 
-cudaError_t gram_accumulate(GramPlan& plan, const void* d_x, int elem_bits, int n, int n_rows, int64_t nv, int64_t ld,
-                            int64_t panel, int32_t* d_S, cudaStream_t stream, std::string* err) {
-    if (nv <= 0) return cudaSuccess;
-    EncodeTiledFn encode = get_encode_fn();
-    if (encode == nullptr) {
-        if (err) *err = "cuTensorMapEncodeTiled entry point not available";
-        return cudaErrorNotSupported;
-    }
+static void plan_init(GramPlan& plan) {
     if (plan.num_sms == 0) {
         int dev = 0;
         cudaGetDevice(&dev);
@@ -1083,6 +1248,28 @@
         if (gain != nullptr) plan.gain = std::min(1.0, std::max(0.1, atof(gain)));
         const char* ex = getenv("VPCA_EXACT_COVER");
         if (ex != nullptr) plan.exact_cover = atoi(ex) != 0;
+        const char* im = getenv("VPCA_I8_MXF4");
+        if (im != nullptr) plan.i8_mxf4 = atoi(im) != 0;
+        const char* rs = getenv("VPCA_I8_MXF4_RING");
+        if (rs != nullptr) plan.ring_slots = std::max(1, atoi(rs));
+    }
+}
+
+struct Route {
+    bool fp4;
+    const int* guard;
+    GramPlan* owner;
+    int max_mult;
+    bool declined;
+};
+
+static cudaError_t accumulate_impl(GramPlan& plan, const void* d_x, int elem_bits, int n, int n_rows, int64_t nv, int64_t ld,
+                                   int64_t panel, int32_t* d_S, cudaStream_t stream, std::string* err, Route* route) {
+    const bool fp4 = route != nullptr && route->fp4;
+    EncodeTiledFn encode = get_encode_fn();
+    if (encode == nullptr) {
+        if (err) *err = "cuTensorMapEncodeTiled entry point not available";
+        return cudaErrorNotSupported;
     }
     if (plan.d_win_done == nullptr) {
         cudaError_t e = cudaMalloc(&plan.d_win_done, GramPlan::kMaxWindows * sizeof(int));
@@ -1095,11 +1282,11 @@
         if (e != cudaSuccess) return e;
     }
     if (plan.d_err == nullptr) {
-        cudaError_t e = cudaHostAlloc(&plan.d_err, 4 * sizeof(int), cudaHostAllocMapped);
+        cudaError_t e = cudaHostAlloc(&plan.d_err, 8 * sizeof(int), cudaHostAllocMapped);
         if (e != cudaSuccess) return e;
-        for (int i = 0; i < 4; ++i) plan.d_err[i] = 0;
-    }
-    const bool mxf4 = (elem_bits == 4 && plan.e2m1_mxf4);
+        for (int i = 0; i < 8; ++i) plan.d_err[i] = 0;
+    }
+    const bool mxf4 = (elem_bits == 4 && plan.e2m1_mxf4) || fp4;
     const int tile_bn = mxf4 ? kUmmaNScaled : kUmmaN;
     const bool banded = plan.own_hi > plan.own_lo && plan.num_peers <= 1;
     const int row_lo = banded ? plan.own_lo : 0, row_hi = banded ? plan.own_hi : n_rows;
@@ -1130,7 +1317,7 @@
     const int cgp = plan.cta_group;
     const int workers = (cgp == 2) ? plan.num_sms / 2 : plan.num_sms;
     const int elems_per_kb = (elem_bits == 16) ? 64 : (mxf4 ? 256 : 128);
-    const int kind = (elem_bits == 8) ? 0 : (elem_bits == 16 ? 1 : (mxf4 ? 3 : 2));
+    const int kind = fp4 ? 4 : ((elem_bits == 8) ? 0 : (elem_bits == 16 ? 1 : (mxf4 ? 3 : 2)));
     if (mxf4 && panel > 0 && (panel % 256) != 0) {
         if (err) *err = "kind::mxf4 needs panel_variants % 256 == 0";
         return cudaErrorInvalidValue;
@@ -1138,18 +1325,20 @@
 
     CUtensorMap tmap;
     const int64_t npanels = panel > 0 ? (nv + panel - 1) / panel : 1;
+    const int tm_bits = fp4 ? 4 : elem_bits;
+    void* tm_base = fp4 ? static_cast<void*>(route->owner->d_ring) : const_cast<void*>(d_x);
     const int64_t dim0 = panel > 0 ? panel : (elem_bits == 4 ? (mxf4 ? ((nv + 1) / 2) * 2 : ((nv + 127) / 128) * 128) : nv);
-    const cuuint64_t gdim[3] = {(cuuint64_t)dim0, (cuuint64_t)n_rows, (cuuint64_t)npanels};
-    const cuuint64_t gstride[2] = {(cuuint64_t)ld * (cuuint64_t)elem_bits / 8,
-                                   (cuuint64_t)n_rows * (cuuint64_t)ld * (cuuint64_t)elem_bits / 8};
+    const cuuint64_t gdim[3] = {(cuuint64_t)dim0, (cuuint64_t)n_rows, (cuuint64_t)(fp4 ? route->owner->ring_slots : npanels)};
+    const cuuint64_t gstride[2] = {(cuuint64_t)ld * (cuuint64_t)tm_bits / 8,
+                                   (cuuint64_t)n_rows * (cuuint64_t)ld * (cuuint64_t)tm_bits / 8};
     const cuuint32_t box[3] = {(cuuint32_t)elems_per_kb, (cuuint32_t)kBoxRows, 1};
     const cuuint32_t estr[3] = {1, 1, 1};
-    const CUtensorMapDataType tmtype = elem_bits == 8 ? CU_TENSOR_MAP_DATA_TYPE_UINT8
-                                       : (elem_bits == 16 ? CU_TENSOR_MAP_DATA_TYPE_BFLOAT16
-                                                          : (mxf4 ? CU_TENSOR_MAP_DATA_TYPE_16U4_ALIGN8B
-                                                                  : CU_TENSOR_MAP_DATA_TYPE_16U4_ALIGN16B));
+    const CUtensorMapDataType tmtype = tm_bits == 8 ? CU_TENSOR_MAP_DATA_TYPE_UINT8
+                                       : (tm_bits == 16 ? CU_TENSOR_MAP_DATA_TYPE_BFLOAT16
+                                                        : (mxf4 ? CU_TENSOR_MAP_DATA_TYPE_16U4_ALIGN8B
+                                                                : CU_TENSOR_MAP_DATA_TYPE_16U4_ALIGN16B));
     CUresult r = encode(&tmap, tmtype, 3,
-                        const_cast<void*>(d_x), gdim, gstride, box, estr, CU_TENSOR_MAP_INTERLEAVE_NONE,
+                        tm_base, gdim, gstride, box, estr, CU_TENSOR_MAP_INTERLEAVE_NONE,
                         CU_TENSOR_MAP_SWIZZLE_128B, CU_TENSOR_MAP_L2_PROMOTION_L2_256B,
                         CU_TENSOR_MAP_FLOAT_OOB_FILL_NONE);
     if (r != CUDA_SUCCESS) {
@@ -1158,7 +1347,7 @@
     }
     CUtensorMap tmap_half;
     const cuuint32_t box_half[3] = {(cuuint32_t)elems_per_kb, (cuuint32_t)(kBoxRows / 2), 1};
-    r = encode(&tmap_half, tmtype, 3, const_cast<void*>(d_x), gdim, gstride, box_half, estr, CU_TENSOR_MAP_INTERLEAVE_NONE,
+    r = encode(&tmap_half, tmtype, 3, tm_base, gdim, gstride, box_half, estr, CU_TENSOR_MAP_INTERLEAVE_NONE,
                CU_TENSOR_MAP_SWIZZLE_128B, CU_TENSOR_MAP_L2_PROMOTION_L2_256B, CU_TENSOR_MAP_FLOAT_OOB_FILL_NONE);
     if (r != CUDA_SUCCESS) {
         if (err) *err = "cuTensorMapEncodeTiled (64-row box) failed with CUresult " + std::to_string((int)r);
@@ -1186,7 +1375,7 @@
     args.row_limit = row_hi;
     args.red64 = plan.red64 ? 1 : 0;
     {
-        int kbw = plan.kb_window;
+        int kbw = fp4 ? args.kb_per_panel : plan.kb_window;
         if (kbw <= 0 && panel > 0) kbw = args.kb_per_panel;
         if (kbw <= 0) {
             const long long target = 32ll << 20;
@@ -1195,16 +1384,20 @@
         kbw = std::min(kbw, args.kb_total);
         std::vector<double> cum0;
         args.resident = (plan.num_tiles <= 4 * workers && initial_split(plan, workers, kbw, cum0)) ? 1 : 0;
+        if (fp4 && (!args.resident || (args.kb_total + kbw - 1) / kbw > GramPlan::kMaxWindows)) {
+            route->declined = true;
+            return cudaSuccess;
+        }
         int dev = 0;
         cudaGetDevice(&dev);
         args.kb_window = args.resident ? kbw : args.kb_total;
         if (args.resident && (plan.d_cum == nullptr || plan.cum_workers != workers || plan.cum_tiles != plan.num_tiles ||
                               plan.cum_kbw != kbw || plan.cum_for_n != n || plan.cum_for_rows != n_rows ||
-                              plan.cum_elem != elem_bits)) {
+                              plan.cum_elem != elem_bits || plan.cum_kind != kind)) {
             remember_split(plan);
             if (plan.adaptive && !banded) {
                 std::lock_guard<std::mutex> lk(g_split_mu);
-                auto it = g_splits.find(SplitKey{dev, n, n_rows, plan.num_tiles, kbw, workers, elem_bits});
+                auto it = g_splits.find(SplitKey{dev, n, n_rows, plan.num_tiles, kbw, workers, elem_bits, kind});
                 if (it != g_splits.end()) {
                     std::vector<double> learned = it->second;
                     const TileDesc* tiles = reinterpret_cast<const TileDesc*>(plan.h_tiles.data());
@@ -1229,15 +1422,17 @@
             plan.cum_for_rows = n_rows;
             plan.cum_dev = dev;
             plan.cum_elem = elem_bits;
+            plan.cum_kind = kind;
         }
     }
     plan.last_resident = args.resident;
     const int nwin = (args.kb_total + args.kb_window - 1) / args.kb_window;
     const long long uw = (long long)args.total_weight * args.kb_window;
     args.active_workers = (int)std::min<long long>(workers, uw);
-    args.sync_lead = (args.resident && nwin <= GramPlan::kMaxWindows) ? plan.sync_lead : 0;
+    args.sync_lead = (args.resident && nwin <= GramPlan::kMaxWindows && !fp4) ? plan.sync_lead : 0;
     args.win_done = plan.d_win_done;
-    const bool adapt = plan.adaptive && args.resident && workers <= 1024 && args.active_workers == workers;
+    const bool guarded = route != nullptr && route->guard != nullptr;
+    const bool adapt = plan.adaptive && args.resident && workers <= 1024 && args.active_workers == workers && !guarded;
     args.prof = (plan.profile || adapt) ? plan.d_prof : nullptr;
     args.cum = plan.d_cum;
     args.tx_shift = (elem_bits == 4 && !mxf4 && getenv("VPCA_E2M1_TX_FULL") == nullptr) ? 1 : 0;
@@ -1245,17 +1440,40 @@
         cudaError_t e = cudaMemsetAsync(plan.d_win_done, 0, (size_t)nwin * sizeof(int), stream);
         if (e != cudaSuccess) return e;
     }
-
+    if (guarded) {
+        args.guard = route->guard;
+        cudaHostGetDevicePointer(reinterpret_cast<void**>(&args.recomputes), plan.d_err + 4, 0);
+    }
     const int grid = workers * cgp;
-    cudaError_t le;
-    if (cgp == 2)
+    cudaError_t le = cudaSuccess;
+    if (fp4) {
+        GramPlan& o = *route->owner;
+        args.xsrc = static_cast<const int8_t*>(d_x);
+        args.ring = o.d_ring;
+        args.ring_slots = o.ring_slots;
+        args.n_rows_x = n_rows;
+        args.max_mult = route->max_mult;
+        args.last_valid = (int)(((nv - (npanels - 1) * panel) + 127) / 128 * 128);
+        args.bad = o.d_sync;
+        args.win_ready = o.d_sync + 1;
+        args.win_free = o.d_sync + 1 + nwin;
+        cudaError_t e = cudaMemsetAsync(o.d_sync, 0, (size_t)(1 + 2 * nwin) * sizeof(int), stream);
+        if (e != cudaSuccess) return e;
+        if (launch<2, 4>(tmap, tmap_half, args, grid, stream) != cudaSuccess) {
+            cudaGetLastError();
+            o.i8_mxf4_coop = 0;
+            route->declined = true;
+            return cudaSuccess;
+        }
+    } else if (cgp == 2) {
         le = kind == 0 ? launch<2, 0>(tmap, tmap_half, args, grid, stream)
                        : (kind == 1 ? launch<2, 1>(tmap, tmap_half, args, grid, stream)
                                     : (kind == 2 ? launch<2, 2>(tmap, tmap_half, args, grid, stream) : launch<2, 3>(tmap, tmap_half, args, grid, stream)));
-    else
+    } else {
         le = kind == 0 ? launch<1, 0>(tmap, tmap_half, args, grid, stream)
                        : (kind == 1 ? launch<1, 1>(tmap, tmap_half, args, grid, stream)
                                     : (kind == 2 ? launch<1, 2>(tmap, tmap_half, args, grid, stream) : launch<1, 3>(tmap, tmap_half, args, grid, stream)));
+    }
     if (le != cudaSuccess) return le;
     if (adapt) {
         rebalance_kernel<<<1, 1024, 0, stream>>>(plan.d_prof, plan.d_cum, workers, cgp, plan.gain, 1.35, 300000,
@@ -1266,12 +1484,68 @@
     return le;
 }
 
+cudaError_t gram_accumulate(GramPlan& plan, const void* d_x, int elem_bits, int n, int n_rows, int64_t nv, int64_t ld,
+                            int64_t panel, int max_mult, int32_t* d_S, cudaStream_t stream, std::string* err) {
+    if (nv <= 0) return cudaSuccess;
+    plan_init(plan);
+    const bool banded = plan.own_hi > plan.own_lo && plan.num_peers <= 1;
+    if (!(elem_bits == 8 && panel > 0 && panel % 256 == 0 && max_mult >= 1 && max_mult <= 4 && plan.i8_mxf4 &&
+          plan.cta_group == 2 && !plan.exact_cover && plan.num_peers <= 1 && !banded))
+        return accumulate_impl(plan, d_x, elem_bits, n, n_rows, nv, ld, panel, d_S, stream, err, nullptr);
+    if (plan.fp4 == nullptr) {
+        plan.fp4 = new GramPlan();
+        GramPlan& f = *plan.fp4;
+        f.num_sms = plan.num_sms;
+        f.cta_group = plan.cta_group;
+        f.profile = plan.profile;
+        f.adaptive = plan.adaptive;
+        f.self_b = plan.self_b;
+        f.red64 = plan.red64;
+        f.gain = plan.gain;
+    }
+    GramPlan& f = *plan.fp4;
+    if (plan.i8_mxf4_coop < 0) plan.i8_mxf4_coop = i8_mxf4_fits(plan.num_sms / 2 * 2) ? 1 : 0;
+    if (plan.i8_mxf4_coop == 0)
+        return accumulate_impl(plan, d_x, elem_bits, n, n_rows, nv, ld, panel, d_S, stream, err, nullptr);
+    const size_t ring = (size_t)plan.ring_slots * n_rows * (size_t)(panel / 2);
+    if (plan.ring_bytes < ring) {
+        if (plan.d_ring) cudaFree(plan.d_ring);
+        plan.d_ring = nullptr;
+        plan.ring_bytes = 0;
+        cudaError_t e = cudaMalloc(&plan.d_ring, ring);
+        if (e != cudaSuccess) return e;
+        plan.ring_bytes = ring;
+    }
+    if (plan.d_sync == nullptr) {
+        cudaError_t e = cudaMalloc(&plan.d_sync, (size_t)(1 + 2 * GramPlan::kMaxWindows) * sizeof(int));
+        if (e != cudaSuccess) return e;
+    }
+    const int64_t limit = (16777216ll / ((int64_t)max_mult * max_mult)) / panel * panel;
+    for (int64_t v0 = 0; v0 < nv; v0 += limit) {
+        const int64_t cnt = std::min(limit, nv - v0);
+        const char* x = static_cast<const char*>(d_x) + (size_t)(v0 / panel) * (size_t)n_rows * (size_t)panel;
+        Route fr{true, nullptr, &plan, max_mult, false};
+        cudaError_t e = accumulate_impl(f, x, elem_bits, n, n_rows, cnt, ld, panel, d_S, stream, err, &fr);
+        if (e != cudaSuccess) return e;
+        if (fr.declined) {
+            plan.i8_mxf4_declined += 1;
+            e = accumulate_impl(plan, x, elem_bits, n, n_rows, cnt, ld, panel, d_S, stream, err, nullptr);
+        } else {
+            plan.i8_mxf4_launches += 1;
+            Route gr{false, plan.d_sync, &plan, max_mult, false};
+            e = accumulate_impl(plan, x, elem_bits, n, n_rows, cnt, ld, panel, d_S, stream, err, &gr);
+        }
+        if (e != cudaSuccess) return e;
+    }
+    return cudaSuccess;
+}
+
 cudaError_t gram_preload_kernels(cudaStream_t stream) {
     cudaFuncAttributes fa;
     cudaError_t e = cudaSuccess;
 #define VPCA_LOAD(k) if (e == cudaSuccess) e = cudaFuncGetAttributes(&fa, k)
     VPCA_LOAD((gram_kernel<1, 0>)); VPCA_LOAD((gram_kernel<1, 1>)); VPCA_LOAD((gram_kernel<1, 2>)); VPCA_LOAD((gram_kernel<1, 3>));
-    VPCA_LOAD((gram_kernel<2, 0>)); VPCA_LOAD((gram_kernel<2, 1>)); VPCA_LOAD((gram_kernel<2, 2>)); VPCA_LOAD((gram_kernel<2, 3>));
+    VPCA_LOAD((gram_kernel<2, 0>)); VPCA_LOAD((gram_kernel<2, 1>)); VPCA_LOAD((gram_kernel<2, 2>)); VPCA_LOAD((gram_kernel<2, 3>)); VPCA_LOAD((gram_kernel<2, 4>));
     VPCA_LOAD(rebalance_kernel); VPCA_LOAD(symmetrize_kernel); VPCA_LOAD(add_i32_kernel); VPCA_LOAD(add_i32_peers_kernel);
     VPCA_LOAD(add_i32_owner_kernel); VPCA_LOAD(gather_rows_kernel); VPCA_LOAD(push_rows_kernel); VPCA_LOAD(peer_barrier_kernel);
 #undef VPCA_LOAD
diff --git a/spark_examples_b200/csrc/vpca.cu b/spark_examples_b200/csrc/vpca.cu
--- a/spark_examples_b200/csrc/vpca.cu
+++ b/spark_examples_b200/csrc/vpca.cu
@@ -313,7 +313,7 @@
         const size_t byte_off = panel > 0 ? (size_t)(v0 / panel) * (size_t)ctx->rows() * (size_t)panel * ctx->elem_bits / 8
                                           : (size_t)v0 * ctx->elem_bits / 8;
         cudaError_t e = gram_accumulate(plan, static_cast<const char*>(d_x) + byte_off, ctx->elem_bits, ctx->n, ctx->rows(),
-                                        cnt, ld, panel, d_target, stream, &msg);
+                                        cnt, ld, panel, ctx->max_mult, d_target, stream, &msg);
         cudaEventRecord(t1, stream);
         if (e != cudaSuccess)
             return fail(ctx, VPCA_ERR_CUDA, "Gram launch failed: %s %s", cudaGetErrorString(e), msg.c_str());
@@ -1766,6 +1766,19 @@
     return VPCA_OK;
 }
 
+int vpca_get_i8_mxf4_stats(vpca_ctx* ctx, int64_t* out) {
+    if (ctx == nullptr || out == nullptr) return fail(ctx, VPCA_ERR_BAD_ARG, "NULL argument");
+    std::lock_guard<std::mutex> lk(ctx->mu);
+    out[0] = out[1] = 0;
+    auto add = [&](const GramPlan& p) {
+        out[0] += p.i8_mxf4_launches;
+        out[1] += p.i8_mxf4_declined + (p.d_err != nullptr ? *reinterpret_cast<volatile int*>(p.d_err + 4) : 0);
+    };
+    add(ctx->plan);
+    for (const auto& L : ctx->lanes) add(L.plan);
+    return VPCA_OK;
+}
+
 int vpca_gram_export_ipc(vpca_ctx* ctx, void* handle64) {
     if (ctx == nullptr || handle64 == nullptr) return fail(ctx, VPCA_ERR_BAD_ARG, "NULL argument");
     REFUSE_ON_SCORING(ctx);
diff --git a/spark_examples_b200/csrc/vpca_internal.h b/spark_examples_b200/csrc/vpca_internal.h
--- a/spark_examples_b200/csrc/vpca_internal.h
+++ b/spark_examples_b200/csrc/vpca_internal.h
@@ -46,11 +46,21 @@
     int own_end[16] = {};
     bool profile = false;
     long long* d_prof = nullptr;
+    int cum_kind = 0;
+    bool i8_mxf4 = true;
+    int i8_mxf4_coop = -1;
+    int ring_slots = 3;
+    GramPlan* fp4 = nullptr;
+    uint8_t* d_ring = nullptr;
+    size_t ring_bytes = 0;
+    int* d_sync = nullptr;
+    int64_t i8_mxf4_launches = 0;
+    int64_t i8_mxf4_declined = 0;
 };
 int gram_read_profile(GramPlan& plan, long long* out, int max_ctas);
 
 cudaError_t gram_accumulate(GramPlan& plan, const void* d_x, int elem_bits, int n, int n_rows, int64_t nv, int64_t ld,
-                            int64_t panel, int32_t* d_S, cudaStream_t stream, std::string* err);
+                            int64_t panel, int max_mult, int32_t* d_S, cudaStream_t stream, std::string* err);
 cudaError_t gram_symmetrize(int32_t* d_S, int n, cudaStream_t stream);
 cudaError_t gram_add(int32_t* d_dst, const int32_t* d_src, int64_t count, cudaStream_t stream);
 cudaError_t gram_add_peers(GramPlan& plan, const int32_t* d_src, int64_t count, cudaStream_t stream);
diff --git a/spark_examples_b200/native.py b/spark_examples_b200/native.py
--- a/spark_examples_b200/native.py
+++ b/spark_examples_b200/native.py
@@ -31,7 +31,7 @@
     "vpca_version", "vpca_create", "vpca_destroy", "vpca_last_error", "vpca_reset", "vpca_encode_calls",
     "vpca_accumulate_calls", "vpca_commit", "vpca_abort", "vpca_accumulate_dense", "vpca_gram_device_ptr",
     "vpca_finalize_gram", "vpca_get_gram", "vpca_set_gram", "vpca_compute_pca", "vpca_get_centered",
-    "vpca_get_tridiagonal", "vpca_synth_dense_device", "vpca_get_stats", "vpca_debug_gram_profile",
+    "vpca_get_tridiagonal", "vpca_synth_dense_device", "vpca_get_stats", "vpca_get_i8_mxf4_stats", "vpca_debug_gram_profile",
     "vpca_gram_export_ipc", "vpca_gram_set_peers", "vpca_peer_barrier", "vpca_accumulate_panels",
     "vpca_synth_panels_device", "vpca_accumulate_calls_u16", "vpca_get_partial_gram", "vpca_load_partial_gram",
     "vpca_accumulate_bits", "vpca_gram_set_peer_mode", "vpca_gram_gather", "vpca_accumulate_bed",
@@ -248,6 +248,8 @@
     L.vpca_synth_dense_device.argtypes = [vp, ctypes.c_uint64, i64, i64, ctypes.c_int, vp, i64]
     L.vpca_get_stats.restype = ctypes.c_int
     L.vpca_get_stats.argtypes = [vp, ctypes.POINTER(VpcaStats)]
+    L.vpca_get_i8_mxf4_stats.restype = ctypes.c_int
+    L.vpca_get_i8_mxf4_stats.argtypes = [vp, vp]
     L.vpca_accumulate_panels.restype = ctypes.c_int
     L.vpca_accumulate_panels.argtypes = [vp, vp, i64, i64]
     L.vpca_synth_panels_device.restype = ctypes.c_int
@@ -677,6 +679,11 @@
         self._check(self._lib.vpca_get_stats(self._h, ctypes.byref(st)))
         return {name: getattr(st, name) for name, _ in VpcaStats._fields_}
 
+    def i8Mxf4Stats(self) -> dict:
+        out = np.zeros(2, np.int64)
+        self._check(self._lib.vpca_get_i8_mxf4_stats(self._h, _host_ptr(out)))
+        return {"i8_mxf4_launches": int(out[0]), "i8_mxf4_fallbacks": int(out[1])}
+
 
 def debugTiles(n_samples: int, cta_group: int = 2, exact: bool = True) -> np.ndarray:
     L = load_library()
```

Result: faster. 1782 billion (median of 6 runs) (+16.6%).
